# ktht/chan_vese

Measured on AMD Instinct MI355X. Metric: Mpixel-iterations/s (CSV u-update), higher is better.
Workload: dtype f64

## Files before the change

chan_vese_amd/csrc/api.hip:

```cpp
#include "cvh_host.h"

static thread_local char g_create_err[kErrLen] = "no error";
char *create_err() { return g_create_err; }

int fail(cvh_context *ctx, int code, const char *fmt, ...)
{
  char *dst = ctx ? ctx->err : g_create_err;
  va_list ap;
  va_start(ap, fmt);
  vsnprintf(dst, 512, fmt, ap);
  va_end(ap);
  return code;
}

extern "C" const char *cvh_version(void) { return "chanvese_hip 0.1 (gfx950)"; }

void cvh_fill_note(CvhLaunchNote *note, unsigned grid, unsigned block, size_t lds, const char *fmt, ...)
{
  va_list ap;
  va_start(ap, fmt);
  vsnprintf(note->name, sizeof(note->name), fmt, ap);
  va_end(ap);
  note->grid = grid; note->block = block; note->lds = (unsigned)lds;
}

void fill_atan_tables(double *tab)
{
  const long double pil = 3.14159265358979323846264338327950288L;
  for (int i = 0; i < CVH_ATAN_N; ++i) {
    const long double at = atanl((long double)i / (CVH_ATAN_N - 1));
    tab[i] = (double)at;
    tab[CVH_ATAN_N + i] = (double)(pil / 2 - at);
  }
  for (int j = 0; j < CVH_ATAN2_N; ++j)
    tab[2 * CVH_ATAN_N + j] = (double)((pil / 4 + atanl((long double)(j - 128) / 128)) / pil);
}

extern "C" void cvh_default_params(cvh_params *p)
{
  if (!p) return;
  p->mu = 0.5; p->nu = 0.0; p->dt = 1.0; p->eps = 1.0; p->tol = 0.001;
  for (int k = 0; k < CVH_MAX_CHANNELS; ++k) { p->lambda1[k] = 1.0; p->lambda2[k] = 1.0; }
}

extern "C" int cvh_device_count(int *count)
{
  if (!count) return CVH_ERR_ARG;
  int n = 0;
  hipError_t e = hipGetDeviceCount(&n);
  if (e != hipSuccess) { *count = 0; return fail(nullptr, CVH_ERR_HIP, "hipGetDeviceCount: %s", hipGetErrorString(e)); }
  *count = n;
  return CVH_OK;
}

extern "C" const char *cvh_last_error(const cvh_context *ctx) { return ctx ? ctx->err : g_create_err; }

static int check_params(cvh_context *ctx, const cvh_params *p, int C)
{
  if (!(p->dt > 0)) return fail(ctx, CVH_ERR_ARG, "Cannot have negative or zero timestep: %f.", p->dt);
  if (p->mu < 0) return fail(ctx, CVH_ERR_ARG, "Length penalty parameter cannot be negative: %f.", p->mu);
  for (int k = 0; k < C; ++k) {
    if (p->lambda1[k] < 0) return fail(ctx, CVH_ERR_ARG, "The value of lambda1 cannot be negative.");
    if (p->lambda2[k] < 0) return fail(ctx, CVH_ERR_ARG, "The value of lambda2 cannot be negative.");
  }
  return CVH_OK;
}

static std::mutex g_live_mu;
static std::vector<cvh_context *> g_live;

static int live_contexts(const cvh_context *c)
{
  std::lock_guard<std::mutex> lk(g_live_mu);
  int k = 0;
  for (const cvh_context *o : g_live)
    if (o->device == c->device && o->co_resident && ((o->have_u && o->have_image) || o == c)) ++k;
  return k;
}

bool run_is_alone(const cvh_context *c)
{
  if (c->run_alone < 0 || c->enqueued == 0) c->run_alone = live_contexts(c) <= 1 ? 1 : 0;
  return c->run_alone != 0;
}

double live_footprint(const cvh_context *c)
{
  std::lock_guard<std::mutex> lk(g_live_mu);
  double sum = 0.0;
  for (const cvh_context *o : g_live)
    if (o->device == c->device && o->co_resident && ((o->have_u && o->have_image) || o == c))
      sum += (double)o->n * (2.0 * (o->state_bits / 8) + o->C);
  return sum;
}

extern "C" void cvh_destroy(cvh_context *c)
{
  if (!c) return;
  {
    std::lock_guard<std::mutex> lk(g_live_mu);
    g_live.erase(std::remove(g_live.begin(), g_live.end(), c), g_live.end());
  }
  (void)hipSetDevice(c->device);
  if (c->stream) (void)hipStreamSynchronize(c->stream);
  if (c->d_img_slab) (void)hipFree(c->d_img_slab);
  if (c->d_u_slab) (void)hipFree(c->d_u_slab);
  if (c->d_uf_slab) (void)hipFree(c->d_uf_slab);
  for (int k = 0; k < 2; ++k) if (c->d_pm[k]) (void)hipFree(c->d_pm[k]);
  if (c->d_state) (void)hipFree(c->d_state);
  if (c->h_state) (void)hipHostFree(c->h_state);
  if (c->d_partials) (void)hipFree(c->d_partials);
  if (c->d_trace) (void)hipFree(c->d_trace);
  if (c->d_mask) (void)hipFree(c->d_mask);
  if (c->d_atan) (void)hipFree(c->d_atan);
  if (c->d_dbg) (void)hipFree(c->d_dbg);
  for (int k = 0; k < 4; ++k) if (c->graphs[k].exec) (void)hipGraphExecDestroy(c->graphs[k].exec);
  if (c->pm_graph) (void)hipGraphExecDestroy(c->pm_graph);
  if (c->d_dummy) (void)hipFree(c->d_dummy);
  if (c->d_chain) (void)hipFree(c->d_chain);
  if (c->d_resident) (void)hipFree(c->d_resident);
  if (c->d_res_halo) (void)hipFree(c->d_res_halo);
  if (c->d_pm_halo) (void)hipFree(c->d_pm_halo);
  free_table(&c->pm_batch);
  free_table(&c->io_table);
  if (c->h_io) (void)hipHostFree(c->h_io);
  if (c->d_reinit) (void)hipFree(c->d_reinit);
  if (c->d_cc) (void)hipFree(c->d_cc);
  for (DeviceTable *t : {&c->cc_table, &c->regions, &c->contour_edges, &c->contour_points, &c->overlap}) free_table(t);
  if (c->d_contour) (void)hipFree(c->d_contour);
  if (c->d_hist) (void)hipFree(c->d_hist);
  if (c->d_energy) (void)hipFree(c->d_energy);
  if (c->d_score) (void)hipFree(c->d_score);
  if (c->d_morph) (void)hipFree(c->d_morph);
  if (c->d_local) (void)hipFree(c->d_local);
  if (c->d_rank) (void)hipFree(c->d_rank);
  if (c->d_overlap_plane) (void)hipFree(c->d_overlap_plane);
  if (c->ev_io_in) (void)hipEventDestroy(c->ev_io_in);
  if (c->ev_io_out) (void)hipEventDestroy(c->ev_io_out);
  if (c->h_resident) (void)hipHostFree(c->h_resident);
  if (c->d_bounds) (void)hipFree(c->d_bounds);
  if (c->h_status) (void)hipHostFree(c->h_status);
  if (c->d_isums) (void)hipFree(c->d_isums);
  if (c->h_isums) (void)hipHostFree(c->h_isums);
  batch_cache_free(c);
  if (c->ev_join) (void)hipEventDestroy(c->ev_join);
  if (c->ev0) (void)hipEventDestroy(c->ev0);
  if (c->ev1) (void)hipEventDestroy(c->ev1);
  for (int k = 0; k < 4; ++k) if (c->evp[k]) (void)hipEventDestroy(c->evp[k]);
  if (c->stream) (void)hipStreamDestroy(c->stream);
  delete c;
}

static int create_impl(cvh_context *c)
{
  HIPCHK(c, hipSetDevice(c->device));
  HIPCHK(c, hipStreamCreateWithFlags(&c->stream, hipStreamNonBlocking));
  {
    int cus = 0;
    if (hipDeviceGetAttribute(&cus, hipDeviceAttributeMultiprocessorCount, c->device) == hipSuccess && cus > 0) c->num_cus = cus;
  }
  c->img_stride = (c->n + 255) & ~(size_t)255;
  HIPCHK(c, hipMalloc((void **)&c->d_img_slab, c->img_stride * c->C));
  for (int k = 0; k < c->C; ++k) c->d_img[k] = c->d_img_slab + (size_t)k * c->img_stride;
  {
    const size_t each = (((c->n + 64) * sizeof(double)) + ((size_t)2 << 20) - 1) & ~(((size_t)2 << 20) - 1);
    HIPCHK(c, hipMalloc((void **)&c->d_u_slab, 2 * each));
    c->d_u[0] = (double *)c->d_u_slab;
    c->d_u[1] = (double *)((char *)c->d_u_slab + each);
  }
  HIPCHK(c, hipMalloc((void **)&c->d_state, sizeof(CvhState)));
  HIPCHK(c, hipMemset(c->d_state, 0, sizeof(CvhState)));
  HIPCHK(c, hipHostMalloc((void **)&c->h_state, 4 * sizeof(CvhState), hipHostMallocDefault));
  memset(c->h_state, 0, 4 * sizeof(CvhState));
  int step_blocks = cvh_step_max_blocks(c->h, c->w);
  {
    const int wave_blocks = (((c->w + cvh_wave_cols() - 1) / cvh_wave_cols() + 3) / 4) * c->h + 1;
    if (wave_blocks > step_blocks) step_blocks = wave_blocks;
  }
  {
    double tab[2 * CVH_ATAN_N + CVH_ATAN2_N];
    fill_atan_tables(tab);
    HIPCHK(c, hipMalloc((void **)&c->d_atan, sizeof(tab)));
    HIPCHK(c, hipMemcpy(c->d_atan, tab, sizeof(tab), hipMemcpyHostToDevice));
  }
  const int init_blocks = cvh_init_sum_blocks(c->h, c->w);
  c->partial_rows = step_blocks > init_blocks ? step_blocks : init_blocks;
  HIPCHK(c, hipMalloc((void **)&c->d_partials, (size_t)c->partial_rows * cvh_nsums(c->C) * sizeof(double)));
  HIPCHK(c, hipMalloc((void **)&c->d_dummy, (size_t)(c->w > 64 ? c->w : 64) * sizeof(double)));
  HIPCHK(c, hipMalloc((void **)&c->d_bounds, (size_t)(c->h + 2) * sizeof(int)));
  HIPCHK(c, hipMalloc((void **)&c->d_chain, sizeof(CvhChainAcc)));
  HIPCHK(c, hipMemset(c->d_chain, 0, sizeof(CvhChainAcc)));
  HIPCHK(c, hipHostMalloc((void **)&c->h_status, 64, hipHostMallocMapped));
  c->h_status[0] = 0; c->h_status[1] = 0;
  HIPCHK(c, hipMalloc((void **)&c->d_isums, 8 * sizeof(unsigned long long)));
  HIPCHK(c, hipHostMalloc((void **)&c->h_isums, 8 * sizeof(unsigned long long), hipHostMallocDefault));
  HIPCHK(c, hipEventCreate(&c->ev0));
  HIPCHK(c, hipEventCreate(&c->ev1));
  for (hipEvent_t *ev : {&c->evp[0], &c->evp[1], &c->evp[2], &c->evp[3], &c->ev_join, &c->ev_io_in, &c->ev_io_out})
    HIPCHK(c, hipEventCreateWithFlags(ev, hipEventDisableTiming));
  snprintf(c->err, sizeof(c->err), "no error");
  return CVH_OK;
}

extern "C" int cvh_create(cvh_context **out, int h, int w, int channels, const cvh_params *p, int device)
{
  if (!out) return fail(nullptr, CVH_ERR_ARG, "cvh_create: out is NULL");
  *out = nullptr;
  if (h <= 0 || w <= 0) return fail(nullptr, CVH_ERR_ARG, "cvh_create: image size must be positive (got %d x %d)", h, w);
  if (channels != 1 && channels != 3)
    return fail(nullptr, CVH_ERR_ARG, "cvh_create: channels must be 1 (grayscale) or 3 (colour), got %d", channels);
  cvh_params def;
  cvh_default_params(&def);
  if (!p) p = &def;
  int rc = check_params(nullptr, p, channels);
  if (rc != CVH_OK) return rc;
  int ndev = 0;
  if (hipGetDeviceCount(&ndev) != hipSuccess || ndev <= 0)
    return fail(nullptr, CVH_ERR_HIP, "cvh_create: no HIP device available (this library has no CPU fallback)");
  if (device < 0 || device >= ndev) return fail(nullptr, CVH_ERR_ARG, "cvh_create: device %d out of range [0,%d)", device, ndev);
  cvh_context *c = new (std::nothrow) cvh_context();
  if (!c) return fail(nullptr, CVH_ERR_NOMEM, "cvh_create: out of host memory");
  c->h = h; c->w = w; c->C = channels; c->device = device; c->n = (size_t)h * w; c->p = *p;
  rc = create_impl(c);
  if (rc != CVH_OK) {
    snprintf(g_create_err, kErrLen, "%s", c->err);
    cvh_destroy(c);
    return rc;
  }
  {
    std::lock_guard<std::mutex> lk(g_live_mu);
    g_live.push_back(c);
  }
  *out = c;
  return CVH_OK;
}

extern "C" int cvh_set_params(cvh_context *c, const cvh_params *p)
{
  if (!c || !p) return CVH_ERR_ARG;
  int rc = check_params(c, p, c->C);
  if (rc != CVH_OK) return rc;
  if (p->eps != c->p.eps) c->sums_valid = false;
  c->p = *p;
  return CVH_OK;
}

extern "C" int cvh_set_option(cvh_context *c, const char *key, long value)
{
  if (!c || !key) return CVH_ERR_ARG;
  HIPCHK(c, hipSetDevice(c->device));
  { const int rc = settle(c); if (rc != CVH_OK) return rc; }
  if (!strcmp(key, "math_mode")) {
    if (value < 0 || value > 2) return fail(c, CVH_ERR_ARG, "math_mode must be 0, 1 or 2");
    c->math_mode = (int)value;
  } else if (!strcmp(key, "finalize")) {
    if (value != 0 && value != 1) return fail(c, CVH_ERR_ARG, "finalize must be 0 or 1");
    c->finalize_mode = (int)value;
  } else if (!strcmp(key, "tile_rows")) {
    if (value != 0 && value != 12 && value != 14 && value != 16) return fail(c, CVH_ERR_ARG, "tile_rows must be 0 (auto), 12, 14 or 16");
    c->tile_rows = (int)value;
  } else if (!strcmp(key, "kernel")) {
    if (value < -1 || value > 3 || value == 1)
      return fail(c, CVH_ERR_ARG, "kernel must be -1 (auto), 0 (tile), 2 (wave) or 3 (wave, 2 pixels per lane)");
    c->kernel = (int)value;
  } else if (!strcmp(key, "pm_kernel")) {
    if (value < -1 || value > 4 || value == 2)
      return fail(c, CVH_ERR_ARG, "pm_kernel must be -1 (auto), 0 (tile), 1 (wave), 3 (wave, 2 time steps per launch) or 4 (resident plane)");
    c->pm_kernel = (int)value;
  } else if (!strcmp(key, "res_straight")) {
    c->res_straight = value ? 1 : 0;
  } else if (!strcmp(key, "pm_strip_rows")) {
    if (value < 0) return fail(c, CVH_ERR_ARG, "pm_strip_rows must be >= 0");
    c->pm_strip_rows = (int)value;
  } else if (!strcmp(key, "wave_occupancy")) {
    if (value < 3 || value > 5) return fail(c, CVH_ERR_ARG, "wave_occupancy must be 3..5 (more waves per SIMD would spill registers)");
    c->wave_minw = (int)value;
  } else if (!strcmp(key, "debug_times")) {
    if (c->d_dbg) { HIPCHK(c, hipFree(c->d_dbg)); c->d_dbg = nullptr; c->dbg_words = 0; }
    if (value > 0) {
      c->dbg_words = (size_t)c->partial_rows * 20 + 16;
      if (c->dbg_words < (size_t)CVH_RESIDENT_MAX_TILES * 12 + 64) c->dbg_words = (size_t)CVH_RESIDENT_MAX_TILES * 12 + 64;
      HIPCHK(c, hipMalloc((void **)&c->d_dbg, c->dbg_words * 8));
      HIPCHK(c, hipMemset(c->d_dbg, 0, c->dbg_words * 8));
    }
  } else if (!strcmp(key, "graph")) {
    c->use_graph = value != 0;
  } else if (!strcmp(key, "wave_xcd")) {
    c->wave_xcd = value != 0;
  } else if (!strcmp(key, "wave_rev")) {
    c->wave_rev = value != 0;
  } else if (!strcmp(key, "wave_skew")) {
    if (value < 0 || value > 500) return fail(c, CVH_ERR_ARG, "wave_skew must be 0..500 (per mille)");
    c->wave_skew = (int)value;
  } else if (!strcmp(key, "chain")) {
    c->chain_opt = value != 0;
  } else if (!strcmp(key, "resident")) {
    if (value < -1 || value > 1) return fail(c, CVH_ERR_ARG, "resident must be -1 (auto), 0 or 1");
    c->resident_opt = (int)value;
  } else if (!strcmp(key, "far_terms")) {
    if (value != 4 && value != 5) return fail(c, CVH_ERR_ARG, "far_terms must be 4 or 5");
    c->far_terms = (int)value;
  } else if (!strcmp(key, "wave_pol")) {
    if (value < -1 || value > 2) return fail(c, CVH_ERR_ARG, "wave_pol must be -1 (auto), 0, 1 or 2 (diagnostic: non-temporal loads)");
    c->wave_pol = (int)value;
  } else if (!strcmp(key, "wave_cls")) {
    if (value < 0 || value > 2) return fail(c, CVH_ERR_ARG, "wave_cls must be 0 (off), 1 (2-pixel kernel) or 2 (1-pixel kernel too)");
    c->wave_cls = (int)value;
  } else if (!strcmp(key, "wave_cskew")) {
    if (value < 0 || value > 900) return fail(c, CVH_ERR_ARG, "wave_cskew must be 0..900 (per mille)");
    c->wave_cskew = (int)value;
  } else if (!strcmp(key, "wave_depth")) {
    if (value != 4 && value != 8) return fail(c, CVH_ERR_ARG, "wave_depth must be 4 or 8");
    c->wave_depth = (int)value;
  } else if (!strcmp(key, "wave_imgv")) {
    c->wave_imgv = value != 0;
  } else if (!strcmp(key, "wave_sync")) {
    c->wave_sync = value < 0 ? -1 : (value != 0);
  } else if (!strcmp(key, "wave_seam")) {
    if (value != 0 && value != 1) return fail(c, CVH_ERR_ARG, "wave_seam must be 0 or 1");
    c->wave_seam = (int)value;
  } else if (!strcmp(key, "near_switch")) {
    c->near_switch = value != 0;
  } else if (!strcmp(key, "res_prio")) {
    c->res_prio = value != 0;
  } else if (!strcmp(key, "res_go_share")) {
    if (value < 0 || value > 6) return fail(c, CVH_ERR_ARG, "res_go_share must be 0 .. 6");
    c->res_go_share = (int)value;
  } else if (!strcmp(key, "co_resident")) {
    c->co_resident = value != 0;
  } else if (!strcmp(key, "state")) {
    if (value != 32 && value != 64) return fail(c, CVH_ERR_ARG, "state must be 64 or 32");
    if ((int)value != c->state_bits) {
      if (value == 32) {
        if (c->w % 16 != 0 || c->w < 144 || c->n >= ((size_t)1 << 28))
          return fail(c, CVH_ERR_ARG, "state 32 needs a width that is a multiple of 16 and >= 144, and fewer than 2^28 pixels (the 2-pixel wave kernel)");
        c->state_bits = 32;
        if (c->have_u) { const int rc = adopt_f32_state(c); if (rc != CVH_OK) return rc; }
      } else {
        if (c->have_u) { const int rc = ensure_f64_mirror(c); if (rc != CVH_OK) return rc; }
        c->state_bits = 64;
        c->mirror_valid = true;
      }
      c->sums_valid = false;
    }
  } else if (!strcmp(key, "wave_prio")) {
    if (value < 0 || value > 4) return fail(c, CVH_ERR_ARG, "wave_prio must be 0..4");
    c->wave_prio = (int)value;
  } else if (!strcmp(key, "wave_lds_cap")) {
    c->wave_lds_cap = value != 0;
  } else if (!strcmp(key, "strip_rows")) {
    if (value < 0) return fail(c, CVH_ERR_ARG, "strip_rows must be >= 0");
    c->strip_rows = (int)value;
  } else if (!strcmp(key, "strips")) {
    if (value < 0 || value > c->h) return fail(c, CVH_ERR_ARG, "strips must be 0 (auto) .. h");
    c->strips = (int)value;
  } else if (!strcmp(key, "lut")) {
    c->use_lut = value != 0;
  } else if (!strcmp(key, "dma")) {
    c->use_dma = value != 0;
  } else if (!strcmp(key, "sync_every")) {
    if (value < 1) return fail(c, CVH_ERR_ARG, "sync_every must be >= 1");
    c->sync_every = (int)(value > 1000000 ? 1000000 : value);
  } else if (!strcmp(key, "trace")) {
    if (value < 0) return fail(c, CVH_ERR_ARG, "trace capacity must be >= 0");
    HIPCHK(c, hipStreamSynchronize(c->stream));
    if (c->d_trace) { HIPCHK(c, hipFree(c->d_trace)); c->d_trace = nullptr; }
    c->trace_cap = 0;
    if (value > 0) {
      const size_t bytes = (size_t)value * (2 * c->C + 1) * sizeof(double);
      HIPCHK(c, hipMalloc((void **)&c->d_trace, bytes));
      HIPCHK(c, hipMemset(c->d_trace, 0, bytes));
      c->trace_cap = (int)value;
    }
  } else {
    return fail(c, CVH_ERR_ARG, "unknown option \"%s\"", key);
  }
  return CVH_OK;
}

double stop_norm_host(const std::vector<const uint8_t *> &planes, size_t n)
{
  const int C = (int)planes.size();
  const double inv = 1.0 / C;
  double sq[CVH_MAX_CHANNELS * 255 + 1];
  for (int t = 0; t <= 255 * C; ++t) { const double v = (double)t * inv; sq[t] = v * v; }
  auto at = [&](size_t q) {
    int t = 0;
    for (int k = 0; k < C; ++k) t += planes[k][q];
    return sq[t];
  };
  double s = 0;
  size_t i = 0;
  for (; i + 4 <= n; i += 4) s += ((at(i) + at(i + 1)) + at(i + 2)) + at(i + 3);
  for (; i < n; ++i) s += at(i);
  return sqrt(s);
}

int image_stats(cvh_context *c, const uint8_t *const *host_planes)
{
  HIPCHK(c, hipMemsetAsync(c->d_isums, 0, 8 * sizeof(unsigned long long), c->stream));
  HIPCHK(c, cvh_launch_image_sums(c->d_img, c->C, c->n, c->d_isums, c->stream));
  HIPCHK(c, hipMemcpyAsync(c->h_isums, c->d_isums, 8 * sizeof(unsigned long long), hipMemcpyDeviceToHost, c->stream));
  const bool exact_on_device = stop_norm_exact_on_device(c);
  std::vector<std::vector<uint8_t>> fetched;
  std::vector<const uint8_t *> pl;
  if (!exact_on_device) {
    if (host_planes) pl.assign(host_planes, host_planes + c->C);
    else {
      try { fetched.assign(c->C, std::vector<uint8_t>(c->n)); } catch (...) { return fail(c, CVH_ERR_NOMEM, "out of host memory"); }
      for (int k = 0; k < c->C; ++k) {
        HIPCHK(c, hipMemcpyAsync(fetched[k].data(), c->d_img[k], c->n, hipMemcpyDeviceToHost, c->stream));
        pl.push_back(fetched[k].data());
      }
    }
  }
  HIPCHK(c, hipStreamSynchronize(c->stream));
  const double host_norm = exact_on_device ? 0.0 : stop_norm_host(pl, c->n);
  plane_sums_arrived(c, c->h_isums, exact_on_device ? nullptr : &host_norm);
  return CVH_OK;
}

extern "C" int cvh_set_image(cvh_context *c, const uint8_t *const *planes)
{
  if (!c || !planes) return CVH_ERR_ARG;
  for (int k = 0; k < c->C; ++k) if (!planes[k]) return fail(c, CVH_ERR_ARG, "cvh_set_image: plane %d is NULL", k);
  HIPCHK(c, hipSetDevice(c->device));
  { const int rc = settle(c); if (rc != CVH_OK) return rc; }
  for (int k = 0; k < c->C; ++k)
    HIPCHK(c, hipMemcpyAsync(c->d_img[k], planes[k], c->n, hipMemcpyHostToDevice, c->stream));
  return image_stats(c, planes);
}

extern "C" int cvh_get_image(cvh_context *c, uint8_t *const *planes)
{
  if (!c || !planes) return CVH_ERR_ARG;
  if (!c->have_image) return fail(c, CVH_ERR_STATE, "cvh_get_image: no image set");
  HIPCHK(c, hipSetDevice(c->device));
  for (int k = 0; k < c->C; ++k) {
    if (!planes[k]) return fail(c, CVH_ERR_ARG, "cvh_get_image: plane %d is NULL", k);
    HIPCHK(c, hipMemcpyAsync(planes[k], c->d_img[k], c->n, hipMemcpyDeviceToHost, c->stream));
  }
  HIPCHK(c, hipStreamSynchronize(c->stream));
  return CVH_OK;
}

int settle(cvh_context *c) { return c->timing_open || c->chain_pending ? sync_impl(c) : CVH_OK; }

static void begin_run_host(cvh_context *c)
{
  c->cur_base = current_buffer(c);
  c->chain_pb = (c->chain_pb + c->steps_done) & 3;
  c->steps_done = 0;
  c->enqueued = 0;
  c->run_pol = -1; c->run_alone = -1; c->run_chunk = -1;
  c->h_status[0] = 0; c->h_status[1] = 0;
}

int reset_run_impl(cvh_context *c)
{
  { const int rc = settle(c); if (rc != CVH_OK) return rc; }
  begin_run_host(c);
  static const int zeros[4] = {0, 0, 0, 0};
  HIPCHK(c, hipMemcpyAsync(&c->d_state->steps_done, zeros, sizeof(zeros), hipMemcpyHostToDevice, c->stream));
  HIPCHK(c, hipMemsetAsync(&c->d_chain->v[(c->chain_pb + 1) & 3][0], 0, sizeof(c->d_chain->v[0]), c->stream));
  HIPCHK(c, hipStreamSynchronize(c->stream));
  return CVH_OK;
}

int levelset_arrived(cvh_context *c, bool device_cleared)
{
  c->cur_base = c->chain_pb & 1; c->steps_done = 0; c->enqueued = 0;
  c->have_u = true;
  c->sums_valid = false;
  c->mirror_valid = true;
  if (c->state_bits == 32) { const int rc = adopt_f32_state(c); if (rc != CVH_OK) return rc; }
  if (!device_cleared) return reset_run_impl(c);
  begin_run_host(c);
  return CVH_OK;
}

void steps_enqueued(cvh_context *c, int n, int nparts, bool chain, bool resident)
{
  if (resident) { nparts = 0; c->resident_used = true; }
  if (chain) { c->chain_pending = true; c->pending_nparts = nparts; }
  else c->chain_acc_valid = false;
  c->last_nparts = nparts;
  if (c->state_bits == 32) c->mirror_valid = false;
  c->enqueued += n;
}

void sums_taken(cvh_context *c, bool chain) { c->sums_valid = true; c->chain_acc_valid = chain; }

bool stop_norm_exact_on_device(const cvh_context *c) { return c->C == 1 && c->n < ((size_t)1 << 36); }

void planes_changed(cvh_context *c) { c->stop_valid = false; c->sums_valid = false; }

void plane_sums_arrived(cvh_context *c, const unsigned long long *isums, const double *host_norm)
{
  planes_changed(c);
  for (int k = 0; k < c->C; ++k) c->sum_img[k] = (double)isums[2 * k];
  c->stop_norm = host_norm ? *host_norm : sqrt((double)isums[1]);
  c->stop_valid = true;
  c->have_image = true;
}

int adopt_f32_state(cvh_context *c)
{
  if (!c->d_uf_slab) {
    const size_t each = (((c->n + 64) * sizeof(float)) + ((size_t)2 << 20) - 1) & ~(((size_t)2 << 20) - 1);
    HIPCHK(c, hipMalloc((void **)&c->d_uf_slab, 2 * each));
    c->d_uf[0] = (float *)c->d_uf_slab;
    c->d_uf[1] = (float *)((char *)c->d_uf_slab + each);
  }
  const int cur = current_buffer(c);
  HIPCHK(c, cvh_launch_state_narrow(c->d_u[cur], c->d_uf[cur], c->n, c->stream));
  HIPCHK(c, hipStreamSynchronize(c->stream));
  c->mirror_valid = true;
  c->sums_valid = false;
  return CVH_OK;
}

int ensure_f64_mirror(cvh_context *c)
{
  if (c->state_bits != 32 || c->mirror_valid) return CVH_OK;
  { const int rc = settle(c); if (rc != CVH_OK) return rc; }
  const int cur = current_buffer(c);
  HIPCHK(c, cvh_launch_state_widen(c->d_uf[cur], c->d_u[cur], c->n, c->stream));
  HIPCHK(c, hipStreamSynchronize(c->stream));
  c->mirror_valid = true;
  return CVH_OK;
}

extern "C" int cvh_reset_run(cvh_context *c)
{
  if (!c) return CVH_ERR_ARG;
  HIPCHK(c, hipSetDevice(c->device));
  return reset_run_impl(c);
}

extern "C" int cvh_set_levelset(cvh_context *c, const double *u)
{
  if (!c || !u) return CVH_ERR_ARG;
  HIPCHK(c, hipSetDevice(c->device));
  { const int rc = settle(c); if (rc != CVH_OK) return rc; }
  HIPCHK(c, hipStreamSynchronize(c->stream));
  HIPCHK(c, hipMemcpyAsync(c->d_u[c->chain_pb & 1], u, c->n * sizeof(double), hipMemcpyHostToDevice, c->stream));
  HIPCHK(c, hipStreamSynchronize(c->stream));
  return levelset_arrived(c);
}

void checkerboard_factors(int h, int w, double *out)
{
  const double pi = 3.14159265358979323846;
  for (int i = 0; i < h; ++i) out[i] = sin(pi * i / 5);
  for (int j = 0; j < w; ++j) out[(size_t)h + j] = sin(pi * j / 5);
}

extern "C" void cvh_levelset_checkerboard_host(int h, int w, double *u)
{
  std::vector<double> sv((size_t)h + w);
  checkerboard_factors(h, w, sv.data());
  for (int i = 0; i < h; ++i)
    for (int j = 0; j < w; ++j) {
      const double z = sv[i] * sv[(size_t)h + j];
      u[(size_t)i * w + j] = (z == 0) ? 0.0 : (z < 0 ? -1.0 : 1.0);
    }
}

extern "C" int cvh_get_levelset(cvh_context *c, double *u)
{
  if (!c || !u) return CVH_ERR_ARG;
  if (!c->have_u) return fail(c, CVH_ERR_STATE, "cvh_get_levelset: no level set");
  HIPCHK(c, hipSetDevice(c->device));
  { const int rc = ensure_f64_mirror(c); if (rc != CVH_OK) return rc; }
  HIPCHK(c, hipMemcpyAsync(u, c->d_u[current_buffer(c)], c->n * sizeof(double), hipMemcpyDeviceToHost, c->stream));
  HIPCHK(c, hipStreamSynchronize(c->stream));
  return CVH_OK;
}

extern "C" int cvh_get_means(cvh_context *c, double *c1, double *c2)
{
  if (!c || !c1 || !c2) return CVH_ERR_ARG;
  HIPCHK(c, hipSetDevice(c->device));
  if (c->timing_open) return fail(c, CVH_ERR_STATE, "cvh_get_means: steps in flight, call cvh_sync first");
  int rc = prepare(c);
  if (rc != CVH_OK) return rc;
  HIPCHK(c, hipMemcpyAsync(&c->h_state[0], c->d_state, sizeof(CvhState), hipMemcpyDeviceToHost, c->stream));
  HIPCHK(c, hipStreamSynchronize(c->stream));
  for (int k = 0; k < c->C; ++k) { c1[k] = c->h_state[0].c1[k]; c2[k] = c->h_state[0].c2[k]; }
  return CVH_OK;
}

extern "C" int cvh_get_trace(cvh_context *c, double *out, int max_rows, int *rows)
{
  if (!c || !out || !rows || max_rows < 0) return CVH_ERR_ARG;
  HIPCHK(c, hipSetDevice(c->device));
  int n = c->steps_done < c->trace_cap ? c->steps_done : c->trace_cap;
  if (n > max_rows) n = max_rows;
  *rows = n;
  if (n > 0) {
    HIPCHK(c, hipMemcpyAsync(out, c->d_trace, (size_t)n * (2 * c->C + 1) * sizeof(double), hipMemcpyDeviceToHost, c->stream));
    HIPCHK(c, hipStreamSynchronize(c->stream));
  }
  return CVH_OK;
}

extern "C" int cvh_get_stop_condition(cvh_context *c, double *stop_cond)
{
  if (!c || !stop_cond) return CVH_ERR_ARG;
  HIPCHK(c, hipSetDevice(c->device));
  int rc = prepare(c);
  if (rc != CVH_OK) return rc;
  HIPCHK(c, hipStreamSynchronize(c->stream));
  *stop_cond = c->p.tol * c->stop_norm;
  return CVH_OK;
}

extern "C" int cvh_get_mask(cvh_context *c, uint8_t *mask, int invert)
{
  if (!c || !mask) return CVH_ERR_ARG;
  if (!c->have_u) return fail(c, CVH_ERR_STATE, "cvh_get_mask: no level set");
  static const char what[] = "cvh_get_mask";
  return mask_to_host(c, mask, [&]() { return mask_out(&c, 1, &c->d_mask, invert, c->stream, what); });
}

extern "C" int cvh_get_contour(cvh_context *c, uint8_t *contour)
{
  if (!c || !contour) return CVH_ERR_ARG;
  if (!c->have_u) return fail(c, CVH_ERR_STATE, "cvh_get_contour: no level set");
  HIPCHK(c, hipSetDevice(c->device));
  if (!c->d_mask) HIPCHK(c, hipMalloc((void **)&c->d_mask, c->n));
  { const int rc = ensure_f64_mirror(c); if (rc != CVH_OK) return rc; }
  HIPCHK(c, cvh_launch_contour(c->d_u[current_buffer(c)], c->d_mask, c->h, c->w, c->stream));
  HIPCHK(c, hipMemcpyAsync(contour, c->d_mask, c->n, hipMemcpyDeviceToHost, c->stream));
  HIPCHK(c, hipStreamSynchronize(c->stream));
  return CVH_OK;
}

extern "C" int cvh_separate(cvh_context *c, const uint8_t *img3, int invert, uint8_t *selection3)
{
  if (!c || !img3 || !selection3) return CVH_ERR_ARG;
  if (!c->have_u) return fail(c, CVH_ERR_STATE, "cvh_separate: no level set");
  HIPCHK(c, hipSetDevice(c->device));
  { const int rc = ensure_f64_mirror(c); if (rc != CVH_OK) return rc; }
  uint8_t *d_in = nullptr, *d_out = nullptr;
  HIPCHK(c, hipMalloc((void **)&d_in, c->n * 3));
  hipError_t e = hipMalloc((void **)&d_out, c->n * 3);
  if (e != hipSuccess) { (void)hipFree(d_in); return fail(c, CVH_ERR_HIP, "hipMalloc: %s", hipGetErrorString(e)); }
  int rc = CVH_OK;
  do {
    if ((e = hipMemcpyAsync(d_in, img3, c->n * 3, hipMemcpyHostToDevice, c->stream)) != hipSuccess) break;
    if ((e = cvh_launch_separate(d_in, c->d_u[current_buffer(c)], d_out, c->n, invert, c->stream)) != hipSuccess) break;
    if ((e = hipMemcpyAsync(selection3, d_out, c->n * 3, hipMemcpyDeviceToHost, c->stream)) != hipSuccess) break;
    e = hipStreamSynchronize(c->stream);
  } while (0);
  if (e != hipSuccess) rc = fail(c, CVH_ERR_HIP, "cvh_separate: %s", hipGetErrorString(e));
  (void)hipFree(d_in);
  (void)hipFree(d_out);
  return rc;
}

extern "C" int cvh_last_run_ms(cvh_context *c, float *ms)
{
  if (!c || !ms) return CVH_ERR_ARG;
  *ms = c->last_run_ms;
  return CVH_OK;
}

extern "C" int cvh_last_pm_ms(cvh_context *c, float *ms)
{
  if (!c || !ms) return CVH_ERR_ARG;
  *ms = c->last_pm_ms;
  return CVH_OK;
}

extern "C" int cvh_ppf_apply_device(double *d_data, long n, int op, double eps, void *stream)
{
  if (!d_data || n < 0 || op < 0 || op > 2) return fail(nullptr, CVH_ERR_ARG, "cvh_ppf_apply_device: bad argument");
  hipError_t e = cvh_launch_ppf(d_data, (size_t)n, op, eps, (hipStream_t)stream);
  if (e != hipSuccess) return fail(nullptr, CVH_ERR_HIP, "cvh_ppf_apply_device: %s", hipGetErrorString(e));
  return CVH_OK;
}

extern "C" int cvh_ppf_apply(double *data, int w, long start, long end, int op, double eps, int device)
{
  if (!data || w <= 0 || start < 0 || end < start || op < 0 || op > 2)
    return fail(nullptr, CVH_ERR_ARG, "cvh_ppf_apply: bad argument");
  if (end == start) return CVH_OK;
  hipError_t e = hipSetDevice(device);
  if (e != hipSuccess) return fail(nullptr, CVH_ERR_HIP, "cvh_ppf_apply: hipSetDevice: %s (no CPU fallback)", hipGetErrorString(e));
  const size_t n = (size_t)(end - start);
  hipStream_t st = nullptr;
  if ((e = hipStreamCreateWithFlags(&st, hipStreamNonBlocking)) != hipSuccess)
    return fail(nullptr, CVH_ERR_HIP, "cvh_ppf_apply: hipStreamCreate: %s", hipGetErrorString(e));
  double *d = nullptr;
  bool pooled = true;
  if (hipMallocAsync((void **)&d, n * sizeof(double), st) != hipSuccess) {
    (void)hipGetLastError();
    pooled = false;
    if ((e = hipMalloc((void **)&d, n * sizeof(double))) != hipSuccess) {
      (void)hipStreamDestroy(st);
      return fail(nullptr, CVH_ERR_HIP, "cvh_ppf_apply: hipMalloc: %s", hipGetErrorString(e));
    }
  }
  do {
    if ((e = hipMemcpyAsync(d, data + start, n * sizeof(double), hipMemcpyHostToDevice, st)) != hipSuccess) break;
    if ((e = cvh_launch_ppf(d, n, op, eps, st)) != hipSuccess) break;
    if ((e = hipMemcpyAsync(data + start, d, n * sizeof(double), hipMemcpyDeviceToHost, st)) != hipSuccess) break;
    e = hipStreamSynchronize(st);
  } while (0);
  if (pooled) { (void)hipFreeAsync(d, st); (void)hipStreamSynchronize(st); } else (void)hipFree(d);
  (void)hipStreamDestroy(st);
  if (e != hipSuccess) return fail(nullptr, CVH_ERR_HIP, "cvh_ppf_apply: %s", hipGetErrorString(e));
  return CVH_OK;
}

extern "C" int cvh_launch_info(cvh_context *c, int phase, char *buf, int cap)
{
  if (!c || !buf || cap < 1 || (phase != 0 && phase != 1)) return CVH_ERR_ARG;
  if (phase == 1) {
    if (!c->pm_desc[0]) return fail(c, CVH_ERR_STATE, "cvh_launch_info: cvh_perona_malik has not run on this context");
    snprintf(buf, (size_t)cap, "%s", c->pm_desc);
    return CVH_OK;
  }
  CvhLaunchNote note{};
  {
    ResidentGeom rg;
    if (resident_geometry(c, &rg)) {
      const int rc = launch_resident(c, rg, 1, &note);
      if (rc != CVH_OK) return rc;
      snprintf(buf, (size_t)cap, "kernel=%s grid=%u block=%u lds_bytes=%u data_flow=4 tiles_y=%d tiles_x=%d tile_rows=%d chain=1 math=fast "
               "steps_per_launch=chunk", note.name, note.grid, note.block, note.lds, rg.tr, rg.tc, (c->h + rg.tr - 1) / rg.tr);
      return CVH_OK;
    }
  }
  const int rc = launch_one_step(c, current_buffer(c), c->enqueued, true, &note);
  if (rc != CVH_OK) return rc;
  const Geometry g = resolve_geometry(c);
  CvhStepArgs a;
  fill_args(c, &a, current_buffer(c), c->enqueued);
  snprintf(buf, (size_t)cap, "kernel=%s grid=%u block=%u lds_bytes=%u data_flow=%d wave_columns=%d strips=%d strip_rows=%d chain=%d "
           "wave_pol=%d math=%s steps_per_graph=%d wave_seam=%d", note.name, note.grid, note.block, note.lds, g.strip, g.tiles_x, g.tiles_y,
           g.strip_rows, a.chain ? 1 : 0, a.wave_pol, use_fast(c) ? "fast" : "strict", c->use_graph ? kGraphSteps : 0,
           (g.strip == 3 && use_fast(c)) ? a.wave_seam : 0);
  return CVH_OK;
}
```

chan_vese_amd/csrc/csv_batch.hip:

```cpp
#include "cvh_host.h"

struct BatchGroup {
  CvhStepArgs rep;
  int kind = 0, C = 1, fast = 0;
  int n = 0;
  unsigned grid = 0;
  size_t args_off = 0, map_off = 0;
};
struct BatchCache {
  std::vector<cvh_context *> members;
  std::vector<unsigned char> image;
  std::vector<BatchGroup> groups;
  DeviceTable table;
  int rot = 0;
};

int grow_table(cvh_context *c, DeviceTable *t, size_t bytes)
{
  if (t->cap >= bytes) return CVH_OK;
  free_table(t);
  HIPCHK(c, hipMalloc(&t->d, bytes));
  t->cap = bytes;
  return CVH_OK;
}

int grow_table_to(cvh_context *c, DeviceTable *t, size_t want, size_t count, size_t bytes)
{
  if (t->count >= want) return CVH_OK;
  free_table(t);
  HIPCHK(c, hipMalloc(&t->d, bytes));
  t->cap = bytes; t->count = count;
  return CVH_OK;
}

void free_table(DeviceTable *t)
{
  if (t->d) (void)hipFree(t->d);
  t->d = nullptr; t->cap = t->count = 0;
}

void batch_cache_free(cvh_context *c)
{
  if (!c->batch) return;
  free_table(&c->batch->table);
  delete c->batch;
  c->batch = nullptr;
}

int batch_fail(cvh_context *const *ctxs, int n, int code, const char *fmt, ...)
{
  char msg[512];
  va_list ap;
  va_start(ap, fmt);
  vsnprintf(msg, sizeof(msg), fmt, ap);
  va_end(ap);
  snprintf(create_err(), kErrLen, "%s", msg);
  if (ctxs && n >= 1 && ctxs[0]) snprintf(ctxs[0]->err, sizeof(ctxs[0]->err), "%s", msg);
  return code;
}

int members_check(cvh_context *const *ctxs, int n, const char *what, MemberNeeds needs)
{
  if (!ctxs || n < 1) return batch_fail(ctxs, 0, CVH_ERR_ARG, "%s: empty member list (ctxs = %p, n = %d)", what, (const void *)ctxs, n);
  for (int i = 0; i < n; ++i) {
    cvh_context *c = ctxs[i];
    if (!c) return batch_fail(ctxs, i ? n : 0, CVH_ERR_ARG, "%s: member %d is NULL", what, i);
    for (int j = 0; j < i; ++j)
      if (ctxs[j] == c) return batch_fail(ctxs, n, CVH_ERR_ARG, "%s: member %d duplicates member %d", what, i, j);
    if (c->device != ctxs[0]->device)
      return batch_fail(ctxs, n, CVH_ERR_ARG, "%s: member %d is on device %d, member 0 on device %d", what, i, c->device, ctxs[0]->device);
    if (needs == kMembersListed) continue;
    if (!c->have_image) return batch_fail(ctxs, n, CVH_ERR_STATE, "batch: member %d has no image (call cvh_set_image first)", i);
    if (needs == kMembersWithImage) continue;
    if (!c->have_u) return batch_fail(ctxs, n, CVH_ERR_STATE, "batch: member %d has no level set (call cvh_set_levelset or cvh_init_checkerboard first)", i);
    if (c->finalize_mode != 0) return batch_fail(ctxs, n, CVH_ERR_ARG, "batch: member %d has finalize = 1 (a separate finalise kernel per launch): no fused batch", i);
    const Geometry g = resolve_geometry(c);
    if (g.strip < 2) return batch_fail(ctxs, n, CVH_ERR_ARG, "batch: member %d (%d x %d) takes the tile kernel: no fused batch", i, c->h, c->w);
  }
  return CVH_OK;
}


int members_below(cvh_context *const *ctxs, int n, const char *what, int k, int only)
{
  for (int i = std::max(only, 0); i < (only < 0 ? n : only + 1); ++i)
    if (ctxs[i]->n >= ((size_t)1 << k))
      return batch_fail(ctxs, n, CVH_ERR_ARG, "%s: member %d: %d x %d is too large, h * w must stay below 2^%d", what, i, ctxs[i]->h, ctxs[i]->w, k);
  return CVH_OK;
}

int members_distances_fit(cvh_context *const *ctxs, int n, const char *what, int only)
{
  for (int i = std::max(only, 0); i < (only < 0 ? n : only + 1); ++i) {
    const cvh_context *c = ctxs[i];
    if ((unsigned long long)c->h * c->h + (unsigned long long)c->w * c->w >= (1ull << 32))
      return batch_fail(ctxs, n, CVH_ERR_ARG, "%s: member %d: %d x %d is too large, h^2 + w^2 must stay below 2^32", what, i, c->h, c->w);
  }
  return CVH_OK;
}

template <class T>
int members_caps_fit(cvh_context *const *ctxs, int n, const char *what, const void *const *lists, const T *caps, const char *noun, const char *without,
                     int only)
{
  for (int i = std::max(only, 0); lists && i < (only < 0 ? n : only + 1); ++i) {
    if (!lists[i]) continue;
    if (!caps) return batch_fail(ctxs, n, CVH_ERR_ARG, "%s: %s", what, without);
    if (caps[i] < 0) return batch_fail(ctxs, n, CVH_ERR_ARG, "%s: member %d: %s must not be negative, got %ld", what, i, noun, (long)caps[i]);
  }
  return CVH_OK;
}
template int members_caps_fit<int>(cvh_context *const *, int, const char *, const void *const *, const int *, const char *, const char *, int);
template int members_caps_fit<long>(cvh_context *const *, int, const char *, const void *const *, const long *, const char *, const char *, int);

int members_have_images(cvh_context *const *ctxs, int n, const char *what)
{
  for (int i = 0; i < n; ++i)
    if (!ctxs[i]->have_image) return batch_fail(ctxs, n, CVH_ERR_STATE, "%s: member %d has no image (call cvh_set_image first)", what, i);
  return CVH_OK;
}

int members_have_levelsets(cvh_context *const *ctxs, int n, const char *what, int only)
{
  for (int i = std::max(only, 0); i < (only < 0 ? n : only + 1); ++i)
    if (!ctxs[i]->have_u) return batch_fail(ctxs, n, CVH_ERR_STATE, "%s: member %d has no level set", what, i);
  return CVH_OK;
}

int members_mirrors_fresh(cvh_context *const *ctxs, int n, const char *what, int first, const char *noun)
{
  for (int i = first; i < n; ++i) {
    const int rc = ensure_f64_mirror(ctxs[i]);
    if (rc != CVH_OK) return batch_fail(ctxs, n, rc, "%s: %s %d: %s", what, noun, i - first, ctxs[i]->err);
  }
  return CVH_OK;
}

int pairs_check(const PairRoles &p, int n, const char *what, std::vector<cvh_context *> *all, const std::function<int(int)> &rule,
                const std::function<int()> &args)
{
  if (!p.first || !p.second || n < 1)
    return batch_fail(nullptr, 0, CVH_ERR_ARG, "%s: empty pair list (%s = %p, %s = %p, n = %d)", what, p.first_name, (const void *)p.first, p.second_name,
                      (const void *)p.second, n);
  for (int i = 0; i < n; ++i)
    if (!p.first[i] || !p.second[i])
      return batch_fail(nullptr, 0, CVH_ERR_ARG, "%s: pair %d: the %s context is NULL", what, i, p.first[i] ? p.second_role : p.first_role);
  cvh_context *const *dst = p.second_is_dst ? p.second : p.first, *const *src = p.second_is_dst ? p.first : p.second;
  all->assign(dst, dst + n);
  all->insert(all->end(), src, src + n);
  cvh_context *const *ctxs = all->data();
  auto role = [&](int i) { return (i < n) == p.second_is_dst ? p.second_role : p.first_role; };
  for (int i = 0; i < 2 * n; ++i)
    for (int j = 0; j < i; ++j)
      if (ctxs[i] == ctxs[j])
        return batch_fail(ctxs, 2 * n, CVH_ERR_ARG, "%s: pair %d: its %s context is also pair %d's %s context (a context may be listed once)", what, i % n,
                          role(i), j % n, role(j));
  if (args) { const int rc = args(); if (rc != CVH_OK) return rc; }
  for (int i = 0; i < n; ++i) {
    const cvh_context *a = p.first[i], *b = p.second[i];
    for (const cvh_context *x : {a, b})
      if (x->device != ctxs[0]->device)
        return batch_fail(ctxs, 2 * n, CVH_ERR_ARG, "%s: pair %d: its %s context is on device %d, pair 0's on device %d", what, i,
                          x == a ? p.first_role : p.second_role, x->device, ctxs[0]->device);
    const int rc = rule(i);
    if (rc != CVH_OK) return rc;
    if (a->n >= ((size_t)1 << 32))
      return batch_fail(ctxs, 2 * n, CVH_ERR_ARG, "%s: pair %d: %d x %d is too large, h * w must stay below 2^32", what, i, a->h, a->w);
  }
  return CVH_OK;
}

int pair_sources_have_images(cvh_context *const *all, int n, const char *what, const char *role)
{
  for (int i = 0; i < n; ++i)
    if (!all[n + i]->have_image)
      return batch_fail(all, 2 * n, CVH_ERR_STATE, "%s: pair %d: the %s context has no image (call cvh_set_image first)", what, i, role);
  return CVH_OK;
}

constexpr int kBatchOwnRows = 32;
static void batch_share(cvh_context *const *ctxs, int n, bool on)
{
  double tot = 0.0;
  for (int i = 0; i < n; ++i) tot += (double)ctxs[i]->n;
  for (int i = 0; i < n; ++i) {
    cvh_context *c = ctxs[i];
    c->geom_cus = 0;
    if (!on || resolve_geometry(c).strip_rows >= kBatchOwnRows) continue;
    const int share = (int)((double)c->num_cus * (double)c->n / tot + 0.5);
    c->geom_cus = share < 1 ? 1 : share;
  }
}

static int batch_prepare(cvh_context *const *ctxs, int n)
{
  for (int i = 0; i < n; ++i) {
    cvh_context *c = ctxs[i];
    HIPCHK(c, hipSetDevice(c->device));
    int rc = prepare_host(c);
    if (rc != CVH_OK) return batch_fail(ctxs, n, rc, "batch: member %d: %s", i, c->err);
    const Geometry g = resolve_geometry(c);
    rc = upload_strip_bounds(c, g);
    if (rc == CVH_OK) rc = flush_for_grid(c, g.nblocks);
    if (rc == CVH_OK) rc = prepare(c);
    if (rc != CVH_OK) return batch_fail(ctxs, n, rc, "batch: member %d: %s", i, c->err);
  }
  cvh_context *lead = ctxs[0];
  std::vector<BatchGroup> groups;
  std::vector<std::string> names;
  std::vector<int> member_group((size_t)n), local((size_t)n);
  std::vector<unsigned> blocks((size_t)n);
  for (int i = 0; i < n; ++i) {
    cvh_context *c = ctxs[i];
    CvhLaunchNote note{};
    const int rc = launch_one_step(c, (c->cur_base + c->enqueued) & 1, c->enqueued, false, &note);
    if (rc != CVH_OK) return batch_fail(ctxs, n, rc, "batch: member %d: %s", i, c->err);
    char key[160];
    snprintf(key, sizeof(key), "%s lds=%u", note.name, note.lds);
    int gi = 0;
    while (gi < (int)names.size() && names[gi] != key) ++gi;
    if (gi == (int)names.size()) {
      names.push_back(key);
      BatchGroup bg;
      fill_args(c, &bg.rep, (c->cur_base + c->enqueued) & 1, c->enqueued);
      bg.kind = resolve_geometry(c).strip; bg.C = c->C; bg.fast = use_fast(c) ? 1 : 0;
      groups.push_back(bg);
    }
    member_group[i] = gi;
    local[i] = groups[gi].n++;
    blocks[i] = note.grid;
  }
  std::vector<unsigned char> img;
  auto align = [&]() { img.resize((img.size() + 255) & ~(size_t)255); };
  for (size_t gi = 0; gi < groups.size(); ++gi) {
    BatchGroup &bg = groups[gi];
    align();
    bg.args_off = img.size();
    img.resize(img.size() + (size_t)4 * bg.n * sizeof(CvhStepArgs));
    for (int i = 0; i < n; ++i) {
      if (member_group[i] != (int)gi) continue;
      cvh_context *c = ctxs[i];
      for (int q = 0; q < 4; ++q) {
        CvhStepArgs a;
        fill_args(c, &a, (c->cur_base + c->enqueued + q) & 1, c->enqueued + q);
        memcpy(img.data() + bg.args_off + ((size_t)q * bg.n + local[i]) * sizeof(CvhStepArgs), &a, sizeof(a));
      }
    }
    align();
    bg.map_off = img.size();
    unsigned first = 0;
    for (int i = 0; i < n; ++i) {
      if (member_group[i] != (int)gi) continue;
      const unsigned len = (blocks[i] + 7) & ~7u;
      for (unsigned j = 0; j < len; j += 8) {
        const CvhBatchEntry e = {(unsigned)local[i], first, blocks[i], 0u};
        img.insert(img.end(), (const unsigned char *)&e, (const unsigned char *)&e + sizeof(e));
      }
      first += len;
    }
    bg.grid = first;
  }
  BatchCache *bc = lead->batch;
  bool same_members = bc && bc->members.size() == (size_t)n && !memcmp(bc->members.data(), ctxs, (size_t)n * sizeof(cvh_context *));
  if (same_members && bc->image.size() == img.size() && bc->groups.size() == groups.size()) {
    for (int r = 0; r < 4; ++r) {
      bool eq = true;
      for (size_t gi = 0; gi < groups.size() && eq; ++gi) {
        const BatchGroup &bg = groups[gi], &old = bc->groups[gi];
        eq = bg.args_off == old.args_off && bg.map_off == old.map_off && bg.n == old.n && bg.grid == old.grid;
        const size_t row = (size_t)bg.n * sizeof(CvhStepArgs);
        for (int q = 0; q < 4 && eq; ++q)
          eq = !memcmp(img.data() + bg.args_off + (size_t)q * row, bc->image.data() + old.args_off + (size_t)((q + r) & 3) * row, row);
        if (eq) eq = !memcmp(img.data() + bg.map_off, bc->image.data() + old.map_off, (size_t)bg.grid / 8 * sizeof(CvhBatchEntry));
      }
      if (eq) { bc->rot = r; return CVH_OK; }
    }
  }
  if (!bc) { bc = lead->batch = new (std::nothrow) BatchCache(); if (!bc) return batch_fail(ctxs, n, CVH_ERR_NOMEM, "batch: out of host memory"); }
  HIPCHK(lead, hipStreamSynchronize(lead->stream));
  const int rc = grow_table(lead, &bc->table, img.size());
  if (rc != CVH_OK) return rc;
  HIPCHK(lead, hipMemcpy(bc->table.d, img.data(), img.size(), hipMemcpyHostToDevice));
  bc->members.assign(ctxs, ctxs + n);
  bc->image.swap(img);
  bc->groups = groups;
  bc->rot = 0;
  return CVH_OK;
}

int join_into_leader(cvh_context *const *ctxs, int n, const int *member)
{
  cvh_context *lead = ctxs[0];
  for (int i = 1; i < n; ++i) {
    if (member && !member[i]) continue;
    HIPCHK(ctxs[i], hipEventRecord(ctxs[i]->ev_join, ctxs[i]->stream));
    HIPCHK(lead, hipStreamWaitEvent(lead->stream, ctxs[i]->ev_join, 0));
  }
  return CVH_OK;
}

static int batch_launch(cvh_context *const *ctxs, int n, int nsteps)
{
  cvh_context *lead = ctxs[0];
  BatchCache *bc = lead->batch;
  { const int rc = join_into_leader(ctxs, n); if (rc != CVH_OK) return rc; }
  for (int i = 0; i < n; ++i) {
    cvh_context *c = ctxs[i];
    if (!c->timing_open) { HIPCHK(c, hipEventRecord(c->ev0, lead->stream)); c->timing_open = true; }
  }
  const unsigned char *d = (const unsigned char *)bc->table.d;
  for (int t = 0; t < nsteps; ++t) {
    const int q = (t + bc->rot) & 3;
    for (const BatchGroup &bg : bc->groups) {
      CvhBatchLaunch bl;
      bl.k.map = (const CvhBatchEntry *)(d + bg.map_off);
      bl.k.args = (const CvhStepArgs *)(d + bg.args_off) + (size_t)q * bg.n;
      bl.grid = bg.grid;
      if (bg.kind == 3) HIPCHK(lead, cvh_launch_wave2(bg.rep, bg.C, bg.fast, lead->stream, &bl));
      else HIPCHK(lead, cvh_launch_wave(bg.rep, bg.C, bg.fast, lead->stream, &bl));
    }
  }
  bc->rot = (bc->rot + nsteps) & 3;
  HIPCHK(lead, hipEventRecord(lead->ev_join, lead->stream));
  for (int i = 0; i < n; ++i) {
    cvh_context *c = ctxs[i];
    if (i) HIPCHK(c, hipStreamWaitEvent(c->stream, lead->ev_join, 0));
    if (nsteps > 0) {
      const Geometry g = resolve_geometry(c);
      steps_enqueued(c, nsteps, g.nblocks, use_chain(c, g), false);
    }
  }
  return CVH_OK;
}

extern "C" int cvh_enqueue_steps_batch(cvh_context *const *ctxs, int n, int nsteps)
{
  int rc = members_check(ctxs, n, "batch", kMembersForCsv);
  if (rc != CVH_OK) return rc;
  if (nsteps < 0) return batch_fail(ctxs, n, CVH_ERR_ARG, "batch: nsteps = %d", nsteps);
  HIPCHK(ctxs[0], hipSetDevice(ctxs[0]->device));
  batch_share(ctxs, n, true);
  for (int i = 0; i < n; ++i) if (nsteps > 0) ctxs[i]->run_chunk = nsteps;
  rc = batch_prepare(ctxs, n);
  if (rc == CVH_OK) rc = batch_launch(ctxs, n, nsteps);
  batch_share(ctxs, n, false);
  return rc;
}

extern "C" int cvh_run_batch(cvh_context *const *ctxs, int n, int max_steps, int *steps_done, double *last_norm)
{
  int rc = members_check(ctxs, n, "batch", kMembersForCsv);
  if (rc != CVH_OK) return rc;
  cvh_context *lead = ctxs[0];
  HIPCHK(lead, hipSetDevice(lead->device));
  for (int i = 0; i < n; ++i) {
    rc = reset_run_impl(ctxs[i]);
    if (rc != CVH_OK) return batch_fail(ctxs, n, rc, "batch: member %d: %s", i, ctxs[i]->err);
  }
  long remaining = max_steps < 0 ? (long)INT_MAX : (long)max_steps;
  int chunk_len = INT_MAX;
  for (int i = 0; i < n; ++i) if (ctxs[i]->sync_every < chunk_len) chunk_len = ctxs[i]->sync_every;
  if (chunk_len < 1) chunk_len = 1;
  batch_share(ctxs, n, true);
  for (int i = 0; i < n; ++i) ctxs[i]->run_chunk = chunk_len;
  rc = batch_prepare(ctxs, n);
  if (rc == CVH_OK) rc = batch_launch(ctxs, n, 0);
  constexpr int kAhead = 4;
  long queued = 0;
  while (rc == CVH_OK && remaining > 0) {
    bool all_stopped = true;
    for (;;) {
      long lag = 0;
      all_stopped = true;
      for (int i = 0; i < n; ++i) {
        volatile int *hs = ctxs[i]->h_status;
        if (hs[1]) continue;
        all_stopped = false;
        if (queued - hs[0] > lag) lag = queued - hs[0];
      }
      if (all_stopped || lag <= (long)kAhead * chunk_len) break;
      if (hipStreamQuery(lead->stream) == hipSuccess) break;
    }
    if (all_stopped) break;
    const int chunk = (int)(remaining < chunk_len ? remaining : chunk_len);
    rc = batch_launch(ctxs, n, chunk);
    remaining -= chunk;
    queued += chunk;
  }
  batch_share(ctxs, n, false);
  if (rc != CVH_OK) return rc;
  for (int i = 0; i < n; ++i) {
    cvh_context *c = ctxs[i];
    c->timing_open = true;
    rc = sync_impl(c);
    if (rc != CVH_OK) return batch_fail(ctxs, n, rc, "batch: member %d: %s", i, c->err);
    if (steps_done) steps_done[i] = c->h_state[0].steps_done;
    if (last_norm) last_norm[i] = c->h_state[0].norm;
  }
  return CVH_OK;
}
```

chan_vese_amd/csrc/csv_run.hip:

```cpp
#include "cvh_host.h"

Geometry resolve_geometry(const cvh_context *c)
{
  Geometry g;
  g.strip = 0;
  const int cus = c->geom_cus > 0 ? c->geom_cus : c->num_cus;
  const bool two_px_c3 = c->C == 3 && use_fast(c) && (c->kernel == 3 || c->kernel == -1 || c->state_bits == 32);
  if ((c->kernel == 3 || c->state_bits == 32 || (c->kernel == -1 && c->n >= (size_t)600000)) && (c->C == 1 || two_px_c3) && c->w % 16 == 0 &&
      c->w >= 144 && c->n < ((size_t)1 << 28)) {
    g.strip = 3;
    g.rows = 4;
    g.tiles_x = (c->w + cvh_wave2_cols() - 1) / cvh_wave2_cols();
    const int nbc = (g.tiles_x + 1) / 2;
    int sr = c->strip_rows, small_exact = 0;
    if (sr <= 0) {
      const int occ = use_fast(c) ? (c->wave_minw == 4 ? 4 : 3) : 2;
      int nstrips = 2 * ((cus * occ) / nbc);
      bool exact = false;
      if (nstrips > 160) { nstrips = 2 * ((2 * cus) / nbc); if (nstrips < 2) nstrips = 2; exact = true; }
      if (nstrips < 1) nstrips = 1;
      sr = (c->h + nstrips - 1) / nstrips;
      if (sr < 8) { sr = 8; exact = false; }
      if (exact && c->wave_cls && c->wave_xcd) small_exact = nstrips;
    }
    g.strip_rows = sr;
    g.tiles_y = small_exact ? small_exact : (c->h + sr - 1) / sr;
    if (c->strips > 0 && c->strip_rows <= 0 && c->wave_cls && c->wave_xcd) {
      g.tiles_y = c->strips;
      g.strip_rows = (c->h + c->strips - 1) / c->strips;
      if (g.strip_rows < 8) { g.strip_rows = 8; g.tiles_y = (c->h + 7) / 8; }
    }
    g.nblocks = nbc * ((g.tiles_y + 1) / 2);
    return g;
  }
  if ((c->kernel == 2 || c->kernel == 3 || c->kernel == -1) && c->n < ((size_t)1 << 28)) {
    g.strip = 2;
    g.rows = 4;
    g.tiles_x = (c->w + cvh_wave_cols() - 1) / cvh_wave_cols();
    int sr = c->strip_rows;
    if (sr <= 0) {
      const int occ = use_fast(c) ? (c->C == 3 ? 3 : c->wave_minw) : (c->C == 3 ? 2 : 3);
      int nstrips = (cus * occ) / ((g.tiles_x + 3) / 4);
      if (nstrips > 80) nstrips = 64;
      if (nstrips < 1) nstrips = 1;
      sr = (c->h + nstrips - 1) / nstrips;
      if (sr < 8) sr = 8;
    }
    g.strip_rows = sr;
    g.tiles_y = (c->h + sr - 1) / sr;
    g.nblocks = ((g.tiles_x + 3) / 4) * g.tiles_y;
    return g;
  }
  g.rows = c->tile_rows == 16 ? 16 : 14;
  cvh_step_grid(c->h, c->w, g.rows, &g.tiles_x, &g.tiles_y);
  g.strip_rows = g.rows;
  g.nblocks = g.tiles_x * g.tiles_y;
  return g;
}

bool use_chain(const cvh_context *c, const Geometry &g)
{
  return (g.strip == 3 || g.strip == 2) && use_fast(c) && c->finalize_mode == 0 && c->chain_opt;
}

bool resident_tile_grid(int h, int w, int channels, int num_cus, int cap_blocks, ResidentGeom *rg)
{
  if ((channels != 1 && channels != 3) || (w & 1) || w < 16 || h < 16) return false;
  const int tw = cvh_resident_tile_w(), thmax = cvh_resident_tile_hmax(channels);
  const int tc = (w + tw - 1) / tw;
  int cap = cap_blocks < CVH_RESIDENT_MAX_TILES ? cap_blocks : CVH_RESIDENT_MAX_TILES;
  if (cap > num_cus) cap = num_cus;
  int tr = cap / tc;
  if (tr < 1) return false;
  if (tr > h / 16) tr = h / 16;
  if ((h + tr - 1) / tr > thmax) return false;
  rg->tr = tr; rg->tc = tc; rg->band = 0;
  return true;
}

bool launches_cooperatively(cvh_context *c)
{
  if (c->coop_launch < 0) {
    int coop = 0;
    c->coop_launch = hipDeviceGetAttribute(&coop, hipDeviceAttributeCooperativeLaunch, c->device) == hipSuccess && coop ? 1 : 0;
  }
  return c->coop_launch != 0;
}

bool resident_geometry(cvh_context *c, ResidentGeom *rg)
{
  if (c->C == 3 && c->resident_opt != 1) return false;
  if (!c->resident_opt || (c->C != 1 && c->C != 3) || !use_fast(c) || !c->chain_opt || c->finalize_mode != 0 || (c->w & 1) || c->w < 16 || c->h < 16) return false;
  if (c->state_bits == 32) return false;
  if (!(c->kernel == -1 || c->kernel == 2 || c->kernel == 3)) return false;
  if (c->resident_opt < 0 && (c->kernel != -1 || c->strip_rows != 0 || c->strips != 0 || !c->use_graph)) return false;
  if (c->resident_opt < 0 && !run_is_alone(c)) {
    const double px = (double)c->h * (double)c->w;
    const int need = px >= 3.6e6 ? 48 : px >= 2.9e6 ? 72 : px >= 2.2e6 ? 100 : INT_MAX;
    if (c->run_chunk < need) return false;
  }
  if (c->resident_cap < 0) c->resident_cap = launches_cooperatively(c) ? cvh_resident_blocks_per_cu(c->C) * c->num_cus : 0;
  if (c->resident_cap <= 0) return false;
  return resident_tile_grid(c->h, c->w, c->C, c->num_cus, c->resident_cap, rg);
}

static int class_major_cls(const cvh_context *c, const Geometry &g)
{
  return (((g.strip == 3 && c->wave_cls) || (g.strip == 2 && c->wave_cls == 2)) && c->wave_xcd) ? (c->num_cus >= 8 ? c->num_cus / 8 : 1) : 0;
}

void fill_args(const cvh_context *c, CvhStepArgs *a, int in_buf, int step)
{
  memset(a, 0, sizeof(*a));
  a->u_in = c->d_u[in_buf];
  a->u_out = c->d_u[in_buf ^ 1];
  a->state32 = 0;
  if (c->state_bits == 32) {
    a->u_in = reinterpret_cast<const double *>(c->d_uf[in_buf]);
    a->u_out = reinterpret_cast<double *>(c->d_uf[in_buf ^ 1]);
    a->state32 = 1;
  }
  for (int k = 0; k < c->C; ++k) a->img[k] = c->d_img[k];
  a->img_stride = (unsigned)c->img_stride;
  a->st = c->d_state;
  a->partials = c->d_partials;
  a->trace = c->d_trace;
  a->trace_cap = c->trace_cap;
  a->h = c->h; a->w = c->w;
  Geometry g = resolve_geometry(c);
  a->tiles_x = g.tiles_x; a->tiles_y = g.tiles_y;
  a->nparts = g.nblocks;
  a->tile_rows = g.rows;
  a->strip_rows = g.strip_rows;
  a->fused_finalize = c->finalize_mode == 0;
  a->alpha = c->p.mu * c->p.dt;
  a->beta = (1.0 / c->C) * c->p.dt;
  a->gamma = -c->p.nu * c->p.dt;
  a->eps = c->p.eps;
  for (int k = 0; k < CVH_MAX_CHANNELS; ++k) { a->lambda1[k] = c->p.lambda1[k]; a->lambda2[k] = c->p.lambda2[k]; }
  const double pi = 3.14159265358979323846;
  a->atan_tab = c->d_atan;
  a->atan2_tab = c->d_atan + 2 * CVH_ATAN_N;
  a->wave_minw = c->wave_minw;
  a->wave_lds_cap = c->wave_lds_cap;
  a->wave_prio = c->wave_prio;
  a->wave_sync = c->wave_sync >= 0 ? c->wave_sync : (c->C == 3 ? 0 : 1);
  a->near_switch = c->near_switch;
  a->wave_seam = c->wave_seam;
  a->res_prio = c->res_prio;
  a->res_go_shift = c->res_go_share;
  a->wave_depth = c->wave_depth;
  a->wave_imgv = c->wave_imgv;
  a->dummy = c->d_dummy;
  a->strip_bounds = c->d_bounds;
  a->wave_rev = c->wave_rev;
  a->wave_xcd = c->wave_xcd;
  if (use_chain(c, g)) {
    a->chain = c->d_chain;
    a->chain_pb = c->chain_pb;
    a->chain_phase = (c->chain_pb + step) & 3;
    a->chain_s4 = c->d_partials;
    const double bound[4] = {0.5 * (double)c->n, 127.5 * (double)c->n, 127.5 * (double)c->n, 127.5 * (double)c->n};
    for (int k = 0; k < 4; ++k) {
      int e = 0;
      while (ldexp(1.0, e) < bound[k] + 1.0) ++e;
      a->chain_scale[k] = ldexp(1.0, 62 - e);
      a->chain_inv[k] = ldexp(1.0, e - 62);
    }
  }
  if (c->wave_pol >= 0) a->wave_pol = c->wave_pol;
  else {
    if (c->run_pol < 0 || c->enqueued == 0) c->run_pol = live_footprint(c) <= 300e6 ? 1 : 0;
    a->wave_pol = c->run_pol;
  }
  a->wave_cls = class_major_cls(c, g);
  a->host_status = c->h_status;
  a->dbg_times = c->d_dbg;
  a->inv_eps = 1.0 / c->p.eps;
  a->dk1 = pi / c->p.eps;
  a->dk2 = pi * c->p.eps;
  far_coef(c->p.eps, c->far_terms, a->far_k, &a->far_thr);
  a->stop_cond = c->stop_cond_h;
  a->npix = (double)c->n;
  for (int k = 0; k < CVH_MAX_CHANNELS; ++k) a->sum_img[k] = c->sum_img[k];
  a->derive_complement = use_fast(c) ? (g.strip >= 2 ? 2 : 1) : 0;
  a->use_lut = c->use_lut;
  a->use_dma = c->use_dma;
}

void far_coef(double eps, int far_terms, double k[5], double *thr)
{
  const double pi = 3.14159265358979323846;
  const double e = eps, e2 = e * e;
  k[0] = e / pi; k[1] = -(e * e2) / (3.0 * pi);
  k[2] = (e * e2 * e2) / (5.0 * pi); k[3] = -(e * e2 * e2 * e2) / (7.0 * pi);
  k[4] = far_terms == 5 ? (e * e2 * e2 * e2 * e2) / (9.0 * pi) : 0.0;
  *thr = (far_terms == 5 ? 32.0 : 64.0) * e;
}

int prepare_host(cvh_context *c)
{
  if (!c->have_image) return fail(c, CVH_ERR_STATE, "no image set (call cvh_set_image first)");
  if (!c->have_u) return fail(c, CVH_ERR_STATE, "no level set (call cvh_set_levelset or cvh_init_checkerboard first)");
  if (!c->stop_valid) {
    const int rc = image_stats(c, nullptr);
    if (rc != CVH_OK) return rc;
  }
  c->stop_cond_h = c->p.tol * c->stop_norm;
  if (c->state_bits == 32 && (!use_fast(c) || resolve_geometry(c).strip != 3))
    return fail(c, CVH_ERR_ARG, "state 32 runs the 2-pixel wave kernel in FAST arithmetic only (math_mode, kernel)");
  return CVH_OK;
}

int prepare(cvh_context *c)
{
  int rc0 = prepare_host(c);
  if (rc0 != CVH_OK) return rc0;
  const bool chain = use_chain(c, resolve_geometry(c));
  if (!c->sums_valid || (chain && !c->chain_acc_valid)) {
    CvhStepArgs a;
    fill_args(c, &a, current_buffer(c), c->enqueued);
    if (c->state_bits == 32) {
      const int rc = ensure_f64_mirror(c);
      if (rc != CVH_OK) return rc;
      a.u_in = c->d_u[current_buffer(c)];
    }
    int nparts = 0;
    HIPCHK(c, cvh_launch_init_sums(a, c->C, use_fast(c), &nparts, c->stream));
    a.nparts = nparts;
    HIPCHK(c, cvh_launch_finalize(a, c->C, 1, c->stream));
    sums_taken(c, chain);
  }
  return CVH_OK;
}

void compute_strip_bounds(int kind, int h, int tiles_x, int S, int strip_rows, int nblocks, int cls, int cskew, int skew,
                          std::vector<int> &b)
{
  b.assign((size_t)S + 1, 0);
  if (cls) {
    const int spw = kind == 3 ? 2 : 1;
    const int nbc = kind == 3 ? (tiles_x + 1) / 2 : (tiles_x + 3) / 4, nb = nblocks, q = nb >> 3, r = nb & 7;
    const int npairs = (S + spw - 1) / spw;
    int ncls = 0;
    std::vector<long> K;
    for (;; ++ncls) {
      long tot = 0;
      for (int x = 0; x < 8; ++x) { const int nx = q + (x < r ? 1 : 0); const long lim = (long)(ncls + 1) * cls; tot += nx < lim ? nx : lim; }
      K.push_back(tot);
      if (tot >= nb) { ++ncls; break; }
    }
    const double a_ = cskew / 1000.0, mid = (ncls - 1) / 2.0;
    std::vector<double> wgt((size_t)S);
    double total = 0;
    for (int sp = 0; sp < npairs; ++sp) {
      const long rank = (long)sp * nbc + nbc / 2;
      int k = 0;
      while (k < ncls - 1 && rank >= K[k]) ++k;
      const double wv = 1.0 + a_ * (mid - k) / (mid > 0 ? mid : 1.0);
      for (int t = 0; t < spw && spw * sp + t < S; ++t) { wgt[spw * sp + t] = wv; total += wv; }
    }
    double cum = 0;
    for (int k = 0; k < S; ++k) { b[k] = (int)((double)h * (cum / total) + 0.5); cum += wgt[k]; }
    for (int k = 1; k < S; ++k) if (b[k] < b[k - 1]) b[k] = b[k - 1];
  } else {
    const double alpha = skew / 1000.0;
    for (int k = 0; k <= S; ++k) {
      long v;
      if (skew == 0) v = (long)k * strip_rows;
      else { const double x = (double)k / S; v = (long)((double)h * (x + alpha * x * (1.0 - x))); }
      b[k] = (int)(v < h ? v : h);
    }
  }
  b[S] = h;
}

int upload_strip_bounds(cvh_context *c, const Geometry &g)
{
  const int cls = class_major_cls(c, g);
  const bool alone = run_is_alone(c);
  const int key[4] = {g.tiles_y, g.strip_rows, c->wave_skew + 1000 * (cls ? c->wave_cskew + 1 : 0) + 10000000 * g.strip + (c->state_bits == 32 ? 500000000 : 0) + (alone ? 0 : 250000000), c->h};
  if (!memcmp(key, c->bounds_key, sizeof(key))) return CVH_OK;
  std::vector<int> b;
  int cskew = c->wave_cskew;
  if (g.strip_rows > 46) cskew = g.strip_rows >= 128 ? 0 : (int)(cskew * (128.0 - g.strip_rows) / (128.0 - 46.0));
  if (c->C == 3 && c->wave_cskew == 500) cskew = c->state_bits == 32 ? 0 : 425;
  if (!alone && c->wave_cskew == 500) cskew = 0;
  compute_strip_bounds(g.strip, c->h, g.tiles_x, g.tiles_y, g.strip_rows, g.nblocks, cls, cskew, c->wave_skew, b);
  HIPCHK(c, hipStreamSynchronize(c->stream));
  HIPCHK(c, hipMemcpy(c->d_bounds, b.data(), b.size() * sizeof(int), hipMemcpyHostToDevice));
  memcpy(c->bounds_key, key, sizeof(key));
  return CVH_OK;
}

int launch_one_step(cvh_context *c, int in_buf, int step, bool capturing, CvhLaunchNote *note)
{
  CvhStepArgs a;
  fill_args(c, &a, in_buf, step);
  a.note = note;
  const int kind = resolve_geometry(c).strip;
  if (kind == 3) HIPCHK(c, cvh_launch_wave2(a, c->C, use_fast(c), c->stream));
  else if (kind == 2) HIPCHK(c, cvh_launch_wave(a, c->C, use_fast(c), c->stream));
  else HIPCHK(c, cvh_launch_step(a, c->C, use_fast(c), c->stream));
  if (note) return CVH_OK;
  if (c->finalize_mode == 1) HIPCHK(c, cvh_launch_finalize(a, c->C, 0, c->stream));
  if (!capturing) steps_enqueued(c, 1, a.nparts, a.chain != nullptr, false);
  return CVH_OK;
}

static int chain_flush(cvh_context *c)
{
  if (!c->chain_pending) return CVH_OK;
  CvhStepArgs a;
  fill_args(c, &a, 0, 0);
  if (!a.chain) return fail(c, CVH_ERR_STATE, "chain-mode launches are pending but the context no longer selects chain mode");
  if (c->pending_nparts > 0) a.nparts = c->pending_nparts;
  HIPCHK(c, cvh_launch_chain_flush(a, c->C, c->stream));
  c->chain_pending = false;
  return CVH_OK;
}

int flush_for_grid(cvh_context *c, int nparts)
{
  if (c->chain_pending && c->pending_nparts > 0 && c->pending_nparts != nparts) return chain_flush(c);
  return CVH_OK;
}

static int ensure_step_graph(cvh_context *c, int parity)
{
  StepGraph &g = c->graphs[(c->chain_pb + c->enqueued) & 3];
  CvhStepArgs key[4];
  for (int s = 0; s < 4; ++s) fill_args(c, &key[s], parity ^ (s & 1), c->enqueued + s);
  const int kind = resolve_geometry(c).strip, flavour = (use_fast(c) ? 1 : 0) | (c->finalize_mode << 1);
  if (g.exec && g.kind == kind && g.flavour == flavour && !memcmp(key, g.key, sizeof(key))) return CVH_OK;
  if (g.exec) {
    HIPCHK(c, hipStreamSynchronize(c->stream));
    (void)hipGraphExecDestroy(g.exec);
    g.exec = nullptr;
  }
  const int rc = capture_graph(c, &g.exec, [&] {
    int r = CVH_OK;
    for (int s = 0; s < kGraphSteps && r == CVH_OK; ++s) r = launch_one_step(c, parity ^ (s & 1), c->enqueued + s, true);
    return r;
  }, "hipStreamEndCapture: %s");
  if (rc != CVH_OK) return rc;
  memcpy(g.key, key, sizeof(key));
  g.kind = kind; g.flavour = flavour;
  return CVH_OK;
}

static int warm_impl(cvh_context *c, long nsteps)
{
  if (nsteps > 0) c->run_chunk = (int)(nsteps < 1024 ? nsteps : 1024);
  { ResidentGeom rg; if (resident_geometry(c, &rg)) return CVH_OK; }
  const Geometry g = resolve_geometry(c);
  if (g.strip >= 2) { const int rc = upload_strip_bounds(c, g); if (rc != CVH_OK) return rc; }
  if (c->use_graph && nsteps >= kGraphSteps) {
    const int ahead = (int)(nsteps % kGraphSteps);
    c->enqueued += ahead;
    const int rc = ensure_step_graph(c, (c->cur_base + c->enqueued) & 1);
    c->enqueued -= ahead;
    if (rc != CVH_OK) return rc;
  }
  return CVH_OK;
}

int ensure_resident_buffers(cvh_context *c)
{
  if (c->d_resident) return CVH_OK;
  const int halo = cvh_resident_halo_doubles();
  HIPCHK(c, hipMalloc((void **)&c->d_resident, sizeof(CvhResident)));
  HIPCHK(c, hipMalloc((void **)&c->d_res_halo, (size_t)2 * CVH_RESIDENT_MAX_TILES * halo * sizeof(double)));
  HIPCHK(c, hipHostMalloc((void **)&c->h_resident, 64, hipHostMallocDefault));
  memset(c->h_resident, 0, 64);
  return CVH_OK;
}

int launch_resident(cvh_context *c, const ResidentGeom &rg, int nsteps, CvhLaunchNote *note)
{
  const int ntiles = rg.tr * rg.tc;
  if (!note) { const int rc = ensure_resident_buffers(c); if (rc != CVH_OK) return rc; }
  if (!note) { const int rc = flush_for_grid(c, -1); if (rc != CVH_OK) return rc; }
  constexpr int kMaxPerLaunch = 4096;
  for (int s = 0; s < nsteps || note;) {
    const int n = nsteps - s < kMaxPerLaunch ? nsteps - s : kMaxPerLaunch;
    CvhStepArgs a;
    fill_args(c, &a, (c->cur_base + c->enqueued) & 1, c->enqueued);
    if (!a.chain) return fail(c, CVH_ERR_STATE, "resident mode needs chain-mode sums");
    a.tiles_x = rg.tc; a.tiles_y = rg.tr; a.nparts = ntiles;
    {
      const int th = c->h % rg.tr == 0 ? c->h / rg.tr : 0;
      a.res_band_rows = (c->res_straight && (th == 16 || th == 32 || th == 64 || th == 128) && th <= cvh_resident_tile_hmax(c->C)) ? th / 8 : 0;
    }
    a.resident = c->d_resident;
    a.res_halo = c->d_res_halo;
    a.res_steps = n;
    a.res_t0 = c->enqueued;
    a.res_poll_cap = 2000000;
    a.note = note;
    if (note) { HIPCHK(c, cvh_launch_resident(a, c->C, c->stream)); return CVH_OK; }
    HIPCHK(c, hipMemsetAsync(c->d_resident, 0, c->C == 1 ? CVH_RESIDENT_C1_BYTES : sizeof(CvhResident), c->stream));
    HIPCHK(c, cvh_launch_resident(a, c->C, c->stream));
    steps_enqueued(c, n, ntiles, true, true);
    s += n;
  }
  return CVH_OK;
}

static int enqueue_impl(cvh_context *c, int nsteps)
{
  if (nsteps > 0) c->run_chunk = nsteps;
  {
    ResidentGeom rg;
    if (resident_geometry(c, &rg)) return launch_resident(c, rg, nsteps, nullptr);
    const Geometry g = resolve_geometry(c);
    if (g.strip >= 2) { const int rc = upload_strip_bounds(c, g); if (rc != CVH_OK) return rc; }
    const int rc = flush_for_grid(c, g.nblocks);
    if (rc != CVH_OK) return rc;
  }
  int s = 0;
  const int plain = (c->use_graph && nsteps >= kGraphSteps) ? nsteps % kGraphSteps : nsteps;
  for (; s < plain; ++s) {
    const int rc = launch_one_step(c, (c->cur_base + c->enqueued) & 1, c->enqueued);
    if (rc != CVH_OK) return rc;
  }
  while (nsteps - s >= kGraphSteps) {
    const int parity = (c->cur_base + c->enqueued) & 1;
    const int rc = ensure_step_graph(c, parity);
    if (rc != CVH_OK) return rc;
    const StepGraph &sg = c->graphs[(c->chain_pb + c->enqueued) & 3];
    HIPCHK(c, hipGraphLaunch(sg.exec, c->stream));
    steps_enqueued(c, kGraphSteps, sg.key[0].nparts, sg.key[0].chain != nullptr, false);
    s += kGraphSteps;
  }
  return CVH_OK;
}

extern "C" int cvh_enqueue_steps(cvh_context *c, int nsteps)
{
  if (!c || nsteps < 0) return CVH_ERR_ARG;
  HIPCHK(c, hipSetDevice(c->device));
  int rc = prepare_host(c);
  if (rc != CVH_OK) return rc;
  rc = warm_impl(c, nsteps);
  if (rc != CVH_OK) return rc;
  if (!c->timing_open) {
    HIPCHK(c, hipEventRecord(c->ev0, c->stream));
    c->timing_open = true;
  }
  rc = prepare(c);
  if (rc != CVH_OK) return rc;
  return enqueue_impl(c, nsteps);
}

extern "C" int cvh_warm(cvh_context *c, int nsteps)
{
  if (!c || nsteps < 0) return CVH_ERR_ARG;
  HIPCHK(c, hipSetDevice(c->device));
  int rc = prepare_host(c);
  if (rc != CVH_OK) return rc;
  return warm_impl(c, nsteps);
}

int sync_impl(cvh_context *c)
{
  const bool via_flush = c->chain_pending;
  int rc = chain_flush(c);
  if (rc != CVH_OK) return rc;
  if (c->timing_open) HIPCHK(c, hipEventRecord(c->ev1, c->stream));
  if (!via_flush) HIPCHK(c, hipMemcpyAsync(&c->h_state[0], c->d_state, sizeof(CvhState), hipMemcpyDeviceToHost, c->stream));
  if (c->resident_used) HIPCHK(c, hipMemcpyAsync(c->h_resident, c->d_resident, 4, hipMemcpyDeviceToHost, c->stream));
  HIPCHK(c, hipStreamSynchronize(c->stream));
  if (c->resident_used) {
    c->resident_used = false;
    if (c->h_resident[0]) {
      c->timing_open = false;
      return fail(c, CVH_ERR_HIP, "the resident step kernel gave up waiting for a workgroup: the level set of this run is invalid");
    }
  }
  if (via_flush) {
    c->h_state[0].steps_done = c->h_status[0];
    c->h_state[0].stopped = c->h_status[1];
    memcpy(&c->h_state[0].norm, &c->h_status[2], sizeof(double));
  }
  if (c->timing_open) {
    HIPCHK(c, hipEventElapsedTime(&c->last_run_ms, c->ev0, c->ev1));
    c->timing_open = false;
  }
  c->steps_done = c->h_state[0].steps_done;
  c->enqueued = c->steps_done;
  return CVH_OK;
}

extern "C" int cvh_sync(cvh_context *c, int *steps_done_total, double *last_norm, int *stopped)
{
  if (!c) return CVH_ERR_ARG;
  HIPCHK(c, hipSetDevice(c->device));
  const int rc = sync_impl(c);
  if (rc != CVH_OK) return rc;
  if (steps_done_total) *steps_done_total = c->h_state[0].steps_done;
  if (last_norm) *last_norm = c->h_state[0].norm;
  if (stopped) *stopped = c->h_state[0].stopped;
  return CVH_OK;
}

extern "C" int cvh_run(cvh_context *c, int max_steps, int *steps_done, double *last_norm)
{
  if (!c) return CVH_ERR_ARG;
  HIPCHK(c, hipSetDevice(c->device));
  if (!c->have_image) return fail(c, CVH_ERR_STATE, "no image set (call cvh_set_image first)");
  if (!c->have_u) return fail(c, CVH_ERR_STATE, "no level set (call cvh_set_levelset or cvh_init_checkerboard first)");
  int rc = reset_run_impl(c);
  if (rc != CVH_OK) return rc;
  long remaining = max_steps < 0 ? (long)INT_MAX : (long)max_steps;
  rc = prepare_host(c);
  if (rc != CVH_OK) return rc;
  rc = warm_impl(c, remaining < c->sync_every ? remaining : (long)c->sync_every);
  if (rc != CVH_OK) return rc;
  HIPCHK(c, hipEventRecord(c->ev0, c->stream));
  rc = prepare(c);
  if (rc != CVH_OK) return rc;
  constexpr int kAhead = 4;
  volatile int *hs = c->h_status;
  bool stopped = false;
  int queued = 0;
  int chunk_len = c->sync_every;
  c->run_chunk = (int)(remaining < 1024 ? remaining : 1024);
  { ResidentGeom rg; if (resident_geometry(c, &rg) && chunk_len < 1024) chunk_len = 1024; else c->run_chunk = chunk_len; }
  while (remaining > 0 && !stopped) {
    while (queued - hs[0] > kAhead * chunk_len && !hs[1]) {
      if (hipStreamQuery(c->stream) == hipSuccess) break;
    }
    if (hs[1]) { stopped = true; break; }
    const int chunk = (int)(remaining < chunk_len ? remaining : chunk_len);
    rc = enqueue_impl(c, chunk);
    if (rc != CVH_OK) return rc;
    remaining -= chunk;
    queued += chunk;
  }
  c->timing_open = true;
  rc = sync_impl(c);
  if (rc != CVH_OK) return rc;
  if (steps_done) *steps_done = c->h_state[0].steps_done;
  if (last_norm) *last_norm = c->h_state[0].norm;
  return CVH_OK;
}
```

chan_vese_amd/csrc/csv_wave2_body.inc:

```
  static_assert(C == 1 || FAST, "the 3-channel flavour exists in FAST arithmetic only (STRICT: kernel 2)");
  static_assert(!ST32 || FAST, "the declared FP32-state mode exists in FAST arithmetic only");
  using IO = StateIO<ST32, POL>;
  static_assert(FAST ? MINW == 3 : MINW == 2, "compiled for 3 waves per SIMD (FAST: branch-free rows) or 2 (STRICT)");
  using L = Wave2Smem<FAST, C>;
  constexpr int NS = cvh_nsums(C), R = R2;
  constexpr int NIQ = (9 * R * C + 63) / 64;
  extern __shared__ __attribute__((aligned(16))) double smem[];
  double *sred = smem + L::off_red;
  double *sfin = smem + L::off_fin;
  double *satan = smem + L::off_atan;
  double *slut = smem + L::off_lut;
  int *s_last = (int *)(smem + L::off_flag);
  constexpr unsigned kLutAddr = (unsigned)(L::off_lut * sizeof(double));
  if (!lds_base_is_zero(smem)) __builtin_trap();

  const int tid = threadIdx.x, lane = tid & 63;
  const int wave = __builtin_amdgcn_readfirstlane(tid >> 6);
  const bool chain = FAST && a.chain != nullptr;
  const int h = a.h, w = a.w;

  const int nwc = a.tiles_x, nstrips = a.tiles_y;
  const int nbc = (nwc + 1) >> 1;
  int bid = (int)blk;
  const bool bookkeeper = bid >= a.nparts;
  if (a.wave_xcd && !bookkeeper) {
    const int nb = a.nparts, x = bid & 7, j = bid >> 3, q = nb >> 3, r = nb & 7;
    if (a.wave_cls > 0) {
      const int S = a.wave_cls, cl = j / S;
      int rank = 0;
      for (int xx = 0; xx < 8; ++xx) {
        const int nx = q + (xx < r ? 1 : 0);
        const int before = nx < cl * S ? nx : cl * S;
        int mine = nx - cl * S;
        mine = mine < 0 ? 0 : (mine > S ? S : mine);
        rank += before + (xx < x ? mine : 0);
      }
      bid = rank + (j - cl * S);
    } else {
      bid = x * q + (x < r ? x : r) + j;
    }
  }
  const int wc = (bid % nbc) * 2 + (wave & 1);
  const int ws = (bid / nbc) * 2 + (wave >> 1);
  const bool active = !bookkeeper && wc < nwc && ws < nstrips;
  const int wsa = bookkeeper ? 0 : (bid / nbc) * 2;
  const const_int_p sb = (const_int_p)a.strip_bounds;
  const int stopped = *(const_int_p)&a.st->stopped;
  const int b0 = sb[wsa], b1 = sb[wsa + 1 <= nstrips ? wsa + 1 : nstrips], b2 = sb[wsa + 2 <= nstrips ? wsa + 2 : nstrips];
  if ((stopped != 0) | (b1 < b0) | (b2 < b1)) return;

  const unsigned long long t_start = a.dbg_times ? __builtin_amdgcn_s_memrealtime() : 0ull;
  double *xs = smem + L::off_x + wave * L::wave_doubles;
  if (tid == 0) *s_last = 0;

  double c1, c2;
  double cm1[C], cm2[C];
  long long chain_entry = 0;
  if (chain) chain_entry = a.chain->v[a.chain_phase][lane];
  else if (C == 1) { c1 = a.st->c1[0]; c2 = a.st->c2[0]; }
  else {
#pragma unroll
    for (int k = 0; k < C; ++k) { cm1[k] = a.st->c1[k]; cm2[k] = a.st->c2[k]; }
  }
  if (bookkeeper) { chain_bookkeeper_block<C>(a, chain_entry, sred); return; }
  const double l1 = a.lambda1[0], l2 = a.lambda2[0];
  const double eps = a.eps, eps2 = eps * eps;
  const FarCoef fc = {a.far_k[0], a.far_k[1], a.far_k[2], a.far_k[3], a.far_k[4], a.far_thr};

  auto fill_tables = [&]() {
    if (C == 1) {
      if (chain) { double m1[1], m2[1]; chain_means<1>(a, chain_entry, m1, m2); c1 = m1[0]; c2 = m2[0]; }
      if (FAST) {
        for (int q = tid; q < CVH_ATAN2_N; q += CVH_BLOCK) satan[q] = a.atan2_tab[q];
        const double v = (double)tid;
        const double d1 = v - c1, d2 = v - c2;
        const double reg = (d2 * d2) * l2 - (d1 * d1) * l1;
        slut[2 * tid] = __builtin_fma(reg, a.beta, a.gamma);
        slut[2 * tid + 1] = v;
      }
    } else {
      if (chain) chain_means<C>(a, chain_entry, cm1, cm2);
      for (int q = tid; q < CVH_ATAN2_N; q += CVH_BLOCK) satan[q] = a.atan2_tab[q];
      {
#pragma unroll
        for (int k = 0; k < C; ++k) {
          const double v = (double)tid;
          const double d1 = v - cm1[k], d2 = v - cm2[k];
          const double reg = (d2 * d2) * a.lambda2[k] - (d1 * d1) * a.lambda1[k];
          slut[2 * (k * 256 + tid)] = (k == 0) ? __builtin_fma(reg, a.beta, a.gamma) : reg * a.beta;
          slut[2 * (k * 256 + tid) + 1] = v;
        }
      }
    }
  };

  double acc[NS];
#pragma unroll
  for (int s = 0; s < NS; ++s) acc[s] = 0;

  int wg_groups = 0;
  {
    const int la = b1 - b0, lb = b2 - b1;
    wg_groups = ((la > lb ? la : lb) + R - 1) / R;
  }
  int groups_done = 0;

  if (active) {
    const int s0 = (wave >> 1) ? b1 : b0, s1 = (wave >> 1) ? b2 : b1;
    const int c0 = W2 * wc - 2 + 2 * lane;
    const bool lane_valid = lane >= 1 && c0 < w;
    const int cl = c0 < 0 ? 0 : (c0 > w - 2 ? w - 2 : c0);
    const double fxa = (c0 <= 0) ? 0.0 : 1.0;
    const int pa = 2 * lane;
    const int pw = (lane == 0 || c0 <= 0) ? pa : pa - 1;
    const int pe = (c0 + 2 >= w) ? pa + 1 : pa + 2;
    const double2_t *x_own = reinterpret_cast<const double2_t *>(xs + pa);
    const double *x_w = xs + pw, *x_e = xs + pe;
    double2_t *x_put = reinterpret_cast<double2_t *>(xs + pa);
    const bool xlane = lane < R;
    const int xrow = xlane ? lane : 0;
    const int xcol = clampi(W2 * wc + W2, 0, w - 1);
    double *x_ext = xlane ? xs + xrow * XP2 + 128 : xs + R * XP2 + lane;
    using raw2_t = typename IO::raw2_t;
    using raw1_t = typename IO::raw1_t;
    constexpr unsigned SB = IO::kBytes;
    const unsigned rowbytes = (unsigned)w * SB, ubytes = (unsigned)h * rowbytes;
    const unsigned voff_u = (unsigned)cl * SB;
    const unsigned voff_st = lane_valid ? (unsigned)c0 * SB : kOobOffset;
    const unsigned voff_x = ((unsigned)xrow * (unsigned)w + (unsigned)xcol) * SB;
    const __amdgpu_buffer_rsrc_t ru = make_rsrc(a.u_in, ubytes);
    const int ulast = s1 < h - 1 ? s1 : h - 1, ilast = s1 - 1;
    auto U = [&](int r) -> raw2_t { return IO::load2(ru, voff_u, (unsigned)clampi(r, 0, ulast) * rowbytes); };
    auto UX = [&](int r0) -> raw1_t {
      if (r0 + R - 1 <= ulast) return IO::load1(ru, voff_x, (unsigned)r0 * rowbytes);
      return IO::load1(ru, ((unsigned)clampi(r0 + xrow, 0, ulast) * (unsigned)w + (unsigned)xcol) * SB, 0u);
    };
    unsigned char *simg = reinterpret_cast<unsigned char *>(xs + R * XP2 + 64);
    const int icol0 = (W2 * wc - 2) & ~15;
    const int ipiece = lane % 9, irow = lane / 9;
    const bool ilane = lane < 9 * R;
    int ipc = icol0 + 16 * ipiece;
    ipc = ipc < 0 ? 0 : (ipc > w - 16 ? w - 16 : ipc);
    const unsigned voff_i = (unsigned)(ilane ? irow : 0) * (unsigned)w + (unsigned)ipc;
    unsigned char *ipiece_dst = simg + irow * IMGP2 + ((icol0 + 16 * ipiece) == ipc ? 16 * ipiece : ipc - icol0);
    const int ibyte = cl - icol0;
    const __amdgpu_buffer_rsrc_t ri = make_rsrc(a.img[0], (unsigned)(C - 1) * a.img_stride + (unsigned)h * (unsigned)w);
    auto IMQ = [&](int r0) -> u32x4_t {
      if (r0 + R - 1 <= ilast) return buf_load_b128(ri, voff_i, (unsigned)r0 * (unsigned)w);
      return buf_load_b128(ri, (unsigned)clampi(r0 + (ilane ? irow : 0), 0, ilast) * (unsigned)w + (unsigned)ipc, 0u);
    };
    bool q_on[NIQ];
    int q_row[NIQ];
    unsigned q_voff[NIQ], q_voff_cl[NIQ];
    unsigned char *q_dst[NIQ];
#pragma unroll
    for (int j = 0; j < NIQ; ++j) {
      const int q = 64 * j + lane, qc = q < 9 * R * C ? q : 0;
      const int ch = qc / (9 * R), il = qc % (9 * R), pr = il / 9, pp = il % 9;
      int pcq = icol0 + 16 * pp;
      pcq = pcq < 0 ? 0 : (pcq > w - 16 ? w - 16 : pcq);
      q_on[j] = q < 9 * R * C;
      q_row[j] = pr;
      q_voff_cl[j] = (unsigned)ch * a.img_stride + (unsigned)pcq;
      q_voff[j] = q_voff_cl[j] + (unsigned)pr * (unsigned)w;
      q_dst[j] = simg + (ch * R + pr) * IMGP2 + ((icol0 + 16 * pp) == pcq ? 16 * pp : pcq - icol0);
    }
    auto IMQ3 = [&](int r0, int j) -> u32x4_t {
      if (r0 + R - 1 <= ilast) return buf_load_b128(ri, q_voff[j], (unsigned)r0 * (unsigned)w);
      return buf_load_b128(ri, q_voff_cl[j] + (unsigned)clampi(r0 + q_row[j], 0, ilast) * (unsigned)w, 0u);
    };
    auto lds_fence = [&]() {
      __builtin_amdgcn_fence(__ATOMIC_RELEASE, "wavefront");
      __builtin_amdgcn_wave_barrier();
      __builtin_amdgcn_fence(__ATOMIC_ACQUIRE, "wavefront");
    };
    int im[R];
    auto park = [&](const raw2_t (&T)[R], raw1_t X, const u32x4_t (&IQ)[NIQ]) {
      lds_fence();
#pragma unroll
      for (int j = 0; j < R; ++j) x_put[j * (XP2 / 2)] = IO::widen(T[j]);
      *x_ext = IO::widen(X);
      if (C == 1) {
        if (ilane) *reinterpret_cast<u32x4_t *>(ipiece_dst) = IQ[0];
      } else {
#pragma unroll
        for (int j = 0; j < NIQ; ++j) if (q_on[j]) *reinterpret_cast<u32x4_t *>(q_dst[j]) = IQ[j];
      }
      lds_fence();
      if (C == 1) {
#pragma unroll
        for (int k = 0; k < R; ++k) im[k] = (int)*reinterpret_cast<const unsigned short *>(simg + k * IMGP2 + ibyte);
      }
    };
    auto samples = [&](int ch, int k) -> int { return (int)*reinterpret_cast<const unsigned short *>(simg + (ch * R + k) * IMGP2 + ibyte); };

    const double2_t um2 = IO::widen(U(s0 - 2));
    double2_t um = IO::widen(U(s0 - 1)), u0 = IO::widen(U(s0));
    double uw, ue;
    {
      raw2_t T[R];
#pragma unroll
      for (int j = 0; j < R; ++j) T[j] = U(s0 + 1 + j);
      const double X0 = IO::widen(UX(s0));
      const raw1_t X = UX(s0 + 1);
      u32x4_t IQ[NIQ];
      if (C == 1) IQ[0] = IMQ(s0);
      else {
#pragma unroll
        for (int j = 0; j < NIQ; ++j) IQ[j] = IMQ3(s0, j);
      }
      fill_tables();
      __syncthreads();
      x_put[0] = u0;
      if (xrow == 0) *x_ext = X0;
      lds_fence();
      uw = x_w[0]; ue = x_e[0];
      park(T, X, IQ);
    }
    auto norm = [&](double fwd, double bwd, double c) -> double {
      return FAST ? normalised4(fwd, bwd, c + c) : normalised<false>(fwd - c, central(bwd, fwd));
    };
    double nypa = norm(u0.x, um2.x, um.x), nypb = norm(u0.y, um2.y, um.y);
    if (s0 == 0) {
      const double2_t up0 = x_own[0];
      nypa = norm(up0.x, um.x, u0.x); nypb = norm(up0.y, um.y, u0.y);
    }

    auto pixel = [&](double c, double n_, double s_, double nx, double nxl, double fx, double &nyp, int byte,
                     double &ud_out, double &Ik_out) -> double {
      const double ny = norm(s_, n_, c);
      double kappa, ud, Ik;
      if (FAST) {
        kappa = __builtin_fma(nx - nxl, fx, ny - nyp);
        const double2_t e = lds_read_d2(kLutAddr + (unsigned)byte);
        Ik = e.y;
        ud = __builtin_fma(kappa, a.alpha, e.x);
        ud = ud * rcp_refined(inv_delta_eps(c, eps2, a.dk1));
      } else {
        const double kx = (fx == 0.0) ? 0.0 : nx - nxl;
        const double ky = ny - nyp;
        kappa = kx + ky;
        Ik = (double)byte;
        const double d1 = Ik - c1, d2 = Ik - c2;
        const double vin = (d1 * d1) * l1, vout = (d2 * d2) * l2;
        ud = 0.0;
        ud += vout - vin;
        ud = kappa * a.alpha + ud * a.beta + a.gamma;
        ud = ud * (eps / (kPi * (eps2 + c * c)));
      }
      nyp = ny;
      ud_out = ud; Ik_out = Ik;
      return c + ud;
    };

    auto pixel3 = [&](double c, double n_, double s_, double nx, double nxl, double fx, double &nyp, const int (&byte)[C],
                      double &ud_out, double (&Ik)[C]) -> double {
      const double ny = norm(s_, n_, c);
      const double kappa = __builtin_fma(nx - nxl, fx, ny - nyp);
      double reg;
      {
        const double2_t e0 = lds_read_d2(kLutAddr + (unsigned)byte[0]);
        reg = e0.x; Ik[0] = e0.y;
#pragma unroll
        for (int ch = 1; ch < C; ++ch) {
          const double2_t e = lds_read_d2(kLutAddr + (unsigned)(ch * 4096) + (unsigned)byte[ch]);
          reg += e.x; Ik[ch] = e.y;
        }
      }
      double ud = __builtin_fma(kappa, a.alpha, reg);
      const double qd = __builtin_fma(c, c, eps2) * a.dk1;
      const double r0 = __builtin_amdgcn_rcp(qd);
      const double er = __builtin_fma(-qd, r0, 1.0);
      ud = ud * __builtin_fma(__builtin_fma(er, er, er), r0, r0);
      nyp = ny;
      ud_out = ud;
      return c + ud;
    };

    constexpr bool DEFER = FAST;
    double2_t keep[R];
    unsigned long long near_mask[R];
    int smp3[C][R];
    auto row = [&](int i, int k, bool live, auto near_tag) {
      constexpr bool NEARFORM = decltype(near_tag)::value;
      const double2_t up = x_own[k * (XP2 / 2)];
      const double uw_n = x_w[k * XP2], ue_n = x_e[k * XP2];
      int sa[C], sb[C];
      if (C == 1) {
        if (FAST) { sa[0] = (int)byte_x16<0>((unsigned)im[k]); sb[0] = (int)byte_x16<1>((unsigned)im[k]); }
        else { sa[0] = im[k] & 0xff; sb[0] = (im[k] >> 8) & 0xff; }
      } else {
#pragma unroll
        for (int ch = 0; ch < C; ++ch) { const unsigned s = (unsigned)samples(ch, k); sa[ch] = (int)byte_x16<0>(s); sb[ch] = (int)byte_x16<1>(s); }
      }
      const int ba = sa[0], bb = sb[0];
      const double nxa = norm(u0.y, uw, u0.x);
      const double nxb = norm(ue, u0.x, u0.y);
      const double nxla = dpp_from_left(nxb);
      double uda, udb, Ia, Ib, nya = nypa, nyb = nypb;
      double Ika[C], Ikb[C];
      double va, vb;
      if (C == 1) {
        va = pixel(u0.x, um.x, up.x, nxa, nxla, fxa, nya, ba, uda, Ia);
        vb = pixel(u0.y, um.y, up.y, nxb, nxa, 1.0, nyb, bb, udb, Ib);
      } else {
        va = pixel3(u0.x, um.x, up.x, nxa, nxla, fxa, nya, sa, uda, Ika);
        vb = pixel3(u0.y, um.y, up.y, nxb, nxa, 1.0, nyb, sb, udb, Ikb);
      }
      double hva, hvb;
      if (ST32) { va = IO::stored(va); vb = IO::stored(vb); }
      keep[k] = double2_t{va, vb};
      if (FAST && DEFER && NEARFORM) {
        hva = 0.0; hvb = 0.0;
        near_mask[k] = 0ull;
      } else if (FAST && DEFER) {
        hva = heaviside_centred_far(va, fc); hvb = heaviside_centred_far(vb, fc);
        near_mask[k] = __builtin_amdgcn_ballot_w64(fabs(va) < fc.thr || fabs(vb) < fc.thr);
      } else {
        hva = heaviside_strict(va, eps); hvb = heaviside_strict(vb, eps);
      }
      IO::store2(keep[k], make_rsrc(a.u_out, live ? ubytes : 0u), voff_st, (unsigned)i * rowbytes);
      if (live) {
        if (FAST && DEFER && NEARFORM) {
          acc[2 + 2 * C] = __builtin_fma(uda, uda, acc[2 + 2 * C]); acc[2 + 2 * C] = __builtin_fma(udb, udb, acc[2 + 2 * C]);
        } else if (FAST && C == 1) {
          acc[0] += hva; acc[0] += hvb;
          acc[2] = __builtin_fma(Ia, hva, acc[2]); acc[2] = __builtin_fma(Ib, hvb, acc[2]);
          acc[4] = __builtin_fma(uda, uda, acc[4]); acc[4] = __builtin_fma(udb, udb, acc[4]);
        } else if (FAST) {
          acc[0] += hva; acc[0] += hvb;
#pragma unroll
          for (int ch = 0; ch < C; ++ch) {
            acc[2 + ch] = __builtin_fma(Ika[ch], hva, acc[2 + ch]); acc[2 + ch] = __builtin_fma(Ikb[ch], hvb, acc[2 + ch]);
          }
          acc[2 + 2 * C] = __builtin_fma(uda, uda, acc[2 + 2 * C]); acc[2 + 2 * C] = __builtin_fma(udb, udb, acc[2 + 2 * C]);
        } else {
          acc[0] += hva; acc[1] += (1 - hva); acc[2] += Ia * hva; acc[3] += Ia * (1 - hva); acc[4] += uda * uda;
          acc[0] += hvb; acc[1] += (1 - hvb); acc[2] += Ib * hvb; acc[3] += Ib * (1 - hvb); acc[4] += udb * udb;
        }
        nypa = nya; nypb = nyb;
      }
      um = u0; u0 = up;
      uw = uw_n; ue = ue_n;
    };

    int prio = 3;
    if (a.wave_prio) __builtin_amdgcn_s_setprio(3);
    const bool skip_dead_prefetch = FAST && a.wave_seam != 0;
    auto group = [&](int ib, auto interior_tag, auto near_tag) {
      constexpr bool INTERIOR = decltype(interior_tag)::value;
      constexpr bool NEARFORM = decltype(near_tag)::value;
      const bool last = !INTERIOR && skip_dead_prefetch && ib + R >= s1;
      if (a.wave_sync) { __builtin_amdgcn_s_barrier(); ++groups_done; }
      if (a.wave_prio) {
        const int rem = s1 - ib, len = s1 - s0;
        int pq;
        if (a.wave_prio == 1) pq = (rem * 4 - 1) / len;
        else {
          const int sh = a.wave_prio == 4 ? 1 : a.wave_prio;
          pq = (rem << (4 - sh)) > len ? 3 : ((rem << (5 - sh)) > len ? 2 : ((rem << (6 - sh)) > len ? 1 : 0));
        }
        if (pq != prio) {
          prio = pq;
          if (pq >= 3) __builtin_amdgcn_s_setprio(3);
          else if (pq == 2) __builtin_amdgcn_s_setprio(2);
          else if (pq == 1) __builtin_amdgcn_s_setprio(1);
          else __builtin_amdgcn_s_setprio(0);
        }
      }
      raw2_t T[R];
      raw1_t X;
      u32x4_t IQ[NIQ];
      if (!last) {
#pragma unroll
        for (int j = 0; j < R; ++j) T[j] = INTERIOR ? IO::load2(ru, voff_u, (unsigned)(ib + R + 1 + j) * rowbytes) : U(ib + R + 1 + j);
        X = INTERIOR ? IO::load1(ru, voff_x, (unsigned)(ib + R + 1) * rowbytes) : UX(ib + R + 1);
        if (C == 1) IQ[0] = INTERIOR ? buf_load_b128(ri, voff_i, (unsigned)(ib + R) * (unsigned)w) : IMQ(ib + R);
        else {
#pragma unroll
          for (int j = 0; j < NIQ; ++j) IQ[j] = INTERIOR ? buf_load_b128(ri, q_voff[j], (unsigned)(ib + R) * (unsigned)w) : IMQ3(ib + R, j);
        }
      }
#pragma unroll
      for (int k = 0; k < R; ++k) {
        if (INTERIOR || (ib + k) < s1) row(ib + k, k, true, near_tag);
        else near_mask[k] = 0ull;
      }
      const bool any_near = DEFER && !NEARFORM && (near_mask[0] | near_mask[1] | near_mask[2] | near_mask[3]) != 0ull;
      auto finish_row = [&](int k, int smp0, auto table_tag) {
        constexpr bool TABLE = decltype(table_tag)::value;
        const double xa = keep[k].x, xb = keep[k].y;
        double da, db;
        if (TABLE) {
          da = heaviside_centred_near(xa, a.inv_eps, satan); db = heaviside_centred_near(xb, a.inv_eps, satan);
        } else {
          da = (fabs(xa) < fc.thr) ? heaviside_centred_near(xa, a.inv_eps, satan) - heaviside_centred_far(xa, fc) : 0.0;
          db = (fabs(xb) < fc.thr) ? heaviside_centred_near(xb, a.inv_eps, satan) - heaviside_centred_far(xb, fc) : 0.0;
        }
        acc[0] += da; acc[0] += db;
        if (C == 1) {
          acc[2] = __builtin_fma((double)(smp0 & 0xff), da, acc[2]);
          acc[2] = __builtin_fma((double)((smp0 >> 8) & 0xff), db, acc[2]);
        } else {
#pragma unroll
          for (int ch = 0; ch < C; ++ch) {
            const int s = TABLE ? smp3[ch][k] : samples(ch, k);
            acc[2 + ch] = __builtin_fma((double)(s & 0xff), da, acc[2 + ch]);
            acc[2 + ch] = __builtin_fma((double)(s >> 8), db, acc[2 + ch]);
          }
        }
      };
      if (DEFER && !NEARFORM && any_near) {
#pragma unroll
        for (int k = 0; k < R; ++k)
          if (near_mask[k] != 0ull && (INTERIOR || (ib + k) < s1)) finish_row(k, im[k], std::false_type{});
      }
      if (DEFER && NEARFORM) {
        int smp1[R];
#pragma unroll
        for (int k = 0; k < R; ++k) {
          smp1[k] = (C == 1) ? im[k] : 0;
          if (C > 1) {
#pragma unroll
            for (int ch = 0; ch < C; ++ch) smp3[ch][k] = samples(ch, k);
          }
        }
        if (!last) park(T, X, IQ);
#pragma unroll
        for (int k = 0; k < R; ++k)
          if (INTERIOR || (ib + k) < s1) finish_row(k, smp1[k], std::true_type{});
#pragma unroll
        for (int k = 0; k < R; ++k) asm volatile("; row %2 of the group: store data still live" :: "v"(keep[k].x), "v"(keep[k].y), "n"(0));
      } else {
#pragma unroll
        for (int k = 0; k < R; ++k) asm volatile("; row %2 of the group: store data still live" :: "v"(keep[k].x), "v"(keep[k].y), "n"(0));
        if (!last) park(T, X, IQ);
      }
    };
    const unsigned long long t_first = a.dbg_times ? __builtin_amdgcn_s_memrealtime() : 0ull;
    if (a.dbg_times && lane == 0) a.dbg_times[(size_t)(blk * 4 + wave) * 4 + 2] = t_first;
    int ib = s0;
    const bool near_strip = DEFER && a.near_switch &&
        __builtin_popcountll(__builtin_amdgcn_ballot_w64(lane_valid && (fabs(u0.x) < fc.thr || fabs(u0.y) < fc.thr))) >= 32;
    if (__builtin_expect(DEFER && near_strip, 0)) {
      for (; ib + 2 * R <= ulast; ib += R) group(ib, std::true_type{}, std::true_type{});
      for (; ib < s1; ib += R) group(ib, std::false_type{}, std::true_type{});
    } else {
      for (; ib + 2 * R <= ulast; ib += R) group(ib, std::true_type{}, std::false_type{});
      for (; ib < s1; ib += R) group(ib, std::false_type{}, std::false_type{});
    }
    const double vmask = lane_valid ? 1.0 : 0.0;
#pragma unroll
    for (int s = 0; s < NS; ++s) acc[s] = acc[s] * vmask;
  } else {
    fill_tables();
    __syncthreads();
  }
  if (a.wave_sync) {
    for (; groups_done < wg_groups; ++groups_done) __builtin_amdgcn_s_barrier();
  }
  if (a.dbg_times && lane == 0) {
    unsigned long long *d = a.dbg_times + (size_t)(blk * 4 + wave) * 4;
    d[0] = t_start;
    d[1] = __builtin_amdgcn_s_memrealtime();
    unsigned hwid, xcc;
    asm volatile("s_getreg_b32 %0, hwreg(HW_REG_HW_ID)" : "=s"(hwid));
    asm volatile("s_getreg_b32 %0, hwreg(HW_REG_XCC_ID)" : "=s"(xcc));
    d[3] = (unsigned long long)xcc | ((unsigned long long)hwid << 8) | ((unsigned long long)(unsigned)bid << 40);
  }
  const double total = block_reduce<NS>(acc, sred);
  if (chain) {
    chain_publish<C>(a, total, blk);
  } else {
    publish_partials_and_maybe_finalize<C>(a, total, sred, sfin, s_last, a.nparts, blk);
  }
  if (a.dbg_times && tid == 0) a.dbg_times[(size_t)a.nparts * 16 + blk] = __builtin_amdgcn_s_memrealtime();
```

chan_vese_amd/csrc/csv_wave2_kernel.hip:

```cpp
#include "csv_device.h"
#include "buffer_ops.h"
#include "wave_math.h"
#include "chain_device.h"
#include "wave2_device.h"
#include <type_traits>

using namespace cvh_dev;

namespace {

template <int C, bool FAST, int MINW, int POL, bool ST32>
__global__ __launch_bounds__(CVH_BLOCK, MINW) void csv_wave2_kernel(const CvhStepArgs a)
{
  const unsigned blk = blockIdx.x;
#include "csv_wave2_body.inc"
}

template <int C, bool FAST, int MINW, int POL, bool ST32>
__global__ __launch_bounds__(CVH_BLOCK, MINW) void csv_wave2_batch_kernel(const CvhBatchArgs b)
{
  unsigned blk;
  const CvhStepArgs *const ap = batch_member(b, &blk);
  if (!ap) return;
  const CvhStepArgs &a = *ap;
#include "csv_wave2_body.inc"
}

template <int C, bool FAST, int MINW, int POL, bool ST32 = false>
hipError_t launch_wave2(const CvhStepArgs &a, hipStream_t s, const CvhBatchLaunch *batch)
{
  using L = Wave2Smem<FAST, C>;
  static_assert(L::bytes <= 64 * 1024, "dynamic LDS above 64 KiB would need hipFuncSetAttribute");
  static_assert(MINW * L::bytes <= 160 * 1024, "the kernel is compiled for MINW workgroups per CU: their LDS must fit the CU's 160 KiB");
  const int extra = (FAST && a.chain) ? 1 : 0;
  CVH_LAUNCH_B((csv_wave2_kernel<C, FAST, MINW, POL, ST32>), (csv_wave2_batch_kernel<C, FAST, MINW, POL, ST32>), a.nparts + extra, L::bytes, s, a, batch,
               "csv_wave2_kernel<%d, %s, %d, %d, %s>", C, CVH_TF(FAST), MINW, POL, CVH_TF(ST32));
  return hipGetLastError();
}

}

int cvh_wave2_cols() { return W2; }

hipError_t cvh_launch_wave2(const CvhStepArgs &a, int channels, int fast, hipStream_t s, const CvhBatchLaunch *batch)
{
  if (a.state32) {
    if (channels == 3) return a.wave_pol ? launch_wave2<3, true, 3, 1, true>(a, s, batch) : launch_wave2<3, true, 3, 0, true>(a, s, batch);
    return a.wave_pol ? launch_wave2<1, true, 3, 1, true>(a, s, batch) : launch_wave2<1, true, 3, 0, true>(a, s, batch);
  }
  if (channels == 3) return a.wave_pol ? launch_wave2<3, true, 3, 1>(a, s, batch) : launch_wave2<3, true, 3, 0>(a, s, batch);
  if (!fast) return launch_wave2<1, false, 2, 1>(a, s, batch);
  if (a.wave_pol == 2) return launch_wave2<1, true, 3, 2>(a, s, batch);
  return a.wave_pol ? launch_wave2<1, true, 3, 1>(a, s, batch) : launch_wave2<1, true, 3, 0>(a, s, batch);
}
```

chan_vese_amd/csrc/cvh_host.h:

```cpp
#pragma once
#include <limits.h>
#include <math.h>
#include <stdarg.h>
#include <stdio.h>
#include <stdlib.h>
#include <string.h>

#include <algorithm>
#include <atomic>
#include <functional>
#include <mutex>
#include <string>
#include <vector>

#include "cvh_internal.h"

struct DeviceTable { void *d = nullptr; size_t cap = 0, count = 0; };

constexpr int kGraphSteps = 16;
struct StepGraph { hipGraphExec_t exec = nullptr; CvhStepArgs key[4]; int kind = -1, flavour = -1; };
struct BatchCache;

struct cvh_context {
  int h = 0, w = 0, C = 0, device = 0;
  size_t n = 0;
  int num_cus = 256;
  hipStream_t stream = nullptr;
  uint8_t *d_img[CVH_MAX_CHANNELS] = {nullptr, nullptr, nullptr};
  uint8_t *d_img_slab = nullptr;
  size_t img_stride = 0;
  double *d_u[2] = {nullptr, nullptr};
  void *d_u_slab = nullptr;
  float *d_uf[2] = {nullptr, nullptr};
  void *d_uf_slab = nullptr;
  CvhState *d_state = nullptr;
  CvhState *h_state = nullptr;
  int *h_status = nullptr;
  double *d_partials = nullptr;
  int partial_rows = 0;
  double *d_trace = nullptr;
  int trace_cap = 0;
  double *d_pm[2] = {nullptr, nullptr};
  int pm_plane = -1;
  uint8_t *d_mask = nullptr;
  double *d_dummy = nullptr;
  double *d_atan = nullptr;
  CvhChainAcc *d_chain = nullptr;
  int *d_bounds = nullptr;
  unsigned long long *d_isums = nullptr, *h_isums = nullptr;
  unsigned long long *d_dbg = nullptr;
  size_t dbg_words = 0;
  CvhResident *d_resident = nullptr;
  double *d_res_halo = nullptr;
  double *d_pm_halo = nullptr;
  int *h_resident = nullptr;
  unsigned pm_res_serial = 0;
  char err[512] = {0};
  bool have_image = false, have_u = false, stop_valid = false;
  bool sums_valid = false;
  double sum_img[CVH_MAX_CHANNELS] = {0, 0, 0};
  double stop_norm = 0.0;
  bool mirror_valid = true;
  int cur_base = 0;
  int enqueued = 0;
  int steps_done = 0;
  int chain_pb = 0;
  bool chain_pending = false;
  bool chain_acc_valid = false;
  int pending_nparts = 0;
  int last_nparts = 0;
  bool resident_used = false;
  bool timing_open = false;
  mutable int run_pol = -1;
  mutable int run_alone = -1;
  int run_chunk = -1;
  int geom_cus = 0;
  double stop_cond_h = 0.0;
  float last_run_ms = 0.f, last_pm_ms = 0.f;
  float last_reinit_ms = 0.f;
  cvh_params p{};
  int state_bits = 64;
  int co_resident = 1;
  int math_mode = CVH_MATH_DEFAULT, finalize_mode = 0, sync_every = 32;
  int tile_rows = 0 , use_lut = 1, use_dma = 0;
  int kernel = -1;
  int pm_kernel = -1;
  int pm_strip_rows = 0;
  int wave_minw = 5, wave_lds_cap = 0, wave_prio = 1, wave_sync = -1 , wave_imgv = 1, wave_depth = 4;
  int res_prio = 1;
  int res_go_share = 5;
  int wave_seam = 1;
  int near_switch = 1;
  int wave_rev = 0, wave_xcd = 1;
  int use_graph = 1;
  int wave_skew = 0;
  int chain_opt = 1;
  int res_straight = 1;
  int resident_opt = -1;
  int far_terms = 5;
  int wave_pol = -1;
  int wave_cls = 1;
  int wave_cskew = 500;
  int strip_rows = 0;
  int strips = 0;
  StepGraph graphs[4];
  char pm_desc[256] = {0};
  hipGraphExec_t pm_graph = nullptr;
  CvhPmArgs pm_graph_key{};
  int pm_graph_kind = -1;
  int bounds_key[4] = {-1, -1, -1, -1};
  int tiles_x = 0, tiles_y = 0;
  BatchCache *batch = nullptr;
  DeviceTable pm_batch;
  DeviceTable io_table;
  void *h_io = nullptr;
  size_t h_io_cap = 0;
  hipEvent_t ev_io_in = nullptr, ev_io_out = nullptr;
  void *d_reinit = nullptr;
  void *d_cc = nullptr;
  DeviceTable cc_table;
  DeviceTable regions;
  void *d_contour = nullptr;
  DeviceTable contour_edges;
  DeviceTable contour_points;
  unsigned *d_hist = nullptr;
  void *d_energy = nullptr;
  void *d_score = nullptr;
  void *d_morph = nullptr;
  void *d_local = nullptr;
  void *d_rank = nullptr;
  DeviceTable overlap;
  void *d_overlap_plane = nullptr;
  int coop_launch = -1;
  int resident_cap = -1;
  int pm_resident_cap = -1;
  hipEvent_t ev0 = nullptr, ev1 = nullptr, evp[4] = {nullptr, nullptr, nullptr, nullptr};
  hipEvent_t ev_join = nullptr;
};

struct Geometry { int strip; int rows; int tiles_x, tiles_y, strip_rows, nblocks; };
struct ResidentGeom { int tr, tc, band; };

constexpr int kPmMaxPerLaunch = 1 << 16;
constexpr int kPmPollCap = 2000000;

#define HIPCHK(ctx, call)                                                                      \
  do {                                                                                         \
    hipError_t e_ = (call);                                                                    \
    if (e_ != hipSuccess)                                                                      \
      return fail((ctx), CVH_ERR_HIP, "HIP error %d (%s) in %s", (int)e_, hipGetErrorString(e_), \
                  #call);                                                                      \
  } while (0)

#pragma GCC visibility push(hidden)
inline bool use_fast(const cvh_context *c)
{
  const int m = c->math_mode == CVH_MATH_DEFAULT ? CVH_MATH_FAST : c->math_mode;
  return m == CVH_MATH_FAST;
}

inline int current_buffer(const cvh_context *c) { return (c->cur_base + c->steps_done) & 1; }

constexpr size_t kErrLen = 512;
char *create_err();
int fail(cvh_context *ctx, int code, const char *fmt, ...);

bool run_is_alone(const cvh_context *c);
double live_footprint(const cvh_context *c);
int image_stats(cvh_context *c, const uint8_t *const *host_planes);
double stop_norm_host(const std::vector<const uint8_t *> &planes, size_t n);
void fill_atan_tables(double *tab);

int settle(cvh_context *c);
int reset_run_impl(cvh_context *c);
int levelset_arrived(cvh_context *c, bool device_cleared = false);
void steps_enqueued(cvh_context *c, int n, int nparts, bool chain, bool resident);
void sums_taken(cvh_context *c, bool chain);
bool stop_norm_exact_on_device(const cvh_context *c);
void planes_changed(cvh_context *c);
void plane_sums_arrived(cvh_context *c, const unsigned long long *isums, const double *host_norm);
int adopt_f32_state(cvh_context *c);
int ensure_f64_mirror(cvh_context *c);

Geometry resolve_geometry(const cvh_context *c);
bool use_chain(const cvh_context *c, const Geometry &g);
bool launches_cooperatively(cvh_context *c);
bool resident_geometry(cvh_context *c, ResidentGeom *rg);
bool resident_tile_grid(int h, int w, int channels, int num_cus, int cap_blocks, ResidentGeom *rg);
void fill_args(const cvh_context *c, CvhStepArgs *a, int in_buf, int step);
void far_coef(double eps, int far_terms, double k[5], double *thr);
int prepare_host(cvh_context *c);
int prepare(cvh_context *c);
void compute_strip_bounds(int kind, int h, int tiles_x, int S, int strip_rows, int nblocks, int cls, int cskew, int skew, std::vector<int> &b);
int upload_strip_bounds(cvh_context *c, const Geometry &g);
int launch_one_step(cvh_context *c, int in_buf, int step, bool capturing = false, CvhLaunchNote *note = nullptr);
int flush_for_grid(cvh_context *c, int nparts);
int ensure_resident_buffers(cvh_context *c);
int launch_resident(cvh_context *c, const ResidentGeom &rg, int nsteps, CvhLaunchNote *note);
int sync_impl(cvh_context *c);

void batch_cache_free(cvh_context *c);
int batch_fail(cvh_context *const *ctxs, int n, int code, const char *fmt, ...);
enum MemberNeeds { kMembersListed, kMembersWithImage, kMembersForCsv };
int members_check(cvh_context *const *ctxs, int n, const char *what, MemberNeeds needs);
int members_below(cvh_context *const *ctxs, int n, const char *what, int k, int only = -1);
int members_distances_fit(cvh_context *const *ctxs, int n, const char *what, int only = -1);
template <class T>
int members_caps_fit(cvh_context *const *ctxs, int n, const char *what, const void *const *lists, const T *caps, const char *noun, const char *without,
                     int only = -1);
int members_have_images(cvh_context *const *ctxs, int n, const char *what);
int members_have_levelsets(cvh_context *const *ctxs, int n, const char *what, int only = -1);
int members_mirrors_fresh(cvh_context *const *ctxs, int n, const char *what, int first = 0, const char *noun = "member");
struct PairRoles { cvh_context *const *first, *const *second; const char *first_name, *second_name, *first_role, *second_role; bool second_is_dst; };
int pairs_check(const PairRoles &p, int n, const char *what, std::vector<cvh_context *> *all, const std::function<int(int)> &rule,
                const std::function<int()> &args = nullptr);
int pair_sources_have_images(cvh_context *const *all, int n, const char *what, const char *role);
int join_into_leader(cvh_context *const *ctxs, int n, const int *member = nullptr);
int grow_table(cvh_context *c, DeviceTable *t, size_t bytes);
int grow_table_to(cvh_context *c, DeviceTable *t, size_t want, size_t count, size_t bytes);
void free_table(DeviceTable *t);

enum LaunchCounter { kReinitLaunchSets, kPyramidLaunches, kColourLaunches, kEnergyLaunchSets, kScoreLaunchSets, kMorphLaunchSets, kOverlapLaunchSets, kLocalLaunchSets, kRankLaunchSets, kLaunchCounters };
extern std::atomic<unsigned long> g_launches[kLaunchCounters];

int pointer_check(cvh_context *const *ctxs, int n, int i, const void *p, const char *what);
int element_pointer_check(cvh_context *const *ctxs, int n, int i, const void *p, size_t size, const char *what);
int settle_all(cvh_context *const *ctxs, int n, const char *what);
int open_call(cvh_context *const *ctxs, int n, void *stream);
int close_call(cvh_context *const *ctxs, int n, void *stream, bool to_caller);
unsigned lay_out(CvhIoMember *tab, int n);
int mask_out(cvh_context *const *ctxs, int n, uint8_t *const *d_masks, int invert, void *stream, const char *what);
void checkerboard_factors(int h, int w, double *out);
void levelset_target(const cvh_context *c, CvhIoMember *m);
int ensure_workspace(cvh_context *c, void **slot, size_t bytes, const char *name, bool mirror = true);

struct MemberCall;
struct MaskSource {
  int conn = 4, invert = 0;
  long min_area = 0, fill_holes = 0;
  int keep_largest = 0;

  bool drop() const { return min_area > 1; }
  bool cleaned() const { return drop() || fill_holes || keep_largest; }
  int check(cvh_context *const *ctxs, int n, const char *what) const;
  int ready(cvh_context *const *ctxs, int n, const char *what, bool need_cc) const;
  void fill(MemberCall *call, int i, void *dst, unsigned long long *sums, bool need_cc) const;
  int launch(const MemberCall &call, bool raw_too) const;
};

inline size_t align_up(size_t v, size_t a) { return (v + a - 1) & ~(a - 1); }

struct MemberCall {
  cvh_context *const *ctxs = nullptr;
  int n = 0;
  const char *what = nullptr;
  cvh_context *lead = nullptr;
  unsigned char *hb = nullptr, *db = nullptr;
  CvhIoMember *tab = nullptr, *tab2 = nullptr;
  size_t extra_off = 0, host_off = 0, dev_bytes = 0;
  unsigned grid = 0, grid2 = 0;

  int begin(cvh_context *const *ctxs_, int n_, const char *what_, size_t extra_dev = 0, size_t extra_host = 0, bool two_tables = false);
  const CvhIoMember *dtab() const { return (const CvhIoMember *)db; }
  const CvhIoMember *dtab2() const { return (const CvhIoMember *)(db + ((unsigned char *)tab2 - hb)); }
  int arrived(const int *which = nullptr) const;
  int upload_again(const CvhIoMember *t) const;
  int wait_again(void *stream, bool to_caller) const;

  template <class F>
  int run(void *stream, bool to_caller, bool wait, F launches, hipEvent_t first = nullptr)
  {
    grid = lay_out(tab, n);
    if (tab2) grid2 = lay_out(tab2, n);
    int rc = open_call(ctxs, n, stream);
    if (rc != CVH_OK) return rc;
    if (first) HIPCHK(lead, hipEventRecord(first, lead->stream));
    HIPCHK(lead, hipMemcpyAsync(db, hb, dev_bytes, hipMemcpyHostToDevice, lead->stream));
    rc = launches();
    if (rc != CVH_OK) return rc;
    rc = close_call(ctxs, n, stream, to_caller);
    if (rc != CVH_OK) return rc;
    if (wait) HIPCHK(lead, hipStreamSynchronize(lead->stream));
    return CVH_OK;
  }
};

struct PlaneSums {
  cvh_context *const *ctxs = nullptr;
  int n = 0;
  size_t sums_bytes = 0, fetch_bytes = 0;
  std::vector<int> on_host;
  std::vector<size_t> fetch_off;

  void plan(cvh_context *const *ctxs_, int n_);
  unsigned long long *device_sums(const MemberCall &call, int i) const { return (unsigned long long *)(call.db + call.extra_off) + (size_t)8 * i; }
  int fetch(const MemberCall &call);
  void arrive(const MemberCall &call);
};
int write_planes(cvh_context *const *ctxs, int n_written, int n_members, const char *what, void *stream,
                 const std::function<void(int, CvhIoMember &)> &fill, const std::function<int(const MemberCall &)> &launch);

template <class F>
int mask_to_host(cvh_context *c, uint8_t *mask, F into_d_mask)
{
  HIPCHK(c, hipSetDevice(c->device));
  if (!c->d_mask) HIPCHK(c, hipMalloc((void **)&c->d_mask, c->n));
  const int rc = into_d_mask();
  if (rc != CVH_OK) return rc;
  HIPCHK(c, hipMemcpyAsync(mask, c->d_mask, c->n, hipMemcpyDeviceToHost, c->stream));
  HIPCHK(c, hipStreamSynchronize(c->stream));
  return CVH_OK;
}

template <class F>
int guarded(cvh_context *const *ctxs, int n, const char *what, F body)
{
  try { return body(); }
  catch (...) { return batch_fail(ctxs, n, CVH_ERR_NOMEM, "%s: out of host memory", what); }
}

template <class F>
int guarded_one(cvh_context *c, const char *what, F body)
{
  return c ? guarded(&c, 1, what, [&]() { return body(what); }) : CVH_ERR_ARG;
}

template <class F>
int capture_graph(cvh_context *c, hipGraphExec_t *out, F launches, const char *end_fmt)
{
  HIPCHK(c, hipStreamBeginCapture(c->stream, hipStreamCaptureModeThreadLocal));
  const int rc = launches();
  hipGraph_t graph = nullptr;
  const hipError_t e_end = hipStreamEndCapture(c->stream, &graph);
  if (rc != CVH_OK || e_end != hipSuccess || !graph) {
    if (graph) (void)hipGraphDestroy(graph);
    return rc != CVH_OK ? rc : fail(c, CVH_ERR_HIP, end_fmt, hipGetErrorString(e_end));
  }
  const hipError_t e_inst = hipGraphInstantiate(out, graph, nullptr, nullptr, 0);
  (void)hipGraphDestroy(graph);
  if (e_inst != hipSuccess) { *out = nullptr; return fail(c, CVH_ERR_HIP, "hipGraphInstantiate: %s", hipGetErrorString(e_inst)); }
  return CVH_OK;
}
#pragma GCC visibility pop
```

chan_vese_amd/csrc/cvh_internal.h:

```cpp
#pragma once

#include <hip/hip_runtime.h>
#include <stddef.h>
#include <stdint.h>

#include "chanvese_hip.h"

#define CVH_BLOCK 256


struct CvhState {
  double c1[CVH_MAX_CHANNELS];
  double c2[CVH_MAX_CHANNELS];
  double norm;
  double stop_cond;
  int steps_done;
  int stopped;
  unsigned ticket;
  int pending;
};

constexpr int CVH_CHAIN_SETS = 4;
struct CvhChainAcc { long long v[CVH_CHAIN_SETS][64]; };

constexpr int CVH_RESIDENT_MAX_TILES = 256;
struct CvhResident {
  int error;
  unsigned pad[15];
  unsigned flag[CVH_RESIDENT_MAX_TILES * 16];
  unsigned go[CVH_RESIDENT_MAX_TILES * 16];
  unsigned hflag[CVH_RESIDENT_MAX_TILES * 16];
  unsigned flag_c3[CVH_RESIDENT_MAX_TILES * 4];
  unsigned go_c3[CVH_RESIDENT_MAX_TILES * 32];
};
constexpr size_t CVH_RESIDENT_C1_BYTES = offsetof(CvhResident, flag_c3);

__host__ __device__ constexpr int cvh_nsums(int C) { return 3 + 2 * C; }

struct CvhLaunchNote { char name[112]; unsigned grid, block, lds; };
void cvh_fill_note(CvhLaunchNote *note, unsigned grid, unsigned block, size_t lds, const char *fmt, ...);

struct CvhStepArgs {
  const double *u_in;
  double *u_out;
  const uint8_t *img[CVH_MAX_CHANNELS];
  unsigned img_stride;
  CvhState *st;
  double *partials;
  double *trace;
  int trace_cap;
  int h, w;
  int tiles_x, tiles_y;
  int nparts;
  int fused_finalize;
  double alpha, beta, gamma;
  double eps;
  double lambda1[CVH_MAX_CHANNELS], lambda2[CVH_MAX_CHANNELS];
  const double *atan_tab;
  double inv_eps;
  double dk1, dk2;
  double npix;
  double sum_img[CVH_MAX_CHANNELS];
  double stop_cond;
  double far_k[5], far_thr;
  int derive_complement;
  int tile_rows;
  int use_lut;
  int use_dma;
  int strip_rows;
  const double *atan2_tab;
  int wave_minw;
  unsigned long long *dbg_times;
  int *host_status;
  double *dummy;
  int wave_imgv;
  int wave_xcd;
  int wave_rev;
  const int *strip_bounds;
  int wave_depth;
  int wave_sync;
  int wave_prio;
  int state32;
  int near_switch;
  int wave_lds_cap;
  CvhChainAcc *chain;
  int chain_phase;
  int chain_pb;
  double chain_scale[4], chain_inv[4];
  double *chain_s4;
  int wave_pol;
  int wave_cls;
  int wave_seam;
  CvhLaunchNote *note;
  CvhResident *resident;
  double *res_halo;
  int res_steps, res_poll_cap;
  int res_t0;
  int res_prio;
  int res_band_rows;
  int res_go_shift;
};

struct CvhBatchEntry { unsigned member, first, nblk, pad; };
struct CvhBatchArgs { const CvhBatchEntry *map; const CvhStepArgs *args; };
struct CvhBatchLaunch { CvhBatchArgs k; unsigned grid; };

#define CVH_LAUNCH(KERNEL, GRID, LDS, S, A, ...)                                                  \
  do {                                                                                             \
    if ((A).note) cvh_fill_note((A).note, (unsigned)(GRID), CVH_BLOCK, (size_t)(LDS), __VA_ARGS__); \
    else hipLaunchKernelGGL(KERNEL, dim3(GRID), dim3(CVH_BLOCK), (LDS), (S), (A));                 \
  } while (0)
#define CVH_LAUNCH_B(KERNEL, BKERNEL, GRID, LDS, S, A, B, ...)                                   \
  do {                                                                                             \
    if ((A).note) cvh_fill_note((A).note, (unsigned)(GRID), CVH_BLOCK, (size_t)(LDS), __VA_ARGS__); \
    else if (B) hipLaunchKernelGGL(BKERNEL, dim3((B)->grid), dim3(CVH_BLOCK), (LDS), (S), (B)->k);   \
    else hipLaunchKernelGGL(KERNEL, dim3(GRID), dim3(CVH_BLOCK), (LDS), (S), (A));                 \
  } while (0)
#define CVH_TF(b) ((b) ? "true" : "false")

#define CVH_ATAN_N 129
#define CVH_ATAN2_N 257

struct CvhPmArgs {
  const double *in;
  double *out;
  int h, w;
  int tiles_x, tiles_y;
  double K2;
  double L;
  double invK2, L4;
  int fast;
  int strip_rows;
  int pol;
  CvhResident *resident;
  double *res_halo;
  unsigned res_serial;
  int res_steps;
  int res_band_rows;
  int res_prio;
  int res_poll_cap;
  unsigned long long *dbg_times;
  CvhLaunchNote *note;
};

struct CvhPmBatchPlane { CvhPmArgs a; int tile_base, pad; };
struct CvhPmBatchArgs { const CvhPmBatchPlane *planes; const unsigned *map; int ntiles, nplanes; };
struct CvhPmIoPlane { uint8_t *img; double *state; unsigned long long n; };

struct CvhIoMember {
  const void *src;
  const void *src2;
  void *dst;
  uint8_t *plane[CVH_MAX_CHANNELS];
  unsigned long long *sums;
  int *state_zero;
  long long *chain_zero;
  unsigned long long n;
  int h, w, C;
  int interleaved;
  unsigned first, nblk;
  int h2, w2;
  unsigned long long src_stride;
};

unsigned cvh_io_blocks(size_t n);
unsigned cvh_io_checkerboard_blocks(int h, int w);
hipError_t cvh_launch_io_ingest(const CvhIoMember *tab, int nmem, unsigned grid, hipStream_t s);
hipError_t cvh_launch_image_sums(const uint8_t *const *planes, int channels, size_t n, unsigned long long *out ,
                                 hipStream_t s);
hipError_t cvh_launch_io_checkerboard(const CvhIoMember *tab, int nmem, unsigned grid, hipStream_t s);
hipError_t cvh_launch_io_mask(const CvhIoMember *tab, int nmem, unsigned grid, int invert, hipStream_t s);
hipError_t cvh_launch_io_image_out3(const CvhIoMember *tab, int nmem, unsigned grid, hipStream_t s);
hipError_t cvh_launch_io_narrow(const double *u, float *out, size_t n, hipStream_t s);
#define CVH_REINIT_BAND 32
#define CVH_REINIT_LDS_COLS 8192
unsigned cvh_reinit_column_blocks(int h, int w);
unsigned cvh_reinit_row_blocks(int h);
size_t cvh_reinit_bits_bytes(int h, int w);
size_t cvh_reinit_workspace_bytes(int h, int w);
hipError_t cvh_launch_reinit(const CvhIoMember *cols, unsigned col_grid, const CvhIoMember *rows, unsigned row_grid, int nmem, int max_w,
                             hipStream_t s);
unsigned cvh_cc_blocks(size_t n);
size_t cvh_cc_workspace_bytes(size_t n);
hipError_t cvh_launch_cc_label(const CvhIoMember *tab, int nmem, unsigned grid, int conn, int invert, bool any_labels, hipStream_t s);
hipError_t cvh_launch_cc_table(const CvhIoMember *tab, int nmem, unsigned grid, hipStream_t s);
hipError_t cvh_launch_cc_clean(const CvhIoMember *tab, int nmem, unsigned grid, int conn, int invert, unsigned min_area, long fill_holes,
                               int keep_largest, hipStream_t s);
hipError_t cvh_launch_cc_number(const CvhIoMember *tab, int nmem, unsigned grid, int mode, int conn, int invert, hipStream_t s);
#define CVH_MEASURE_TILE 8192
unsigned cvh_measure_blocks(size_t n);
hipError_t cvh_launch_measure(const CvhIoMember *tab, int nmem, unsigned grid, bool any_c1, bool any_c3, hipStream_t s);
struct CvhOverlapSlot { unsigned long long key; unsigned count, pad; };
#define CVH_OVERLAP_CTL 4
hipError_t cvh_launch_overlap(const CvhIoMember *tab, int nmem, unsigned grid, bool any_rows, hipStream_t s);
unsigned cvh_contour_scan_trip();
unsigned cvh_contour_edge_blocks(size_t edges, size_t n);
size_t cvh_contour_bits_offset(size_t n);
size_t cvh_contour_prefix_offset(size_t n);
size_t cvh_contour_counts_offset(size_t n);
size_t cvh_contour_pixel_bytes(size_t n);
size_t cvh_contour_edge_bytes(size_t cap);
size_t cvh_contour_rows_offset(size_t cap);
hipError_t cvh_launch_contours_count(const CvhIoMember *tab, int nmem, unsigned grid, hipStream_t s);
hipError_t cvh_launch_contours_trace(const CvhIoMember *tab, int nmem, unsigned grid, int conn, int simplify, int rounds, bool any_points,
                                     hipStream_t s);
#define CVH_HIST_MAX_BINS (255 * CVH_MAX_CHANNELS + 1)
enum { CVH_START_THRESHOLD = 0, CVH_START_RECT = 1, CVH_START_DISK = 2 };
struct CvhInitStart { double inside, outside; long long a, b, c, d; int mode, pad; };
unsigned cvh_init_start_blocks(size_t n);
hipError_t cvh_launch_init_histogram(const CvhIoMember *tab, int nmem, unsigned grid, hipStream_t s);
hipError_t cvh_launch_init_start(const CvhIoMember *tab, const CvhInitStart *par, int nmem, unsigned grid, hipStream_t s);
size_t cvh_restrict_items(int fine_h, int fine_w);
size_t cvh_prolong_items(int fine_h, int fine_w);
unsigned cvh_restrict_blocks(int fine_h, int fine_w);
unsigned cvh_prolong_blocks(int fine_h, int fine_w);
hipError_t cvh_launch_restrict(const CvhIoMember *tab, int nmem, unsigned grid, hipStream_t s);
hipError_t cvh_launch_prolong(const CvhIoMember *tab, int nmem, unsigned grid, hipStream_t s);
#define CVH_COLOUR_BLOCK_PIXELS (16 * CVH_BLOCK)
unsigned cvh_colour_blocks(size_t n);
hipError_t cvh_launch_colour_convert(const CvhIoMember *tab, int nmem, unsigned grid, int space, int order, int inverse, hipStream_t s);
hipError_t cvh_launch_colour_luma(const CvhIoMember *tab, int nmem, unsigned grid, int order, hipStream_t s);
#define CVH_WINDOW_SEGMENT 1024
#define CVH_WINDOW_BAND 32
#define CVH_WINDOW_STRIP 256
#define CVH_LOCAL_SEGMENT CVH_WINDOW_SEGMENT
#define CVH_LOCAL_BAND CVH_WINDOW_BAND
#define CVH_RANK_SEGMENT CVH_LOCAL_SEGMENT
#define CVH_RANK_BAND CVH_LOCAL_BAND
__host__ __device__ constexpr size_t cvh_window_pitch(int w) { return ((size_t)w + 3) & ~(size_t)3; }
__host__ __device__ constexpr size_t cvh_local_slot_bytes(int h, int w) { return (6 * (size_t)h * cvh_window_pitch(w) + 15) & ~(size_t)15; }
unsigned cvh_local_blocks(int h, int w, int planes_read);
hipError_t cvh_launch_local(const CvhIoMember *tab, int nmem, unsigned grid, unsigned passes, hipStream_t s);
#define CVH_RANK_MEDIAN_BAND 32
#define CVH_RANK_MEDIAN_STRIP 64
#define CVH_RANK_SLOTS 7
#define CVH_RANK_PASS_ROWS 1u
#define CVH_RANK_PASS_TWICE 2u
#define CVH_RANK_PASS_MEDIAN 4u
__host__ __device__ constexpr size_t cvh_rank_slot_bytes(int h, int w) { return ((size_t)h * cvh_window_pitch(w) + 255) & ~(size_t)255; }
unsigned cvh_rank_blocks(int h, int w, int R, int row_jobs, int median_planes);
hipError_t cvh_launch_rank(const CvhIoMember *tab, int nmem, unsigned grid, unsigned passes, hipStream_t s);
#define CVH_ENERGY_BAND 32
#define CVH_ENERGY_COLS 128
#define CVH_ENERGY_SLOTS (2 + 2 * CVH_MAX_CHANNELS)
#define CVH_ENERGY_ROW 16
__host__ __device__ constexpr unsigned cvh_energy_items(int h, int w)
{
  return (((unsigned)h + CVH_ENERGY_BAND - 1) / CVH_ENERGY_BAND) * (((unsigned)w + CVH_ENERGY_COLS - 1) / CVH_ENERGY_COLS);
}
unsigned cvh_energy_blocks(int h, int w);
hipError_t cvh_launch_energy(const CvhIoMember *tab, int nmem, unsigned grid, hipStream_t s);
#define CVH_SCORE_ROW 16
enum { CVH_SCORE_TP, CVH_SCORE_FP, CVH_SCORE_FN, CVH_SCORE_TN, CVH_SCORE_SURF_M, CVH_SCORE_SURF_T, CVH_SCORE_WITHIN_M, CVH_SCORE_WITHIN_T,
       CVH_SCORE_DIST_M, CVH_SCORE_DIST_T, CVH_SCORE_HD2_M, CVH_SCORE_HD2_T };
__host__ __device__ constexpr size_t cvh_score_words_bytes(int h, int w)
{
  return ((size_t)((h + CVH_REINIT_BAND - 1) / CVH_REINIT_BAND) * (size_t)w * sizeof(unsigned) + 255) & ~(size_t)255;
}
inline size_t cvh_score_truth_offset(int h, int w) { return 4 * cvh_score_words_bytes(h, w) + (size_t)h * (size_t)w * sizeof(unsigned); }
inline size_t cvh_score_workspace_bytes(int h, int w) { return cvh_score_truth_offset(h, w) + (size_t)h * (size_t)w; }
hipError_t cvh_launch_score(const CvhIoMember *cols, unsigned col_grid, const CvhIoMember *rows, unsigned row_grid, int nmem, int max_w,
                            int invert, unsigned tol2, hipStream_t s);
struct CvhMorphPar { double inside, outside; unsigned r2, root, pad[2]; };
inline size_t cvh_morph_dist_offset(int h, int w) { return 2 * cvh_score_words_bytes(h, w); }
inline size_t cvh_morph_bytes_offset(int h, int w) { return cvh_morph_dist_offset(h, w) + (((size_t)h * (size_t)w * sizeof(unsigned short) + 255) & ~(size_t)255); }
inline size_t cvh_morph_workspace_bytes(int h, int w) { return cvh_morph_bytes_offset(h, w) + (size_t)h * (size_t)w; }
hipError_t cvh_launch_morph_bits(const CvhIoMember *cols, int nmem, unsigned col_grid, bool from_levelset, int invert, hipStream_t s);
hipError_t cvh_launch_morph_passes(const CvhIoMember *cols, const CvhMorphPar *par, int nmem, unsigned col_grid, int npass, const bool *complement,
                                   hipStream_t s);
hipError_t cvh_launch_morph_emit(const CvhIoMember *tab, const CvhMorphPar *par, int nmem, unsigned grid, bool from_bytes, bool to_levelset,
                                 hipStream_t s);
void cvh_step_grid(int h, int w, int tile_rows, int *tiles_x, int *tiles_y);
int cvh_step_max_blocks(int h, int w);
hipError_t cvh_launch_step(const CvhStepArgs &a, int channels, int fast, hipStream_t s);
int cvh_wave2_cols();
hipError_t cvh_launch_wave2(const CvhStepArgs &a, int channels, int fast, hipStream_t s, const CvhBatchLaunch *batch = nullptr);
hipError_t cvh_launch_chain_flush(const CvhStepArgs &a, int channels, hipStream_t s);
size_t cvh_pm_resident_lds_bytes();
int cvh_pm_resident_halo_doubles();
int cvh_pm_resident_blocks_per_cu();
hipError_t cvh_launch_pm_resident(const CvhPmArgs &a, hipStream_t s);
int cvh_pm_resident_batch_blocks_per_cu();
hipError_t cvh_launch_pm_resident_batch(const CvhPmBatchArgs &b, int fast, int nr, hipStream_t s, CvhLaunchNote *note = nullptr);
hipError_t cvh_launch_pm_load_batch(const CvhPmIoPlane *planes, int nplanes, size_t nmax, hipStream_t s);
hipError_t cvh_launch_pm_store_batch(const CvhPmIoPlane *planes, int nplanes, size_t nmax, hipStream_t s);
size_t cvh_resident_lds_bytes(int channels);
int cvh_resident_tile_w();
int cvh_resident_tile_hmax(int channels);
int cvh_resident_halo_doubles();
int cvh_resident_blocks_per_cu(int channels);
hipError_t cvh_launch_resident(const CvhStepArgs &a, int channels, hipStream_t s);
hipError_t cvh_launch_wave(const CvhStepArgs &a, int channels, int fast, hipStream_t s, const CvhBatchLaunch *batch = nullptr);
int cvh_wave_cols();
hipError_t cvh_launch_init_sums(const CvhStepArgs &a, int channels, int fast, int *nparts_out,
                                hipStream_t s);
hipError_t cvh_launch_finalize(const CvhStepArgs &a, int channels, int is_init, hipStream_t s);
int cvh_init_sum_blocks(int h, int w);

hipError_t cvh_launch_pm_load(const uint8_t *plane, double *state, size_t n, hipStream_t s);
hipError_t cvh_launch_pm_step(const CvhPmArgs &a, hipStream_t s);
hipError_t cvh_launch_pm_wave(const CvhPmArgs &a, hipStream_t s);
int cvh_pm_wave_k2_cols();
hipError_t cvh_launch_pm_wave_k2(const CvhPmArgs &a, hipStream_t s);
int cvh_pm_wave_cols();
hipError_t cvh_launch_pm_store(const double *state, uint8_t *plane, size_t n, hipStream_t s);
void cvh_pm_grid(int h, int w, int *tiles_x, int *tiles_y);

hipError_t cvh_launch_contour(const double *u, uint8_t *out, int h, int w, hipStream_t s);
hipError_t cvh_launch_state_narrow(double *u, float *uf, size_t n, hipStream_t s);
hipError_t cvh_launch_state_widen(const float *uf, double *u, size_t n, hipStream_t s);
hipError_t cvh_launch_ppf(double *data, size_t n, int op, double eps, hipStream_t s);
hipError_t cvh_launch_separate(const uint8_t *img3, const double *u, uint8_t *sel3, size_t n,
                               int invert, hipStream_t s);
```

chan_vese_amd/csrc/debug_exports.hip:

```cpp
#include "cvh_host.h"
#include "wave_math.h"
#include "local_math.h"
#include "rank_math.h"

extern "C" int cvh_debug_strip_bounds(int kind, int h, int tiles_x, int S, int strip_rows, int nblocks, int cls, int cskew, int skew, int *out)
{
  if (!out || S < 1 || h < 1 || (kind != 2 && kind != 3)) return CVH_ERR_ARG;
  std::vector<int> b;
  compute_strip_bounds(kind, h, tiles_x, S, strip_rows, nblocks, cls, cskew, skew, b);
  memcpy(out, b.data(), b.size() * sizeof(int));
  return CVH_OK;
}

extern "C" int cvh_debug_data_flow(int h, int w, int channels, int math_mode, int kernel, int state_bits, int num_cus, int *flow, int *tiles_x,
                                   int *tiles_y, int *strip_rows)
{
  if (h < 1 || w < 1 || (channels != 1 && channels != 3) || !flow) return CVH_ERR_ARG;
  cvh_context c;
  c.h = h; c.w = w; c.C = channels; c.n = (size_t)h * (size_t)w;
  c.math_mode = math_mode; c.kernel = kernel; c.state_bits = state_bits; c.num_cus = num_cus > 0 ? num_cus : 256;
  const Geometry g = resolve_geometry(&c);
  *flow = g.strip;
  if (tiles_x) *tiles_x = g.tiles_x;
  if (tiles_y) *tiles_y = g.tiles_y;
  if (strip_rows) *strip_rows = g.strip_rows;
  return CVH_OK;
}

enum {
  TRIPS_IO = 0,
  TRIPS_START,
  TRIPS_RESTRICT,
  TRIPS_PROLONG,
  TRIPS_ENERGY_TERMS,
  TRIPS_ENERGY_REDUCE,
  TRIPS_ROWS,
  TRIPS_COLUMNS,
  TRIPS_NOPS,
  TRIPS_MORPH_EMIT = 16,
  TRIPS_END
};

extern "C" int cvh_debug_trip_counts(int op, int h, int w, unsigned long long *items, unsigned *nblk, unsigned *takers)
{
  if (op < 0 || (op >= TRIPS_NOPS && op < TRIPS_MORPH_EMIT) || op >= TRIPS_END || h < 1 || w < 1 || !items || !nblk || !takers) return CVH_ERR_ARG;
  const size_t n = (size_t)h * (size_t)w;
  const unsigned bands = ((unsigned)h + CVH_REINIT_BAND - 1) / CVH_REINIT_BAND, chunks = ((unsigned)w + CVH_BLOCK - 1) / CVH_BLOCK;
  switch (op) {
    case TRIPS_IO: *items = n / 16; *nblk = cvh_io_blocks(n); *takers = CVH_BLOCK; break;
    case TRIPS_START: *items = n / 2; *nblk = cvh_init_start_blocks(n); *takers = CVH_BLOCK; break;
    case TRIPS_RESTRICT: *items = cvh_restrict_items(h, w); *nblk = cvh_restrict_blocks(h, w); *takers = CVH_BLOCK; break;
    case TRIPS_PROLONG: *items = cvh_prolong_items(h, w); *nblk = cvh_prolong_blocks(h, w); *takers = CVH_BLOCK; break;
    case TRIPS_ENERGY_TERMS: *items = cvh_energy_items(h, w); *nblk = cvh_energy_blocks(h, w); *takers = CVH_BLOCK / 64; break;
    case TRIPS_ENERGY_REDUCE: *items = cvh_energy_items(h, w); *nblk = 1; *takers = CVH_BLOCK; break;
    case TRIPS_ROWS: *items = (unsigned long long)h; *nblk = cvh_reinit_row_blocks(h); *takers = 1; break;
    case TRIPS_COLUMNS: *items = (unsigned long long)bands * chunks; *nblk = cvh_reinit_column_blocks(h, w); *takers = 1; break;
    case TRIPS_MORPH_EMIT: *items = n / 16; *nblk = cvh_io_blocks(n); *takers = CVH_BLOCK; break;
  }
  return CVH_OK;
}

extern "C" int cvh_debug_contour_trips(int h, int w, unsigned long long edges, unsigned *pixel_blocks, unsigned *scan_trip, unsigned *edge_blocks,
                                       unsigned long long *edge_lanes)
{
  if (h < 1 || w < 1 || !pixel_blocks || !scan_trip || !edge_blocks || !edge_lanes) return CVH_ERR_ARG;
  *pixel_blocks = cvh_cc_blocks((size_t)h * (size_t)w);
  *scan_trip = cvh_contour_scan_trip();
  *edge_blocks = cvh_contour_edge_blocks((size_t)edges, (size_t)h * (size_t)w);
  *edge_lanes = (unsigned long long)*edge_blocks * CVH_BLOCK;
  return CVH_OK;
}

extern "C" int cvh_debug_resident_grid(int h, int w, int channels, int num_cus, int *tiles_x, int *tiles_y, int *tile_rows)
{
  if (h < 1 || w < 1 || num_cus < 1) return 0;
  ResidentGeom rg;
  if (!resident_tile_grid(h, w, channels, num_cus, num_cus, &rg)) return 0;
  if (tiles_x) *tiles_x = rg.tc;
  if (tiles_y) *tiles_y = rg.tr;
  if (tile_rows) *tile_rows = (h + rg.tr - 1) / rg.tr;
  return 1;
}

extern "C" int cvh_debug_resident_read(cvh_context *c, unsigned *out, int ngo)
{
  if (!c || !out || ngo < 0 || ngo > CVH_RESIDENT_MAX_TILES) return CVH_ERR_ARG;
  if (!c->d_resident) return fail(c, CVH_ERR_STATE, "no resident launch yet");
  HIPCHK(c, hipSetDevice(c->device));
  HIPCHK(c, hipStreamSynchronize(c->stream));
  std::vector<unsigned> tmp(sizeof(CvhResident) / sizeof(unsigned));
  HIPCHK(c, hipMemcpy(tmp.data(), c->d_resident, sizeof(CvhResident), hipMemcpyDeviceToHost));
  out[0] = tmp[0]; out[1] = tmp[1] | (tmp[2] << 12) | (tmp[3] << 24);
  for (int i = 0; i < ngo; ++i) { out[2 + i] = tmp[16 + (size_t)i * 16]; out[2 + ngo + i] = tmp[16 + (size_t)CVH_RESIDENT_MAX_TILES * 16 + (size_t)i * 16]; }
  return CVH_OK;
}

extern "C" int cvh_debug_pm_plane(cvh_context *c, double *out)
{
  if (!c || !out) return CVH_ERR_ARG;
  if (c->pm_plane < 0 || c->pm_plane > 1 || !c->d_pm[c->pm_plane])
    return fail(c, CVH_ERR_STATE, "cvh_debug_pm_plane: no Perona-Malik call has left a plane on this context");
  HIPCHK(c, hipSetDevice(c->device));
  HIPCHK(c, hipStreamSynchronize(c->stream));
  HIPCHK(c, hipMemcpy(out, c->d_pm[c->pm_plane], c->n * sizeof(double), hipMemcpyDeviceToHost));
  return CVH_OK;
}

extern "C" int cvh_debug_num_cus(cvh_context *c, int *out)
{
  if (!c || !out) return CVH_ERR_ARG;
  *out = c->num_cus;
  return CVH_OK;
}

extern "C" unsigned long cvh_debug_reinit_launch_sets(void) { return g_launches[kReinitLaunchSets].load(); }
extern "C" unsigned long cvh_debug_pyramid_launches(void) { return g_launches[kPyramidLaunches].load(); }
extern "C" unsigned long cvh_debug_colour_launches(void) { return g_launches[kColourLaunches].load(); }
extern "C" int cvh_debug_colour_block_pixels(void) { return CVH_COLOUR_BLOCK_PIXELS; }
extern "C" unsigned long cvh_debug_local_launch_sets(void) { return g_launches[kLocalLaunchSets].load(); }
extern "C" void cvh_debug_local_geometry(int *out) { out[0] = CVH_WINDOW_BAND; out[1] = CVH_WINDOW_STRIP; out[2] = CVH_WINDOW_SEGMENT; }
extern "C" unsigned cvh_debug_local_isqrt(unsigned q) { return cvh_local_isqrt(q); }
extern "C" void cvh_debug_local_stats(unsigned n, unsigned S, unsigned Q, unsigned *mean, unsigned *dev)
{
  *mean = cvh_local_mean(n, S);
  *dev = cvh_local_dev(n, S, Q);
}
extern "C" unsigned long cvh_debug_rank_launch_sets(void) { return g_launches[kRankLaunchSets].load(); }
extern "C" void cvh_debug_rank_geometry(int *out)
{
  out[0] = CVH_WINDOW_BAND; out[1] = CVH_WINDOW_STRIP; out[2] = CVH_WINDOW_SEGMENT; out[3] = CVH_RANK_MEDIAN_BAND; out[4] = CVH_RANK_MEDIAN_STRIP;
}
extern "C" int cvh_debug_rank_chain(int code) { return cvh_rank_chain(code); }
extern "C" int cvh_debug_rank_twice(int code) { return cvh_rank_twice(code); }
extern "C" int cvh_debug_rank_band_rows(int R) { return cvh_rank_band_rows(R, CVH_WINDOW_BAND); }
extern "C" unsigned cvh_debug_rank_median_index(unsigned n) { return cvh_rank_median_index(n); }
extern "C" int cvh_debug_rank_walk(const unsigned *words, unsigned *before, unsigned t) { return cvh_rank_walk(words, before, t); }
extern "C" unsigned long cvh_debug_energy_launch_sets(void) { return g_launches[kEnergyLaunchSets].load(); }
extern "C" unsigned long cvh_debug_score_launch_sets(void) { return g_launches[kScoreLaunchSets].load(); }
extern "C" unsigned long cvh_debug_morph_launch_sets(void) { return g_launches[kMorphLaunchSets].load(); }
extern "C" unsigned long cvh_debug_overlap_launch_sets(void) { return g_launches[kOverlapLaunchSets].load(); }

extern "C" int cvh_debug_last_reinit_ms(cvh_context *c, float *ms)
{
  if (!c || !ms) return CVH_ERR_ARG;
  *ms = c->last_reinit_ms;
  return CVH_OK;
}

extern "C" int cvh_debug_read(cvh_context *c, unsigned long long *out, long max_words, long *words, int *nblocks)
{
  if (!c || !out || !words) return CVH_ERR_ARG;
  HIPCHK(c, hipSetDevice(c->device));
  HIPCHK(c, hipStreamSynchronize(c->stream));
  long n = (long)c->dbg_words < max_words ? (long)c->dbg_words : max_words;
  *words = n;
  if (nblocks) *nblocks = c->last_nparts > 0 ? c->last_nparts : resolve_geometry(c).nblocks;
  if (n > 0 && c->d_dbg) HIPCHK(c, hipMemcpy(out, c->d_dbg, (size_t)n * 8, hipMemcpyDeviceToHost));
  return CVH_OK;
}

enum {
  MATH_H_FAR = 0,
  MATH_H_NEAR,
  MATH_H_FAST,
  MATH_H_STRICT,
  MATH_ATAN_TABLE,
  MATH_INV_DELTA,
  MATH_DELTA,
  MATH_INV_DELTA_TILE,
  MATH_DELTA_TILE,
  MATH_RCP,
  MATH_RSQRT,
  MATH_NORMALISED,
  MATH_NORMALISED4,
  MATH_NOPS
};

extern "C" int cvh_debug_csv_math_arity(int op)
{
  return op < 0 || op >= MATH_NOPS ? 0 : op == MATH_NORMALISED ? 2 : op == MATH_NORMALISED4 ? 3 : 1;
}

namespace {
constexpr int kMathTab = 2 * CVH_ATAN_N + CVH_ATAN2_N;

__global__ void __launch_bounds__(256) csv_math_kernel(int op, int n, const double *x, double eps, double inv_eps, double dk1, double dk2,
                                                       cvh_dev::FarCoef fc, const double *tab, double *out)
{
  using namespace cvh_dev;
  __shared__ double stab[kMathTab];
  for (int q = threadIdx.x; q < kMathTab; q += blockDim.x) stab[q] = tab[q];
  __syncthreads();
  const int i = blockIdx.x * blockDim.x + threadIdx.x;
  if (i >= n) return;
  const double v = x[i];
  const double *satan2 = stab + 2 * CVH_ATAN_N;
  double r = 0.0;
  switch (op) {
    case MATH_H_FAR: r = heaviside_centred_far(v, fc); break;
    case MATH_H_NEAR: r = heaviside_centred_near(v, inv_eps, satan2); break;
    case MATH_H_FAST: r = heaviside_centred_far(v, fc) + near_field_correction(v, inv_eps, satan2, fc); break;
    case MATH_H_STRICT: r = heaviside_strict(v, eps); break;
    case MATH_ATAN_TABLE: r = atan_table(v, stab); break;
    case MATH_INV_DELTA: r = inv_delta_eps(v, eps * eps, dk1); break;
    case MATH_DELTA: r = rcp_refined(inv_delta_eps(v, eps * eps, dk1)); break;
    case MATH_INV_DELTA_TILE: r = inv_delta_eps_tile(v, dk1, dk2); break;
    case MATH_DELTA_TILE: r = rcp_refined(inv_delta_eps_tile(v, dk1, dk2)); break;
    case MATH_RCP: r = rcp_refined(v); break;
    case MATH_RSQRT: r = rsqrt_refined(v); break;
    case MATH_NORMALISED: r = normalised<true>(v, x[(size_t)n + i]); break;
    case MATH_NORMALISED4: r = normalised4(v, x[(size_t)n + i], x[2 * (size_t)n + i]); break;
  }
  out[i] = r;
}
}

extern "C" int cvh_debug_csv_math(int op, int n, const double *x, double eps, double *out)
{
  const int arity = cvh_debug_csv_math_arity(op);
  if (!arity || n < 1 || !x || !out || !(eps > 0)) return CVH_ERR_ARG;
  double tab[kMathTab];
  fill_atan_tables(tab);
  cvh_dev::FarCoef fc;
  {
    double k[5];
    far_coef(eps, 5, k, &fc.thr);
    fc.k0 = k[0]; fc.k1 = k[1]; fc.k2 = k[2]; fc.k3 = k[3]; fc.k4 = k[4];
  }
  const double pi = 3.14159265358979323846;
  double *d_x = nullptr, *d_out = nullptr, *d_tab = nullptr;
  const size_t xbytes = (size_t)arity * (size_t)n * sizeof(double), obytes = (size_t)n * sizeof(double);
  hipError_t e = hipMalloc((void **)&d_x, xbytes);
  if (e == hipSuccess) e = hipMalloc((void **)&d_out, obytes);
  if (e == hipSuccess) e = hipMalloc((void **)&d_tab, sizeof(tab));
  if (e == hipSuccess) e = hipMemcpy(d_x, x, xbytes, hipMemcpyHostToDevice);
  if (e == hipSuccess) e = hipMemcpy(d_tab, tab, sizeof(tab), hipMemcpyHostToDevice);
  if (e == hipSuccess) {
    hipLaunchKernelGGL(csv_math_kernel, dim3((n + 255) / 256), dim3(256), 0, 0, op, n, d_x, eps, 1.0 / eps, pi / eps, pi * eps, fc, d_tab, d_out);
    e = hipGetLastError();
  }
  if (e == hipSuccess) e = hipMemcpy(out, d_out, obytes, hipMemcpyDeviceToHost);
  hipFree(d_x); hipFree(d_out); hipFree(d_tab);
  if (e != hipSuccess) return fail(nullptr, CVH_ERR_HIP, "cvh_debug_csv_math: HIP error %d (%s)", (int)e, hipGetErrorString(e));
  return CVH_OK;
}
```

Before: 295,300.

## Run the 2-pixel wave kernel in place on a single padded slab

Adds a one-buffer mode for the single-channel fast f64 wave2 path. The level set lives in one padded slab with per-strip shadow rows and per-column seam slots, so each step reads and writes the same buffer instead of ping-ponging between two. The goal is to shrink the working set enough to stay in the large on-die cache for mid-size images. In exchange it needs extra seam and shadow stores, a pack and unpack on entry and exit, and complex strip-boundary bookkeeping, and it is auto-enabled only under a narrow footprint heuristic.

```diff
diff --git a/chan_vese_amd/csrc/api.hip b/chan_vese_amd/csrc/api.hip
--- a/chan_vese_amd/csrc/api.hip
+++ b/chan_vese_amd/csrc/api.hip
@@ -105,6 +105,8 @@
   if (c->stream) (void)hipStreamSynchronize(c->stream);
   if (c->d_img_slab) (void)hipFree(c->d_img_slab);
   if (c->d_u_slab) (void)hipFree(c->d_u_slab);
+  if (c->d_ob) (void)hipFree(c->d_ob);
+  if (c->d_ob_tab) (void)hipFree(c->d_ob_tab);
   if (c->d_uf_slab) (void)hipFree(c->d_uf_slab);
   for (int k = 0; k < 2; ++k) if (c->d_pm[k]) (void)hipFree(c->d_pm[k]);
   if (c->d_state) (void)hipFree(c->d_state);
@@ -250,6 +252,7 @@
   if (!c || !key) return CVH_ERR_ARG;
   HIPCHK(c, hipSetDevice(c->device));
   { const int rc = settle(c); if (rc != CVH_OK) return rc; }
+  { const int rc = one_buffer_leave(c); if (rc != CVH_OK) return rc; }
   if (!strcmp(key, "math_mode")) {
     if (value < 0 || value > 2) return fail(c, CVH_ERR_ARG, "math_mode must be 0, 1 or 2");
     c->math_mode = (int)value;
@@ -319,6 +322,9 @@
   } else if (!strcmp(key, "wave_seam")) {
     if (value != 0 && value != 1) return fail(c, CVH_ERR_ARG, "wave_seam must be 0 or 1");
     c->wave_seam = (int)value;
+  } else if (!strcmp(key, "one_buffer")) {
+    if (value < -1 || value > 1) return fail(c, CVH_ERR_ARG, "one_buffer must be -1 (auto), 0 or 1");
+    c->one_buffer = (int)value;
   } else if (!strcmp(key, "near_switch")) {
     c->near_switch = value != 0;
   } else if (!strcmp(key, "res_prio")) {
@@ -473,6 +479,7 @@
   c->have_u = true;
   c->sums_valid = false;
   c->mirror_valid = true;
+  c->ob_live = false;
   if (c->state_bits == 32) { const int rc = adopt_f32_state(c); if (rc != CVH_OK) return rc; }
   if (!device_cleared) return reset_run_impl(c);
   begin_run_host(c);
@@ -485,7 +492,7 @@
   if (chain) { c->chain_pending = true; c->pending_nparts = nparts; }
   else c->chain_acc_valid = false;
   c->last_nparts = nparts;
-  if (c->state_bits == 32) c->mirror_valid = false;
+  if (c->state_bits == 32 || c->ob_live) c->mirror_valid = false;
   c->enqueued += n;
 }
 
@@ -522,9 +529,15 @@
 
 int ensure_f64_mirror(cvh_context *c)
 {
-  if (c->state_bits != 32 || c->mirror_valid) return CVH_OK;
+  if ((c->state_bits != 32 && !c->ob_live) || c->mirror_valid) return CVH_OK;
   { const int rc = settle(c); if (rc != CVH_OK) return rc; }
   const int cur = current_buffer(c);
+  if (c->ob_live) {
+    HIPCHK(c, cvh_launch_ob_unpack(c->d_ob, c->d_u[cur], c->h, c->w, (c->w + cvh_wave2_cols() - 1) / cvh_wave2_cols(), c->stream));
+    HIPCHK(c, hipStreamSynchronize(c->stream));
+    c->mirror_valid = true;
+    return CVH_OK;
+  }
   HIPCHK(c, cvh_launch_state_widen(c->d_uf[cur], c->d_u[cur], c->n, c->stream));
   HIPCHK(c, hipStreamSynchronize(c->stream));
   c->mirror_valid = true;
@@ -740,8 +753,8 @@
   CvhStepArgs a;
   fill_args(c, &a, current_buffer(c), c->enqueued);
   snprintf(buf, (size_t)cap, "kernel=%s grid=%u block=%u lds_bytes=%u data_flow=%d wave_columns=%d strips=%d strip_rows=%d chain=%d "
-           "wave_pol=%d math=%s steps_per_graph=%d wave_seam=%d", note.name, note.grid, note.block, note.lds, g.strip, g.tiles_x, g.tiles_y,
+           "wave_pol=%d math=%s steps_per_graph=%d wave_seam=%d one_buffer=%d", note.name, note.grid, note.block, note.lds, g.strip, g.tiles_x, g.tiles_y,
            g.strip_rows, a.chain ? 1 : 0, a.wave_pol, use_fast(c) ? "fast" : "strict", c->use_graph ? kGraphSteps : 0,
-           (g.strip == 3 && use_fast(c)) ? a.wave_seam : 0);
-  return CVH_OK;
-}
+           (g.strip == 3 && use_fast(c)) ? a.wave_seam : 0, a.one_buffer);
+  return CVH_OK;
+}
diff --git a/chan_vese_amd/csrc/csv_batch.hip b/chan_vese_amd/csrc/csv_batch.hip
--- a/chan_vese_amd/csrc/csv_batch.hip
+++ b/chan_vese_amd/csrc/csv_batch.hip
@@ -186,6 +186,7 @@
   for (int i = 0; i < n; ++i) {
     cvh_context *c = ctxs[i];
     c->geom_cus = 0;
+    c->in_batch = on;
     if (!on || resolve_geometry(c).strip_rows >= kBatchOwnRows) continue;
     const int share = (int)((double)c->num_cus * (double)c->n / tot + 0.5);
     c->geom_cus = share < 1 ? 1 : share;
@@ -201,6 +202,7 @@
     if (rc != CVH_OK) return batch_fail(ctxs, n, rc, "batch: member %d: %s", i, c->err);
     const Geometry g = resolve_geometry(c);
     rc = upload_strip_bounds(c, g);
+    if (rc == CVH_OK) rc = one_buffer_leave(c);
     if (rc == CVH_OK) rc = flush_for_grid(c, g.nblocks);
     if (rc == CVH_OK) rc = prepare(c);
     if (rc != CVH_OK) return batch_fail(ctxs, n, rc, "batch: member %d: %s", i, c->err);
diff --git a/chan_vese_amd/csrc/csv_run.hip b/chan_vese_amd/csrc/csv_run.hip
--- a/chan_vese_amd/csrc/csv_run.hip
+++ b/chan_vese_amd/csrc/csv_run.hip
@@ -63,6 +63,83 @@
   return (g.strip == 3 || g.strip == 2) && use_fast(c) && c->finalize_mode == 0 && c->chain_opt;
 }
 
+bool one_buffer_rule(const cvh_context *c, const Geometry &g, bool alone)
+{
+  if (c->one_buffer == 0 || g.strip != 3 || c->C != 1 || !use_fast(c) || c->state_bits != 64 || c->p.tol != 0.0) return false;
+  if (c->wave_pol == 2 || c->in_batch) return false;
+  if (c->resident_opt != 0) {
+    ResidentGeom rg;
+    if (resident_tile_grid(c->h, c->w, c->C, c->num_cus, c->num_cus, &rg)) return false;
+  }
+  const double slab = (double)cvh_ob_rows(c->h, g.tiles_y) * cvh_ob_pitch(c->w, g.tiles_x) * sizeof(double);
+  if (slab >= 2147483648.0) return false;
+  if (c->one_buffer == 1) return true;
+  if (c->kernel != -1 || c->strip_rows != 0 || c->strips != 0 || c->wave_cls != 1 || c->wave_cskew != 500 || c->wave_skew != 0) return false;
+  return alone && (double)c->n * 17.0 > kCachedFootprint && slab + (double)c->n <= kCachedFootprint;
+}
+
+bool wants_one_buffer(const cvh_context *c, const Geometry &g) { return one_buffer_rule(c, g, run_is_alone(c)); }
+
+void one_buffer_table(const std::vector<int> &b, int h, std::vector<int> &tab)
+{
+  const int S = (int)b.size() - 1;
+  tab.assign((size_t)S * CVH_OB_TAB, -1);
+  std::vector<int> ne;
+  for (int k = 0; k < S; ++k) if (b[k + 1] > b[k]) ne.push_back(k);
+  for (size_t t = 0; t < ne.size(); ++t) {
+    const int k = ne[t], kp = t > 0 ? ne[t - 1] : -1, kn = t + 1 < ne.size() ? ne[t + 1] : -1, knn = t + 2 < ne.size() ? ne[t + 2] : -1;
+    const int s0 = b[k], s1 = b[k + 1];
+    int *T = &tab[(size_t)k * CVH_OB_TAB];
+    if (kp >= 0) T[0] = 3 * kp + 2;
+    if (kn >= 0) {
+      T[1] = 3 * kn + 1;
+      if (s1 - s0 >= 2) T[3] = 3 * kn;
+      else if (s0 == 0) T[2] = 3 * kn;
+    }
+    if (knn >= 0 && b[kn + 1] - b[kn] == 1) T[4] = 3 * knn;
+    if (s0 > 0) { T[5] = s0 >= 2 ? s0 - 2 : 0; T[6] = s0 - 1; }
+    if (s1 < h) T[7] = s1;
+  }
+}
+
+int one_buffer_flow(cvh_context *c, const Geometry &g)
+{
+  if (!wants_one_buffer(c, g)) return one_buffer_leave(c);
+  const int pitch = cvh_ob_pitch(c->w, g.tiles_x), rows = cvh_ob_rows(c->h, g.tiles_y);
+  const int key[6] = {c->bounds_key[0], c->bounds_key[1], c->bounds_key[2], c->bounds_key[3], pitch, rows};
+  if (c->ob_live && !memcmp(key, c->ob_key, sizeof(key))) return CVH_OK;
+  int rc = c->ob_live ? one_buffer_leave(c) : settle(c);
+  if (rc == CVH_OK) rc = ensure_f64_mirror(c);
+  if (rc != CVH_OK) return rc;
+  const size_t bytes = (size_t)rows * pitch * sizeof(double);
+  if (bytes > c->ob_cap) {
+    HIPCHK(c, hipStreamSynchronize(c->stream));
+    if (c->d_ob) { HIPCHK(c, hipFree(c->d_ob)); c->d_ob = nullptr; c->ob_cap = 0; }
+    HIPCHK(c, hipMalloc((void **)&c->d_ob, bytes));
+    c->ob_cap = bytes;
+  }
+  HIPCHK(c, hipMemsetAsync(c->d_ob, 0, bytes, c->stream));
+  if (!c->d_ob_tab) HIPCHK(c, hipMalloc((void **)&c->d_ob_tab, (size_t)(c->h + 1) * CVH_OB_TAB * sizeof(int)));
+  std::vector<int> tab;
+  one_buffer_table(c->h_bounds, c->h, tab);
+  if ((int)tab.size() != g.tiles_y * CVH_OB_TAB) return fail(c, CVH_ERR_STATE, "one-buffer flow: the strip table does not match the geometry");
+  HIPCHK(c, hipStreamSynchronize(c->stream));
+  HIPCHK(c, hipMemcpy(c->d_ob_tab, tab.data(), tab.size() * sizeof(int), hipMemcpyHostToDevice));
+  const int par = (c->cur_base + c->enqueued) & 1;
+  HIPCHK(c, cvh_launch_ob_pack(c->d_u[par], c->d_ob, c->d_ob_tab, c->h, c->w, g.tiles_x, g.tiles_y, par, c->stream));
+  memcpy(c->ob_key, key, sizeof(key));
+  c->ob_live = true;
+  return CVH_OK;
+}
+
+int one_buffer_leave(cvh_context *c)
+{
+  if (!c->ob_live) return CVH_OK;
+  const int rc = ensure_f64_mirror(c);
+  if (rc == CVH_OK) c->ob_live = false;
+  return rc;
+}
+
 bool resident_tile_grid(int h, int w, int channels, int num_cus, int cap_blocks, ResidentGeom *rg)
 {
   if ((channels != 1 && channels != 3) || (w & 1) || w < 16 || h < 16) return false;
@@ -133,6 +210,14 @@
   a->tile_rows = g.rows;
   a->strip_rows = g.strip_rows;
   a->fused_finalize = c->finalize_mode == 0;
+  if (wants_one_buffer(c, g)) {
+    a->u_in = c->d_ob; a->u_out = c->d_ob;
+    a->one_buffer = 1;
+    a->ob_pitch = cvh_ob_pitch(c->w, g.tiles_x);
+    a->ob_rows = cvh_ob_rows(c->h, g.tiles_y);
+    a->ob_par = in_buf;
+    a->ob_tab = c->d_ob_tab;
+  }
   a->alpha = c->p.mu * c->p.dt;
   a->beta = (1.0 / c->C) * c->p.dt;
   a->gamma = -c->p.nu * c->p.dt;
@@ -225,6 +310,11 @@
       if (rc != CVH_OK) return rc;
       a.u_in = c->d_u[current_buffer(c)];
     }
+    if (a.one_buffer) {
+      const int rc = ensure_f64_mirror(c);
+      if (rc != CVH_OK) return rc;
+      a.u_in = c->d_u[current_buffer(c)];
+    }
     int nparts = 0;
     HIPCHK(c, cvh_launch_init_sums(a, c->C, use_fast(c), &nparts, c->stream));
     a.nparts = nparts;
@@ -289,6 +379,7 @@
   compute_strip_bounds(g.strip, c->h, g.tiles_x, g.tiles_y, g.strip_rows, g.nblocks, cls, cskew, c->wave_skew, b);
   HIPCHK(c, hipStreamSynchronize(c->stream));
   HIPCHK(c, hipMemcpy(c->d_bounds, b.data(), b.size() * sizeof(int), hipMemcpyHostToDevice));
+  c->h_bounds = b;
   memcpy(c->bounds_key, key, sizeof(key));
   return CVH_OK;
 }
@@ -352,9 +443,10 @@
 static int warm_impl(cvh_context *c, long nsteps)
 {
   if (nsteps > 0) c->run_chunk = (int)(nsteps < 1024 ? nsteps : 1024);
-  { ResidentGeom rg; if (resident_geometry(c, &rg)) return CVH_OK; }
+  { ResidentGeom rg; if (resident_geometry(c, &rg)) return one_buffer_leave(c); }
   const Geometry g = resolve_geometry(c);
   if (g.strip >= 2) { const int rc = upload_strip_bounds(c, g); if (rc != CVH_OK) return rc; }
+  { const int rc = one_buffer_flow(c, g); if (rc != CVH_OK) return rc; }
   if (c->use_graph && nsteps >= kGraphSteps) {
     const int ahead = (int)(nsteps % kGraphSteps);
     c->enqueued += ahead;
@@ -380,6 +472,7 @@
 {
   const int ntiles = rg.tr * rg.tc;
   if (!note) { const int rc = ensure_resident_buffers(c); if (rc != CVH_OK) return rc; }
+  if (!note) { const int rc = one_buffer_leave(c); if (rc != CVH_OK) return rc; }
   if (!note) { const int rc = flush_for_grid(c, -1); if (rc != CVH_OK) return rc; }
   constexpr int kMaxPerLaunch = 4096;
   for (int s = 0; s < nsteps || note;) {
@@ -415,6 +508,7 @@
     if (resident_geometry(c, &rg)) return launch_resident(c, rg, nsteps, nullptr);
     const Geometry g = resolve_geometry(c);
     if (g.strip >= 2) { const int rc = upload_strip_bounds(c, g); if (rc != CVH_OK) return rc; }
+    { const int rc = one_buffer_flow(c, g); if (rc != CVH_OK) return rc; }
     const int rc = flush_for_grid(c, g.nblocks);
     if (rc != CVH_OK) return rc;
   }
diff --git a/chan_vese_amd/csrc/csv_wave2_body.inc b/chan_vese_amd/csrc/csv_wave2_body.inc
--- a/chan_vese_amd/csrc/csv_wave2_body.inc
+++ b/chan_vese_amd/csrc/csv_wave2_body.inc
@@ -124,15 +124,38 @@
     using raw2_t = typename IO::raw2_t;
     using raw1_t = typename IO::raw1_t;
     constexpr unsigned SB = IO::kBytes;
-    const unsigned rowbytes = (unsigned)w * SB, ubytes = (unsigned)h * rowbytes;
-    const unsigned voff_u = (unsigned)cl * SB;
+    const unsigned pitch = OB ? (unsigned)a.ob_pitch : (unsigned)w;
+    const unsigned rowbytes = pitch * SB, ubytes = (unsigned)(OB ? a.ob_rows : h) * rowbytes;
+    const unsigned voff_u = (OB && lane == 0 && wc > 0) ? (unsigned)cvh_ob_slot(w, nwc, a.ob_par, wc - 1, 0) * SB : (unsigned)cl * SB;
     const unsigned voff_st = lane_valid ? (unsigned)c0 * SB : kOobOffset;
-    const unsigned voff_x = ((unsigned)xrow * (unsigned)w + (unsigned)xcol) * SB;
+    const unsigned xoff = (OB && wc + 1 < nwc) ? (unsigned)cvh_ob_slot(w, nwc, a.ob_par, wc + 1, 1) : (unsigned)xcol;
+    const unsigned voff_x = ((unsigned)xrow * pitch + xoff) * SB;
+    const unsigned voff_sh = !OB ? 0u
+        : (lane == 63 && wc + 1 < nwc) ? (unsigned)cvh_ob_slot(w, nwc, a.ob_par ^ 1, wc, 0) * SB
+        : (lane == 1 && wc > 0) ? (unsigned)cvh_ob_slot(w, nwc, a.ob_par ^ 1, wc, 1) * SB : kOobOffset;
     const __amdgpu_buffer_rsrc_t ru = make_rsrc(a.u_in, ubytes);
     const int ulast = s1 < h - 1 ? s1 : h - 1, ilast = s1 - 1;
-    auto U = [&](int r) -> raw2_t { return IO::load2(ru, voff_u, (unsigned)clampi(r, 0, ulast) * rowbytes); };
+    const int llast = OB ? ilast : ulast;
+    const int sh_rd = OB ? cvh_ob_shadow_row(h, nstrips, a.ob_par, 3 * ws) : 0, sh_wr = OB ? cvh_ob_shadow_row(h, nstrips, a.ob_par ^ 1, 0) : 0;
+    int pub[5] = {-1, -1, -1, -1, -1};
+    if (OB) {
+      const const_int_p t = (const_int_p)a.ob_tab + ws * CVH_OB_TAB;
+#pragma unroll
+      for (int q = 0; q < 5; ++q) pub[q] = t[q];
+    }
+    auto rowsel = [&](int r) -> int {
+      if (!OB) return clampi(r, 0, ulast);
+      if (r < s0) return s0 == 0 ? 0 : sh_rd + (r - (s0 - 2));
+      if (r >= s1) return s1 < h ? sh_rd + 2 : h - 1;
+      return r;
+    };
+    auto U = [&](int r) -> raw2_t { return IO::load2(ru, voff_u, (unsigned)rowsel(r) * rowbytes); };
     auto UX = [&](int r0) -> raw1_t {
-      if (r0 + R - 1 <= ulast) return IO::load1(ru, voff_x, (unsigned)r0 * rowbytes);
+      if (r0 + R - 1 <= llast) return IO::load1(ru, voff_x, (unsigned)r0 * rowbytes);
+      if (OB) {
+        const int rr = r0 + xrow;
+        return IO::load1(ru, ((unsigned)(rr >= s1 ? (s1 < h ? sh_rd + 2 : h - 1) : rr) * pitch + xoff) * SB, 0u);
+      }
       return IO::load1(ru, ((unsigned)clampi(r0 + xrow, 0, ulast) * (unsigned)w + (unsigned)xcol) * SB, 0u);
     };
     unsigned char *simg = reinterpret_cast<unsigned char *>(xs + R * XP2 + 64);
@@ -320,6 +343,7 @@
         hva = heaviside_strict(va, eps); hvb = heaviside_strict(vb, eps);
       }
       IO::store2(keep[k], make_rsrc(a.u_out, live ? ubytes : 0u), voff_st, (unsigned)i * rowbytes);
+      if (OB) IO::store2(keep[k], make_rsrc(a.u_out, live ? ubytes : 0u), voff_sh, (unsigned)i * rowbytes);
       if (live) {
         if (FAST && DEFER && NEARFORM) {
           acc[2 + 2 * C] = __builtin_fma(uda, uda, acc[2 + 2 * C]); acc[2 + 2 * C] = __builtin_fma(udb, udb, acc[2 + 2 * C]);
@@ -386,6 +410,20 @@
         if (INTERIOR || (ib + k) < s1) row(ib + k, k, true, near_tag);
         else near_mask[k] = 0ull;
       }
+      if (OB && !INTERIOR) {
+        auto put = [&](int k, int d) {
+          if (d >= 0) IO::store2(keep[k], make_rsrc(a.u_out, ubytes), voff_st, (unsigned)(sh_wr + d) * rowbytes);
+        };
+#pragma unroll
+        for (int k = 0; k < R; ++k) {
+          const int i = ib + k;
+          if (i < s1) {
+            if (i == s0) put(k, pub[0]);
+            if (i == s1 - 1) { put(k, pub[1]); put(k, pub[2]); put(k, pub[4]); }
+            if (i == s1 - 2) put(k, pub[3]);
+          }
+        }
+      }
       const bool any_near = DEFER && !NEARFORM && (near_mask[0] | near_mask[1] | near_mask[2] | near_mask[3]) != 0ull;
       auto finish_row = [&](int k, int smp0, auto table_tag) {
         constexpr bool TABLE = decltype(table_tag)::value;
@@ -442,7 +480,17 @@
     int ib = s0;
     const bool near_strip = DEFER && a.near_switch &&
         __builtin_popcountll(__builtin_amdgcn_ballot_w64(lane_valid && (fabs(u0.x) < fc.thr || fabs(u0.y) < fc.thr))) >= 32;
-    if (__builtin_expect(DEFER && near_strip, 0)) {
+    if (OB) {
+      if (__builtin_expect(near_strip, 0)) {
+        if (ib < s1) { group(ib, std::false_type{}, std::true_type{}); ib += R; }
+        for (; ib + 2 * R <= llast; ib += R) group(ib, std::true_type{}, std::true_type{});
+        for (; ib < s1; ib += R) group(ib, std::false_type{}, std::true_type{});
+      } else {
+        if (ib < s1) { group(ib, std::false_type{}, std::false_type{}); ib += R; }
+        for (; ib + 2 * R <= llast; ib += R) group(ib, std::true_type{}, std::false_type{});
+        for (; ib < s1; ib += R) group(ib, std::false_type{}, std::false_type{});
+      }
+    } else if (__builtin_expect(DEFER && near_strip, 0)) {
       for (; ib + 2 * R <= ulast; ib += R) group(ib, std::true_type{}, std::true_type{});
       for (; ib < s1; ib += R) group(ib, std::false_type{}, std::true_type{});
     } else {
diff --git a/chan_vese_amd/csrc/csv_wave2_kernel.hip b/chan_vese_amd/csrc/csv_wave2_kernel.hip
--- a/chan_vese_amd/csrc/csv_wave2_kernel.hip
+++ b/chan_vese_amd/csrc/csv_wave2_kernel.hip
@@ -12,6 +12,7 @@
 template <int C, bool FAST, int MINW, int POL, bool ST32>
 __global__ __launch_bounds__(CVH_BLOCK, MINW) void csv_wave2_kernel(const CvhStepArgs a)
 {
+  constexpr bool OB = false;
   const unsigned blk = blockIdx.x;
 #include "csv_wave2_body.inc"
 }
@@ -23,7 +24,44 @@
   const CvhStepArgs *const ap = batch_member(b, &blk);
   if (!ap) return;
   const CvhStepArgs &a = *ap;
+  constexpr bool OB = false;
 #include "csv_wave2_body.inc"
+}
+
+template <int POL>
+__global__ __launch_bounds__(CVH_BLOCK, 3) void csv_wave2_ob_kernel(const CvhStepArgs a)
+{
+  constexpr int C = 1, MINW = 3;
+  constexpr bool FAST = true, ST32 = false, OB = true;
+  const unsigned blk = blockIdx.x;
+#include "csv_wave2_body.inc"
+}
+
+__global__ __launch_bounds__(CVH_BLOCK) void ob_pack_kernel(const double *dense, double *slab, const int *tab, int h, int w, int nwc, int nstrips, int par)
+{
+  const int pitch = cvh_ob_pitch(w, nwc), r = (int)blockIdx.x;
+  if (r < h) {
+    const double *src = dense + (size_t)r * w;
+    double *dst = slab + (size_t)r * pitch;
+    for (int j = threadIdx.x; j < w; j += CVH_BLOCK) dst[j] = src[j];
+    for (int q = threadIdx.x; q < 4 * nwc; q += CVH_BLOCK) {
+      const int wc = q >> 2, b = (q >> 1) & 1, col = W2 * wc + (b ? 0 : W2 - 2) + (q & 1);
+      dst[cvh_ob_slot(w, nwc, par, wc, b) + (q & 1)] = col < w ? src[col] : 0.0;
+    }
+    return;
+  }
+  const int q = r - h, from = tab[(q / 3) * CVH_OB_TAB + 5 + q % 3];
+  if (from < 0) return;
+  const double *src = dense + (size_t)from * w;
+  double *dst = slab + (size_t)cvh_ob_shadow_row(h, nstrips, par, q) * pitch;
+  for (int j = threadIdx.x; j < w; j += CVH_BLOCK) dst[j] = src[j];
+}
+
+__global__ __launch_bounds__(CVH_BLOCK) void ob_unpack_kernel(const double *slab, double *dense, int w, int pitch)
+{
+  const double *src = slab + (size_t)blockIdx.x * pitch;
+  double *dst = dense + (size_t)blockIdx.x * w;
+  for (int j = threadIdx.x; j < w; j += CVH_BLOCK) dst[j] = src[j];
 }
 
 template <int C, bool FAST, int MINW, int POL, bool ST32 = false>
@@ -38,9 +76,29 @@
   return hipGetLastError();
 }
 
+template <int POL>
+hipError_t launch_wave2_ob(const CvhStepArgs &a, hipStream_t s)
+{
+  using L = Wave2Smem<true, 1>;
+  CVH_LAUNCH((csv_wave2_ob_kernel<POL>), a.nparts + (a.chain ? 1 : 0), L::bytes, s, a, "csv_wave2_ob_kernel<%d>", POL);
+  return hipGetLastError();
+}
+
 }
 
 int cvh_wave2_cols() { return W2; }
+
+hipError_t cvh_launch_ob_pack(const double *dense, double *slab, const int *tab, int h, int w, int nwc, int nstrips, int par, hipStream_t s)
+{
+  hipLaunchKernelGGL(ob_pack_kernel, dim3(h + 3 * nstrips), dim3(CVH_BLOCK), 0, s, dense, slab, tab, h, w, nwc, nstrips, par);
+  return hipGetLastError();
+}
+
+hipError_t cvh_launch_ob_unpack(const double *slab, double *dense, int h, int w, int nwc, hipStream_t s)
+{
+  hipLaunchKernelGGL(ob_unpack_kernel, dim3(h), dim3(CVH_BLOCK), 0, s, slab, dense, w, cvh_ob_pitch(w, nwc));
+  return hipGetLastError();
+}
 
 hipError_t cvh_launch_wave2(const CvhStepArgs &a, int channels, int fast, hipStream_t s, const CvhBatchLaunch *batch)
 {
@@ -50,6 +108,10 @@
   }
   if (channels == 3) return a.wave_pol ? launch_wave2<3, true, 3, 1>(a, s, batch) : launch_wave2<3, true, 3, 0>(a, s, batch);
   if (!fast) return launch_wave2<1, false, 2, 1>(a, s, batch);
+  if (a.one_buffer) {
+    if (batch || a.wave_pol == 2) return hipErrorInvalidValue;
+    return a.wave_pol ? launch_wave2_ob<1>(a, s) : launch_wave2_ob<0>(a, s);
+  }
   if (a.wave_pol == 2) return launch_wave2<1, true, 3, 2>(a, s, batch);
   return a.wave_pol ? launch_wave2<1, true, 3, 1>(a, s, batch) : launch_wave2<1, true, 3, 0>(a, s, batch);
 }
diff --git a/chan_vese_amd/csrc/cvh_host.h b/chan_vese_amd/csrc/cvh_host.h
--- a/chan_vese_amd/csrc/cvh_host.h
+++ b/chan_vese_amd/csrc/cvh_host.h
@@ -17,6 +17,8 @@
 
 struct DeviceTable { void *d = nullptr; size_t cap = 0, count = 0; };
 
+constexpr int CVH_ONE_BUFFER_DEFAULT = -1;
+constexpr double kCachedFootprint = 205e6;
 constexpr int kGraphSteps = 16;
 struct StepGraph { hipGraphExec_t exec = nullptr; CvhStepArgs key[4]; int kind = -1, flavour = -1; };
 struct BatchCache;
@@ -47,6 +49,10 @@
   double *d_atan = nullptr;
   CvhChainAcc *d_chain = nullptr;
   int *d_bounds = nullptr;
+  std::vector<int> h_bounds;
+  double *d_ob = nullptr;
+  size_t ob_cap = 0;
+  int *d_ob_tab = nullptr;
   unsigned long long *d_isums = nullptr, *h_isums = nullptr;
   unsigned long long *d_dbg = nullptr;
   size_t dbg_words = 0;
@@ -61,6 +67,8 @@
   double sum_img[CVH_MAX_CHANNELS] = {0, 0, 0};
   double stop_norm = 0.0;
   bool mirror_valid = true;
+  bool ob_live = false;
+  int ob_key[6] = {0, 0, 0, 0, 0, 0};
   int cur_base = 0;
   int enqueued = 0;
   int steps_done = 0;
@@ -75,6 +83,7 @@
   mutable int run_alone = -1;
   int run_chunk = -1;
   int geom_cus = 0;
+  bool in_batch = false;
   double stop_cond_h = 0.0;
   float last_run_ms = 0.f, last_pm_ms = 0.f;
   float last_reinit_ms = 0.f;
@@ -89,6 +98,7 @@
   int wave_minw = 5, wave_lds_cap = 0, wave_prio = 1, wave_sync = -1 , wave_imgv = 1, wave_depth = 4;
   int res_prio = 1;
   int res_go_share = 5;
+  int one_buffer = CVH_ONE_BUFFER_DEFAULT;
   int wave_seam = 1;
   int near_switch = 1;
   int wave_rev = 0, wave_xcd = 1;
@@ -193,6 +203,11 @@
 int prepare(cvh_context *c);
 void compute_strip_bounds(int kind, int h, int tiles_x, int S, int strip_rows, int nblocks, int cls, int cskew, int skew, std::vector<int> &b);
 int upload_strip_bounds(cvh_context *c, const Geometry &g);
+bool one_buffer_rule(const cvh_context *c, const Geometry &g, bool alone);
+bool wants_one_buffer(const cvh_context *c, const Geometry &g);
+void one_buffer_table(const std::vector<int> &b, int h, std::vector<int> &tab);
+int one_buffer_flow(cvh_context *c, const Geometry &g);
+int one_buffer_leave(cvh_context *c);
 int launch_one_step(cvh_context *c, int in_buf, int step, bool capturing = false, CvhLaunchNote *note = nullptr);
 int flush_for_grid(cvh_context *c, int nparts);
 int ensure_resident_buffers(cvh_context *c);
diff --git a/chan_vese_amd/csrc/cvh_internal.h b/chan_vese_amd/csrc/cvh_internal.h
--- a/chan_vese_amd/csrc/cvh_internal.h
+++ b/chan_vese_amd/csrc/cvh_internal.h
@@ -99,7 +99,18 @@
   int res_prio;
   int res_band_rows;
   int res_go_shift;
-};
+  int one_buffer;
+  int ob_pitch;
+  int ob_rows;
+  int ob_par;
+  const int *ob_tab;
+};
+
+#define CVH_OB_TAB 8
+__host__ __device__ constexpr int cvh_ob_pitch(int w, int nwc) { return (w + 8 * nwc + 15) & ~15; }
+__host__ __device__ constexpr int cvh_ob_slot(int w, int nwc, int par, int wc, int b) { return w + 4 * nwc * par + 4 * wc + 2 * b; }
+__host__ __device__ constexpr int cvh_ob_rows(int h, int nstrips) { return h + 6 * nstrips; }
+__host__ __device__ constexpr int cvh_ob_shadow_row(int h, int nstrips, int par, int idx) { return h + 3 * nstrips * par + idx; }
 
 struct CvhBatchEntry { unsigned member, first, nblk, pad; };
 struct CvhBatchArgs { const CvhBatchEntry *map; const CvhStepArgs *args; };
@@ -275,6 +286,8 @@
 hipError_t cvh_launch_step(const CvhStepArgs &a, int channels, int fast, hipStream_t s);
 int cvh_wave2_cols();
 hipError_t cvh_launch_wave2(const CvhStepArgs &a, int channels, int fast, hipStream_t s, const CvhBatchLaunch *batch = nullptr);
+hipError_t cvh_launch_ob_pack(const double *dense, double *slab, const int *tab, int h, int w, int nwc, int nstrips, int par, hipStream_t s);
+hipError_t cvh_launch_ob_unpack(const double *slab, double *dense, int h, int w, int nwc, hipStream_t s);
 hipError_t cvh_launch_chain_flush(const CvhStepArgs &a, int channels, hipStream_t s);
 size_t cvh_pm_resident_lds_bytes();
 int cvh_pm_resident_halo_doubles();
diff --git a/chan_vese_amd/csrc/debug_exports.hip b/chan_vese_amd/csrc/debug_exports.hip
--- a/chan_vese_amd/csrc/debug_exports.hip
+++ b/chan_vese_amd/csrc/debug_exports.hip
@@ -24,6 +24,26 @@
   if (tiles_x) *tiles_x = g.tiles_x;
   if (tiles_y) *tiles_y = g.tiles_y;
   if (strip_rows) *strip_rows = g.strip_rows;
+  return CVH_OK;
+}
+
+extern "C" int cvh_debug_one_buffer(int h, int w, int channels, int math_mode, int kernel, int state_bits, int num_cus, int live, double tol,
+                                    int option)
+{
+  if (h < 1 || w < 1 || (channels != 1 && channels != 3)) return -1;
+  cvh_context c;
+  c.h = h; c.w = w; c.C = channels; c.n = (size_t)h * (size_t)w;
+  c.math_mode = math_mode; c.kernel = kernel; c.state_bits = state_bits; c.num_cus = num_cus > 0 ? num_cus : 256;
+  c.p.tol = tol; c.one_buffer = option;
+  return one_buffer_rule(&c, resolve_geometry(&c), live <= 1) ? 1 : 0;
+}
+
+extern "C" int cvh_debug_one_buffer_table(const int *b, int S, int h, int *out)
+{
+  if (!b || !out || S < 1) return CVH_ERR_ARG;
+  std::vector<int> tab;
+  one_buffer_table(std::vector<int>(b, b + S + 1), h, tab);
+  memcpy(out, tab.data(), tab.size() * sizeof(int));
   return CVH_OK;
 }
 
```

New measurement: 303,700 (median of 6 runs). 1.03x the previous value.
